# kwai/blaze

Hardware: NVIDIA H100
Metric: rows/sec on TPC-DS q1 hash-agg+filter at 1/2/4/8 H100; HBM GB/s vs 3.35 TB/s (higher is better)
Workload: dtype int64

## Files before the change

blaze_b200/csrc/capi.cu:

```cuda
#include <algorithm>
#include <cstdio>
#include <cstdlib>
#include <cstring>
#include <functional>
#include <mutex>

#include "lz4_frame.h"
#include "parquet_meta.h"
#include "runtime.h"

namespace b200q {

static thread_local std::string g_last_error;

static std::string format_of(const DType& t) {
  switch (t.id) {
    case T_BOOL: return "b"; case T_INT8: return "c"; case T_INT16: return "s"; case T_INT32: return "i"; case T_INT64: return "l";
    case T_FLOAT32: return "f"; case T_FLOAT64: return "g"; case T_DATE32: return "tdD"; case T_TIMESTAMP_US: return "tsu:";
    case T_DECIMAL128: return "d:" + std::to_string(t.precision) + "," + std::to_string(t.scale);
    case T_BINARY: return "z"; case T_UTF8: return "u"; default: return "n";
  }
}
DType type_of_format(const char* f) {
  DType d; std::string s(f ? f : "");
// ... 501 lines not shown
      const int32_t first = ho[0];
      hc.values = d2h((const uint8_t*)dc.values->ptr + first, (size_t)(ho[n] - first));
      if (first) for (int64_t i = 0; i <= n; i++) ho[i] -= first;
    } else if (dc.type.id == T_BOOL) hc.values = d2h(dc.values->ptr, (size_t)(n + 7) / 8);
    else if (dc.type.id != T_NULL) hc.values = d2h(dc.values->ptr, (size_t)n * dc.type.byte_width());
    hb.cols.push_back(hc);
  }
  B200Q_CUDA(cudaStreamSynchronize(cx.stream));
  return hb;
}

struct ArrayPriv {
  std::shared_ptr<HostBlock> block;
  std::vector<DevMemP> dev;
  std::vector<const void*> buffers;
  std::vector<ArrowArray> children; std::vector<ArrowArray*> child_ptrs;
};
static void release_array(ArrowArray* a) {
  if (!a || !a->release) return;
  auto* p = (ArrayPriv*)a->private_data;
  for (auto& c : p->children) if (c.release) c.release(&c);
  delete p; a->release = nullptr;
}
static int64_t count_nulls(const uint8_t* bits, int64_t off, int64_t n) {
  int64_t set = 0;
  for (int64_t i = 0; i < n; i++) set += (bits[(off + i) >> 3] >> ((off + i) & 7)) & 1;
  return n - set;
}
static void export_host_slice(const HostBatch& hb, int64_t off, int64_t len, ArrowArray* out) {
  auto* top = new ArrayPriv(); top->block = hb.block;
  memset(out, 0, sizeof(*out));
  out->length = len; out->null_count = 0; out->offset = 0; out->n_buffers = 1;
  top->buffers.push_back(nullptr); out->buffers = top->buffers.data();
  top->children.resize(hb.cols.size()); top->child_ptrs.resize(hb.cols.size());
  for (size_t i = 0; i < hb.cols.size(); i++) {
    const HostColumn& hc = hb.cols[i];
    auto* cp = new ArrayPriv(); cp->block = hb.block;
    ArrowArray& c = top->children[i]; memset(&c, 0, sizeof(c));
    c.length = len; c.offset = off;
    c.null_count = hc.validity ? count_nulls((const uint8_t*)hc.validity, off, len) : 0;
    if (hc.type.id == T_NULL) { c.null_count = len; c.n_buffers = 0; }
    else if (hc.type.is_varlen()) { cp->buffers = {hc.validity, hc.offsets, hc.values}; c.n_buffers = 3; }
    else { cp->buffers = {hc.validity, hc.values}; c.n_buffers = 2; }
    c.buffers = cp->buffers.data(); c.release = release_array; c.private_data = cp;
    top->child_ptrs[i] = &c;
  }
  out->n_children = (int64_t)hb.cols.size(); out->children = top->child_ptrs.data();
  out->release = release_array; out->private_data = top;
}
void export_device(DevBatch& db, int device, ArrowDeviceArray* out) {
  auto* top = new ArrayPriv();
  memset(out, 0, sizeof(*out));
  ArrowArray& a = out->array;
  a.length = db.num_rows; a.n_buffers = 1; top->buffers.push_back(nullptr); a.buffers = top->buffers.data();
  top->children.resize(db.cols.size()); top->child_ptrs.resize(db.cols.size());
  for (size_t i = 0; i < db.cols.size(); i++) {
    DevColumn& dc = db.cols[i];
    auto* cp = new ArrayPriv();
    ArrowArray& c = top->children[i]; memset(&c, 0, sizeof(c));
    c.length = db.num_rows; c.offset = dc.offset; c.null_count = dc.validity ? -1 : 0;
    const void* v = dc.validity ? dc.validity->ptr : nullptr;
    if (dc.validity) cp->dev.push_back(dc.validity);
    if (dc.values) cp->dev.push_back(dc.values);
    if (dc.offsets) cp->dev.push_back(dc.offsets);
    if (dc.type.id == T_NULL) { c.n_buffers = 0; c.null_count = db.num_rows; }
    else if (dc.type.is_varlen()) { cp->buffers = {v, dc.offsets->ptr, dc.values->ptr}; c.n_buffers = 3; }
    else { cp->buffers = {v, dc.values ? dc.values->ptr : nullptr}; c.n_buffers = 2; }
    c.buffers = cp->buffers.data(); c.release = release_array; c.private_data = cp;
    top->child_ptrs[i] = &c;
  }
  a.n_children = (int64_t)db.cols.size(); a.children = top->child_ptrs.data();
  a.release = release_array; a.private_data = top;
  out->device_id = device; out->device_type = ARROW_DEVICE_CUDA; out->sync_event = nullptr;
}

static void conf_defaults(b200q_conf* c) {
  memset(c, 0, sizeof(*c));
  c->struct_size = sizeof(b200q_conf);
  c->batch_size = 10000;
  c->suggested_batch_mem_size = 8388608;
  c->partial_agg_skipping_enable = 1;
  c->partial_agg_skipping_ratio = 0.999;
  c->partial_agg_skipping_min_rows = 20000;
  c->staging_rows = 1 << 20;
  c->agg_initial_groups = 1 << 19;
  c->max_launch_rows = 1 << 27;
  c->partial_state_columnar = 0;
  c->force_generic_kernels = 0;
  c->agg_dense_keys = 1;
  c->agg_hot_key_cache = 1;
}

}

#define B200Q_STR2(x) #x
#define B200Q_STR(x) B200Q_STR2(x)

extern "C" {

int32_t b200q_version(void) { return 100; }
const char* b200q_build_info(void) { return "blaze_b200 hot path: Filter/Project/HashAgg, sm_90a, CUDA " B200Q_STR(CUDART_VERSION); }
const char* b200q_last_error(void) { return g_last_error.c_str(); }
int32_t b200q_device_count(void) { int n = 0; if (cudaGetDeviceCount(&n) != cudaSuccess) { cudaGetLastError(); return 0; } return n; }

b200q_status b200q_conf_init(b200q_conf* conf) {
  if (!conf) return fail(B200Q_ERR_INVALID_ARG, "conf is null");
  conf_defaults(conf); return B200Q_OK;
}

b200q_status b200q_plan_explain(const uint8_t* plan, size_t plan_len, int32_t plan_kind, char* buf, size_t cap, size_t* needed) {
  return guarded(nullptr, [&] {
    PlanP p = decode_plan(plan, plan_len, plan_kind);
    std::string s = explain_plan(p);
    if (needed) *needed = s.size() + 1;
    if (buf && cap) { const size_t n = std::min(cap - 1, s.size()); memcpy(buf, s.data(), n); buf[n] = 0; }
  });
}

b200q_status b200q_op_create(const uint8_t* plan, size_t plan_len, int32_t plan_kind, const struct ArrowSchema* input_schema,
                             const b200q_conf* conf, int32_t device, b200q_op** out) {
  if (!out) return fail(B200Q_ERR_INVALID_ARG, "out is null");
  *out = nullptr;
  b200q_op* op = nullptr;
  b200q_status st = guarded(nullptr, [&] {
    PlanP p = decode_plan(plan, plan_len, plan_kind);
    resolve_scalar_subqueries(*p);
    int ndev = 0;
    if (cudaGetDeviceCount(&ndev) != cudaSuccess || ndev == 0) { cudaGetLastError(); throw ExecError(B200Q_ERR_NO_DEVICE, "no CUDA device is visible: the sm_90a kernels cannot run and there is no CPU fallback"); }
    if (device < 0 || device >= ndev) throw ExecError(B200Q_ERR_INVALID_ARG, "invalid device ordinal");
    op = new b200q_op();
    op->plan = p; op->cx.device = device;
    conf_defaults(&op->cx.conf);
    if (conf) { const size_t n = std::min<size_t>(conf->struct_size ? conf->struct_size : sizeof(b200q_conf), sizeof(b200q_conf)); memcpy(&op->cx.conf, conf, n); op->cx.conf.struct_size = sizeof(b200q_conf); }
    if (op->cx.conf.batch_size <= 0) op->cx.conf.batch_size = 10000;
    if (op->cx.conf.max_launch_rows <= 0) op->cx.conf.max_launch_rows = 1 << 27;
    if (op->cx.conf.agg_initial_groups <= 0) op->cx.conf.agg_initial_groups = 1 << 19;
    B200Q_CUDA(cudaSetDevice(device));
    {
      cudaMemPool_t pool; unsigned long long keep = ~0ULL;
      if (cudaDeviceGetDefaultMemPool(&pool, device) == cudaSuccess) cudaMemPoolSetAttribute(pool, cudaMemPoolAttrReleaseThreshold, &keep);
    }
    op->stream_ref = stream_ref_create(device);
    op->cx.stream = op->stream_ref->s;
    B200Q_CUDA(cudaEventCreate(&op->cx.ev0)); B200Q_CUDA(cudaEventCreate(&op->cx.ev1));
    build_pipeline(op);
    if (op->leaf->leaf_kind == "IpcReader") op->ipc = make_ipc_source(op->cx, op->in_schema, op->stages[0]->used_input_cols);
    if (input_schema) {
      if (input_schema->n_children != (int64_t)op->in_schema.fields.size()) throw PlanError(B200Q_ERR_INVALID_ARG, "input_schema does not match the plan leaf: column count");
      for (int64_t i = 0; i < input_schema->n_children; i++)
        if (type_of_format(input_schema->children[i]->format) != op->in_schema.fields[i].type)
          throw PlanError(B200Q_ERR_INVALID_ARG, "input_schema does not match the plan leaf: type of column " + std::to_string(i));
    }
  });
  if (st != B200Q_OK) { if (op) { op->stages.clear(); delete op; } return st; }
  *out = op;
  return B200Q_OK;
}

b200q_status b200q_op_input_schema(b200q_op* op, struct ArrowSchema* out) {
  if (!op || !out) return fail(B200Q_ERR_INVALID_ARG, "null argument");
  return guarded(nullptr, [&] { export_schema(op->in_schema, out); });
}
b200q_status b200q_op_output_schema(b200q_op* op, struct ArrowSchema* out) {
  if (!op || !out) return fail(B200Q_ERR_INVALID_ARG, "null argument");
  return guarded(nullptr, [&] { export_schema(op->out_schema, out); });
}

b200q_status b200q_op_push(b200q_op* op, struct ArrowArray* batch) {
  if (!op) return fail(B200Q_ERR_INVALID_ARG, "op is null");
  b200q_status st = guarded(op, [&] {
    check_push_state(op);
    begin_push(op, batch);
    op->cx.m.input_rows += batch->length; op->cx.m.input_batches++;
    if (batch->length == 0) return;
    const std::vector<int>& used = op->stages[0]->used_input_cols;
    const int64_t srows = op->cx.conf.staging_rows;
    if (srows > 0 && batch->length < srows / 2) { staging_append(op, batch); return; }
    if (op->staging_ready) staging_flush(op);
    DevBatch db = import_direct(op, batch, used);
    PendingRelease pr; pr.arr = *batch; batch->release = nullptr;
    B200Q_CUDA(cudaEventCreateWithFlags(&pr.ev, cudaEventDisableTiming));
    B200Q_CUDA(cudaEventRecord(pr.ev, op->cx.stream));
    op->pending.push_back(pr);
    run_stages(op, db, 0);
  });
  if (batch && batch->release) batch->release(batch);
  return st;
}

b200q_status b200q_op_push_ipc(b200q_op* op, const uint8_t* data, size_t len) {
  if (!op) return fail(B200Q_ERR_INVALID_ARG, "op is null");
  return guarded(op, [&] {
    if (op->finished) throw ExecError(B200Q_ERR_STATE, "push after finish");
    if (!op->ipc) throw ExecError(B200Q_ERR_STATE, "push_ipc: the op's leaf is not an IpcReaderExecNode");
    if (!data && len) throw ExecError(B200Q_ERR_INVALID_ARG, "push_ipc: null data");
    require_right_side(op);
    B200Q_CUDA(cudaSetDevice(op->cx.device));
    poll_pending(op, false);
    op->ipc->push(op->cx, data, len, [&](DevBatch& b) { run_stages(op, b, 0); });
  });
}

b200q_status b200q_op_push_device(b200q_op* op, struct ArrowDeviceArray* dbatch) {
  if (!op) return fail(B200Q_ERR_INVALID_ARG, "op is null");
  b200q_status st = guarded(op, [&] {
    check_push_state(op);
    if (!dbatch) throw ExecError(B200Q_ERR_INVALID_ARG, "null batch");
    if (dbatch->device_type != ARROW_DEVICE_CUDA || dbatch->device_id != op->cx.device) throw ExecError(B200Q_ERR_INVALID_ARG, "push_device: batch is not on this op's CUDA device");
    ArrowArray* batch = &dbatch->array;
    begin_push(op, batch);
    if (op->staging_ready) staging_flush(op);
    if (dbatch->sync_event) B200Q_CUDA(cudaStreamWaitEvent(op->cx.stream, *(cudaEvent_t*)dbatch->sync_event, 0));
    op->cx.m.input_rows += batch->length; op->cx.m.input_batches++;
    if (batch->length == 0) return;
    DevBatch db; db.num_rows = batch->length; db.cols.resize(op->in_schema.fields.size());
    for (size_t i = 0; i < db.cols.size(); i++) {
      const ArrowArray* c = batch->children[i]; DevColumn& dc = db.cols[i];
      dc.type = op->in_schema.fields[i].type; dc.offset = c->offset + batch->offset;
      const size_t huge = (size_t)1 << 60;
      if (c->n_buffers > 0 && c->buffers[0] && c->null_count != 0) dc.validity = DevMem::borrow(c->buffers[0], huge, nullptr);
      if (dc.type.is_varlen()) { dc.offsets = DevMem::borrow(c->buffers[1], huge, nullptr); dc.values = DevMem::borrow(c->buffers[2], huge, nullptr); }
      else if (c->n_buffers > 1 && c->buffers[1]) dc.values = DevMem::borrow(c->buffers[1], huge, nullptr);
    }
    PendingRelease pr; pr.arr = *batch;
    B200Q_CUDA(cudaEventCreateWithFlags(&pr.ev, cudaEventDisableTiming));
    batch->release = nullptr;
    op->pending.push_back(pr);
    const cudaEvent_t ev = pr.ev;
    try { run_stages(op, db, 0); } catch (...) { cudaEventRecord(ev, op->cx.stream); throw; }
    B200Q_CUDA(cudaEventRecord(ev, op->cx.stream));
  });
  if (dbatch && dbatch->array.release) dbatch->array.release(&dbatch->array);
  return st;
}

b200q_status b200q_op_finish(b200q_op* op) {
  if (!op) return fail(B200Q_ERR_INVALID_ARG, "op is null");
  return guarded(op, [&] {
    if (op->finished) return;
    require_right_side(op);
    B200Q_CUDA(cudaSetDevice(op->cx.device));
    if (op->leaf->leaf_kind == "ParquetScan") {
      if (op->cx.m.input_batches) throw ExecError(B200Q_ERR_STATE, "an op whose leaf is a ParquetScanExecNode takes no pushed batches");
      run_parquet_scan(op->cx, *op->leaf, [&](DevBatch& b) { run_stages(op, b, 0); });
    }
    if (op->ipc) op->ipc->flush(op->cx, [&](DevBatch& b) { run_stages(op, b, 0); });
    if (op->staging_ready) staging_flush(op);
    for (size_t i = 0; i < op->stages.size(); i++) {
      std::vector<DevBatch> outs;
      op->cx.cur_stage = (int)i;
      op->stages[i]->finish(op->cx, outs);
      route_outputs(op, i, outs);
    }
    B200Q_CUDA(cudaStreamSynchronize(op->cx.stream));
    poll_pending(op, true);
    op->finished = true;
  });
}

b200q_status b200q_op_pull(b200q_op* op, struct ArrowArray* out, int32_t* has_batch) {
  if (!op || !out || !has_batch) return fail(B200Q_ERR_INVALID_ARG, "null argument");
  *has_batch = 0;
  return guarded(op, [&] {
    if (op->taken) throw ExecError(B200Q_ERR_STATE, "pull: the op's output is the right side of a sort-merge join (b200q_op_attach_right)");
    B200Q_CUDA(cudaSetDevice(op->cx.device));
    if (!op->has_cur_host) {
      if (op->out_queue.empty()) return;
      op->cur_host = to_host(op, op->out_queue.front());
      op->out_queue.pop_front();
      op->has_cur_host = true;
    }
    HostBatch& hb = op->cur_host;
    const int64_t len = std::min<int64_t>(op->cx.conf.batch_size, hb.num_rows - hb.cursor);
    export_host_slice(hb, hb.cursor, len, out);
    hb.cursor += len;
    if (hb.cursor >= hb.num_rows) { op->has_cur_host = false; op->cur_host = HostBatch(); }
    op->cx.m.output_batches++;
    *has_batch = 1;
  });
}

b200q_status b200q_op_pull_device(b200q_op* op, struct ArrowDeviceArray* out, int32_t* has_batch) {
  if (!op || !out || !has_batch) return fail(B200Q_ERR_INVALID_ARG, "null argument");
  *has_batch = 0;
  return guarded(op, [&] {
    if (op->taken) throw ExecError(B200Q_ERR_STATE, "pull_device: the op's output is the right side of a sort-merge join (b200q_op_attach_right)");
    if (op->has_cur_host) throw ExecError(B200Q_ERR_STATE, "pull_device while a host batch is partially pulled");
    if (op->out_queue.empty()) return;
    B200Q_CUDA(cudaSetDevice(op->cx.device));
    B200Q_CUDA(cudaStreamSynchronize(op->cx.stream));
    export_device(op->out_queue.front(), op->cx.device, out);
    op->out_queue.pop_front();
    op->cx.m.output_batches++;
    *has_batch = 1;
  });
}

b200q_status b200q_op_sync(b200q_op* op) {
  if (!op) return fail(B200Q_ERR_INVALID_ARG, "op is null");
  return guarded(op, [&] { B200Q_CUDA(cudaSetDevice(op->cx.device)); B200Q_CUDA(cudaStreamSynchronize(op->cx.stream)); poll_pending(op, true); });
}

b200q_status b200q_op_metrics(b200q_op* op, b200q_metrics* out) {
  if (!op || !out) return fail(B200Q_ERR_INVALID_ARG, "null argument");
  const Metrics& m = op->cx.m;
  b200q_metrics r; memset(&r, 0, sizeof(r)); r.struct_size = sizeof(r);
  r.input_rows = m.input_rows; r.input_batches = m.input_batches; r.output_rows = m.output_rows; r.output_batches = m.output_batches;
  r.elapsed_compute_ns = (int64_t)(m.gpu_ms * 1e6); r.gpu_kernel_launches = m.launches; r.h2d_bytes = m.h2d_bytes; r.d2h_bytes = m.d2h_bytes;
  r.hot_kernel_ns = (int64_t)(m.hot_ms * 1e6); r.hot_kernel_rows = m.hot_rows; r.hot_kernel_launches = m.hot_launches;
  r.num_groups = m.num_groups; r.table_capacity_slots = m.table_capacity; r.table_grow_count = m.grow_count; r.fast_path_launches = m.fast_launches;
  const size_t n = std::min<size_t>(out->struct_size ? out->struct_size : sizeof(r), sizeof(r));
  memcpy(out, &r, n);
  return B200Q_OK;
}

void b200q_op_destroy(b200q_op* op) {
  if (!op) return;
  cudaSetDevice(op->cx.device);
  if (op->cx.stream) cudaStreamSynchronize(op->cx.stream);
  poll_pending(op, true);
  op->out_queue.clear(); op->has_cur_host = false; op->cur_host = HostBatch();
  op->ipc.reset();
  op->stages.clear();
  staging_free(op);
  if (op->cx.ev0) cudaEventDestroy(op->cx.ev0);
  if (op->cx.ev1) cudaEventDestroy(op->cx.ev1);
  if (op->cx.stream) cudaStreamSynchronize(op->cx.stream);
  delete op;
}

b200q_status b200q_parquet_explain(const uint8_t* footer, size_t n, char* buf, size_t cap, size_t* needed) {
  return guarded(nullptr, [&] {
    const PqFileMeta m = parquet_parse_footer(footer, n);
    std::string o = "rows=" + std::to_string(m.num_rows) + " flat=" + (m.flat ? "true" : "false") + "\n";
    for (auto& c : m.columns) o += "column " + c.name + " physical=" + std::to_string(c.type) + (c.optional ? " optional" : " required") + " arrow=" + (c.arrow.id == T_NULL ? std::string("unsupported") : c.arrow.str()) + "\n";
    for (size_t g = 0; g < m.row_groups.size(); g++) {
      o += "row_group " + std::to_string(g) + " rows=" + std::to_string(m.row_groups[g].num_rows) + "\n";
      for (size_t c = 0; c < m.row_groups[g].columns.size(); c++) {
        const PqColumnChunk& cc = m.row_groups[g].columns[c];
        o += "  chunk " + std::to_string(c) + " codec=" + std::to_string(cc.codec) + " values=" + std::to_string(cc.num_values) + " start=" + std::to_string(cc.start()) + " bytes=" + std::to_string(cc.total_compressed_size) +
             " nulls=" + std::to_string(cc.stats.null_count) + " min_max=" + (cc.stats.has_min && cc.stats.has_max ? "yes" : "no") + "\n";
      }
    }
    if (needed) *needed = o.size() + 1;
    if (buf && cap) { const size_t k = std::min(cap - 1, o.size()); memcpy(buf, o.data(), k); buf[k] = 0; }
  });
}
b200q_status b200q_snappy_uncompress(const uint8_t* src, size_t n, uint8_t* dst, size_t cap, size_t* out_len) {
  if ((!src && n) || !out_len) return fail(B200Q_ERR_INVALID_ARG, "null argument");
  return guarded(nullptr, [&] {
    ByteBuf v; snappy_uncompress(src, n, v);
    *out_len = v.size();
    if (!dst || cap < v.size()) throw ExecError(B200Q_ERR_INVALID_ARG, "snappy output needs " + std::to_string(v.size()) + " bytes");
    if (v.size()) memcpy(dst, v.data(), v.size());
  });
}
b200q_status b200q_set_file_reader(b200q_file_reader_fn fn, void* ctx) { set_file_reader(fn, ctx); return B200Q_OK; }
b200q_status b200q_set_scalar_subquery_resolver(b200q_scalar_subquery_fn fn, void* ctx) { set_scalar_subquery_resolver((void*)fn, ctx); return B200Q_OK; }

b200q_status b200q_op_attach_build(b200q_op* probe_op, b200q_op* build_op) {
  if (!probe_op || !build_op) return fail(B200Q_ERR_INVALID_ARG, "null argument");
  return guarded(probe_op, [&] {
    const JoinBuildResult* b = build_op->stages.empty() ? nullptr : dynamic_cast<const JoinBuildResult*>(build_op->stages.back().get());
    if (!b) throw ExecError(B200Q_ERR_STATE, "attach_build: the build op's plan is not rooted at a BroadcastJoinBuildHashMapExecNode");
    if (!build_op->finished || !b->built()) throw ExecError(B200Q_ERR_STATE, "attach_build: finish the build op first");
    JoinProbeAttach* a = nullptr;
    for (auto& st : probe_op->stages) if (auto* j = dynamic_cast<JoinProbeAttach*>(st.get())) a = j;
    if (!a) throw ExecError(B200Q_ERR_STATE, "attach_build: the probe op's plan has no join");
    a->attach(b->built());
  });
}

b200q_status b200q_op_attach_right(b200q_op* join_op, b200q_op* right_op) {
  if (!join_op || !right_op || join_op == right_op) return fail(B200Q_ERR_INVALID_ARG, "attach_right: null or identical op handles");
  if (right_op->sticky_code) return fail(right_op->sticky_code, right_op->sticky_error);
  return guarded(join_op, [&] {
    SmjRightAttach* j = smj_of(join_op);
    if (!j) throw ExecError(B200Q_ERR_STATE, "attach_right: the op's plan has no SortMergeJoinExecNode");
    if (j->right_attached()) throw ExecError(B200Q_ERR_STATE, "attach_right: a right side is already attached");
    if (join_op->finished || join_op->cx.m.input_batches) throw ExecError(B200Q_ERR_STATE, "attach_right: the join op already has input");
    if (!right_op->finished) throw ExecError(B200Q_ERR_STATE, "attach_right: finish the right op first");
    if (right_op->taken || right_op->has_cur_host || right_op->cx.m.output_batches) throw ExecError(B200Q_ERR_STATE, "attach_right: the right op's output has already been pulled or attached");
    if (right_op->cx.device != join_op->cx.device) throw ExecError(B200Q_ERR_INVALID_ARG, "attach_right: the right op runs on another device");
    B200Q_CUDA(cudaSetDevice(join_op->cx.device));
    std::vector<DevBatch> batches(right_op->out_queue.begin(), right_op->out_queue.end());
    j->attach_right(join_op->cx, batches, right_op->out_schema);
    right_op->out_queue.clear();
    right_op->taken = true;
  });
}

b200q_status b200q_op_shuffle_chunk_count(b200q_op* op, int64_t* out_count) {
  if (!op || !out_count) return fail(B200Q_ERR_INVALID_ARG, "null argument");
  return guarded(op, [&] {
    const ShuffleResult* r = op->stages.empty() ? nullptr : dynamic_cast<const ShuffleResult*>(op->stages.back().get());
    if (!r) throw ExecError(B200Q_ERR_STATE, "the plan is not rooted at a ShuffleWriterExecNode");
    *out_count = r->chunk_count();
  });
}
b200q_status b200q_op_shuffle_chunk(b200q_op* op, int64_t index, b200q_shuffle_chunk* out) {
  if (!op || !out) return fail(B200Q_ERR_INVALID_ARG, "null argument");
  return guarded(op, [&] {
    const ShuffleResult* r = op->stages.empty() ? nullptr : dynamic_cast<const ShuffleResult*>(op->stages.back().get());
    if (!r) throw ExecError(B200Q_ERR_STATE, "the plan is not rooted at a ShuffleWriterExecNode");
    if (index < 0 || index >= r->chunk_count()) throw ExecError(B200Q_ERR_INVALID_ARG, "shuffle chunk index out of range");
    r->chunk(index, out);
  });
}
b200q_status b200q_lz4_frame_compress(const uint8_t* src, size_t n, uint8_t* dst, size_t cap, size_t* out_len) {
  if ((!src && n) || !out_len) return fail(B200Q_ERR_INVALID_ARG, "null argument");
  return guarded(nullptr, [&] {
    std::vector<uint8_t> v; lz4_frame_append(src, n, v);
    *out_len = v.size();
    if (!dst || cap < v.size()) throw ExecError(B200Q_ERR_INVALID_ARG, "lz4 frame needs " + std::to_string(v.size()) + " bytes");
    memcpy(dst, v.data(), v.size());
  });
}

b200q_status b200q_lz4_frame_decompress(const uint8_t* src, size_t n, uint8_t* dst, size_t cap, size_t* out_len) {
  if ((!src && n) || !out_len) return fail(B200Q_ERR_INVALID_ARG, "null argument");
  return guarded(nullptr, [&] {
    size_t bound = 0;
    try {
      bound = lz4_frame_bound(src, n);
      if (dst && cap >= bound) { *out_len = lz4_frame_decompress(src, n, dst, cap); return; }
      std::vector<uint8_t> v(bound);
      *out_len = lz4_frame_decompress(src, n, v.data(), v.size());
      if (dst && cap >= *out_len) { memcpy(dst, v.data(), *out_len); return; }
    } catch (const Lz4FrameError& e) {
      throw ExecError(B200Q_ERR_INVALID_ARG, std::string(e.what()) + " at byte " + std::to_string(e.offset));
    }
    throw ExecError(B200Q_ERR_INVALID_ARG, "lz4 frame content needs " + std::to_string(*out_len) + " bytes");
  });
}

b200q_status b200q_murmur3_partition(const struct ArrowSchema* key_schema, const struct ArrowDeviceArray* keys, int32_t num_partitions,
                                     uint32_t* out_pids_device, void* cuda_stream) {
  return guarded(nullptr, [&] {
    if (!key_schema || !keys || !out_pids_device) throw ExecError(B200Q_ERR_INVALID_ARG, "null argument");
    if (num_partitions <= 0) throw ExecError(B200Q_ERR_INVALID_ARG, "num_partitions must be positive");
    const ArrowArray& a = keys->array;
    if (a.n_children != key_schema->n_children || a.n_children > VM_MAX_COLS) throw ExecError(B200Q_ERR_INVALID_ARG, "key schema / array mismatch");
    ColTable ct{}; uint8_t phys[VM_MAX_COLS];
    for (int64_t i = 0; i < a.n_children; i++) {
      const DType t = type_of_format(key_schema->children[i]->format);
      if (t.is_varlen()) throw ExecError(B200Q_ERR_UNSUPPORTED, "murmur3 partition ids over a " + t.str() + " key are not on the GPU path");
      const ArrowArray* c = a.children[i];
      DevColumn dc; dc.type = t; dc.offset = c->offset + a.offset;
      phys[i] = phys_of(t);
      const int w = t.byte_width();
      ct.col[i].values = c->n_buffers > 1 ? (const uint8_t*)c->buffers[1] + (size_t)dc.offset * w : nullptr;
      ct.col[i].validity = (c->n_buffers > 0 && c->null_count != 0) ? (const uint8_t*)c->buffers[0] : nullptr;
      ct.col[i].bit_offset = (uint32_t)dc.offset;
    }
    launch_murmur3_partition(ct, phys, (int)a.n_children, a.length, num_partitions, out_pids_device, (cudaStream_t)cuda_stream);
    B200Q_CUDA(cudaGetLastError());
  });
}

}
```

blaze_b200/csrc/kernels.cu:

```cuda
#include <cstdio>
#include <cstdlib>
#include <cuda_runtime.h>
#include <stdint.h>

#include "agg_device.cuh"
#include "kernels.cuh"
#include "vm.cuh"
#include "emit_device.cuh"

namespace b200q {

__device__ __forceinline__ void load_program(const VmProgram* __restrict__ g, VmInstr* s_code, uint64_t* s_pool) {
  const uint32_t nc = g->n_code, np = g->n_pool;
  for (uint32_t i = threadIdx.x; i < nc; i += blockDim.x) s_code[i] = g->code[i];
  for (uint32_t i = threadIdx.x; i < np; i += blockDim.x) s_pool[i] = g->pool[i];
  __syncthreads();
}

constexpr int FP_BLOCK = 256;
constexpr int FP_R = 2;
constexpr int FP_TILE = FP_BLOCK * FP_R;
constexpr int FP_NW = FP_BLOCK / 32;
constexpr unsigned long long ST_AGG = 1ULL << 62, ST_PREFIX = 2ULL << 62, ST_VALUE = (1ULL << 62) - 1;

// ... 465 lines not shown
  unsigned flags;
  bool inserted = false;
  const uint64_t slot = agg_find_or_insert(lay, tab, kw, knull, h, &flags, &inserted);
  if (slot == AGG_NO_SLOT) return false;
  if (inserted) atomicAdd(tab.counters, 1ULL);
  unsigned long long* const ke = tab.keys + slot * (uint64_t)lay.kstride;
  unsigned long long* const ae = tab.accs + slot * (uint64_t)lay.astride;
  const uint32_t skip = sd->acc_skip;
  int lost = -1;
  for (int j = 0; j < lay.nacc; j++) {
    if ((skip >> j) & 1) continue;
    const AccOp a = lay.acc[j];
    if (acc_is_first(a.kind)) {
      const int o = sd->acc_arg[j][0];
      const bool ov = o != AGG_NO_ARG && ((vb >> o) & 1);
      if (a.oword != lost && first_eligible(a, lay, buf, vb, o, sd->acc_arg[j][1]) &&
          !first_apply(ke, ae, a, buf + lay.out_word[o == AGG_NO_ARG ? 0 : o], ov, ord)) lost = a.oword;
      continue;
    }
    bool valid = true;
    for (int i = 0; i < 4; i++) { const int o = sd->acc_arg[j][i]; if (o != AGG_NO_ARG) valid = valid && ((vb >> o) & 1); }
    if (!valid) continue;
    const int o = sd->acc_arg[j][0];
    acc_apply(a.kind, ke, ae + a.word, buf + lay.out_word[o == AGG_NO_ARG ? 0 : o]);
    slot_mark(ke, flags, a.vbit);
  }
  return true;
}

__global__ void __launch_bounds__(AG_BLOCK) agg_update_kernel(const VmProgram* __restrict__ prog, const ColTable cols, const AggLayout lay, const AggTable tab,
                                                              long long row_begin, long long n, const uint32_t* __restrict__ row_list,
                                                              unsigned long long ord_base) {
  __shared__ VmInstr s_code[VM_MAX_CODE];
  __shared__ uint64_t s_pool[VM_MAX_POOL];
  load_program(prog, s_code, s_pool);
  int* err = (int*)(tab.counters + 2);
  const long long ntiles = (n + AG_TILE - 1) / AG_TILE;
  for (long long tile = blockIdx.x; tile < ntiles; tile += gridDim.x) {
    long long row[AG_R]; bool inb[AG_R], alive[AG_R];
    uint32_t rel[AG_R];
#pragma unroll
    for (int r = 0; r < AG_R; r++) {
      const long long i = tile * AG_TILE + r * AG_BLOCK + threadIdx.x;
      inb[r] = i < n; alive[r] = inb[r];
      rel[r] = inb[r] ? (row_list ? row_list[i] : (uint32_t)i) : 0;
      row[r] = row_begin + rel[r];
    }
    uint64_t buf[AG_R][AGG_MAX_ROW_WORDS];
    uint32_t vb[AG_R];
#pragma unroll
    for (int r = 0; r < AG_R; r++) vb[r] = 0;
    AggSink sink{buf, vb, lay.out_word};
    vm_run<AG_R>(s_code, s_pool, 0, cols, row, inb, alive, err, sink);
#pragma unroll
    for (int r = 0; r < AG_R; r++) {
      if (alive[r] && !agg_upsert(lay, tab, buf[r], vb[r], ord_base + (unsigned long long)row[r])) {
        const unsigned long long at = atomicAdd(tab.counters + 1, 1ULL);
        tab.deferred[at] = rel[r];
      }
    }
  }
}

__global__ void __launch_bounds__(AG_BLOCK) agg_update_sets_kernel(const VmProgram* __restrict__ prog, const ColTable cols, const AggLayout lay, const AggTable tab,
                                                                   long long row_begin, long long n, const uint32_t* __restrict__ row_list,
                                                                   const AggSetDesc* __restrict__ sets, int nsets, unsigned long long ord_base) {
  __shared__ VmInstr s_code[VM_MAX_CODE];
  __shared__ uint64_t s_pool[VM_MAX_POOL];
  load_program(prog, s_code, s_pool);
  int* err = (int*)(tab.counters + 2);
  const long long ntiles = (n + AG_TILE - 1) / AG_TILE;
  for (long long tile = blockIdx.x; tile < ntiles; tile += gridDim.x) {
    long long row[AG_R]; bool inb[AG_R], alive[AG_R];
    uint32_t rel[AG_R]; int only[AG_R];
#pragma unroll
    for (int r = 0; r < AG_R; r++) {
      const long long i = tile * AG_TILE + r * AG_BLOCK + threadIdx.x;
      inb[r] = i < n; alive[r] = inb[r];
      const uint32_t e = inb[r] ? (row_list ? row_list[i] : (uint32_t)i) : 0;
      rel[r] = row_list ? e / (uint32_t)nsets : e;
      only[r] = row_list ? (int)(e % (uint32_t)nsets) : -1;
      row[r] = row_begin + rel[r];
    }
    uint64_t buf[AG_R][AGG_MAX_ROW_WORDS];
    uint32_t vb[AG_R];
#pragma unroll
    for (int r = 0; r < AG_R; r++) vb[r] = 0;
    AggSink sink{buf, vb, lay.out_word};
    vm_run<AG_R>(s_code, s_pool, 0, cols, row, inb, alive, err, sink);
#pragma unroll
    for (int r = 0; r < AG_R; r++) {
      if (!alive[r]) continue;
      const int s0 = only[r] < 0 ? 0 : only[r], s1 = only[r] < 0 ? nsets : only[r] + 1;
      for (int s = s0; s < s1; s++) {
        if (!agg_upsert_set(lay, tab, buf[r], vb[r], sets + s, (ord_base + (unsigned long long)row[r]) * (unsigned)nsets + (unsigned)s)) {
          const unsigned long long at = atomicAdd(tab.counters + 1, 1ULL);
          tab.deferred[at] = rel[r] * (uint32_t)nsets + (uint32_t)s;
        }
      }
    }
  }
}

static int grid_for(int64_t ntiles, int per_sm) {
  int dev = 0, sms = 132; cudaGetDevice(&dev); cudaDeviceGetAttribute(&sms, cudaDevAttrMultiProcessorCount, dev);
  const int64_t cap = (int64_t)sms * per_sm;
  return (int)(ntiles < cap ? (ntiles < 1 ? 1 : ntiles) : cap);
}

int launch_agg_update(const VmProgram* d_prog, const ColTable& cols, const AggLayout& lay, const AggTable& tab, int64_t row_begin, int64_t n,
                      const uint32_t* d_row_list, uint64_t ord_base, cudaStream_t s) {
  if (n <= 0) return 0;
  const int64_t ntiles = (n + AG_TILE - 1) / AG_TILE;
  agg_update_kernel<<<grid_for(ntiles, 8), AG_BLOCK, 0, s>>>(d_prog, cols, lay, tab, row_begin, n, d_row_list, ord_base);
  return 1;
}

int launch_agg_update_sets(const VmProgram* d_prog, const ColTable& cols, const AggLayout& lay, const AggTable& tab, int64_t row_begin, int64_t n,
                           const uint32_t* d_row_list, const AggSetDesc* d_sets, int nsets, uint64_t ord_base, cudaStream_t s) {
  if (n <= 0) return 0;
  const int64_t ntiles = (n + AG_TILE - 1) / AG_TILE;
  agg_update_sets_kernel<<<grid_for(ntiles, 8), AG_BLOCK, 0, s>>>(d_prog, cols, lay, tab, row_begin, n, d_row_list, d_sets, nsets, ord_base);
  return 1;
}

__global__ void __launch_bounds__(256) agg_rehash_kernel(const AggLayout lay, const AggTable old_tab, const AggTable new_tab) {
  const uint64_t cap = old_tab.capacity;
  for (uint64_t i = blockIdx.x * (uint64_t)blockDim.x + threadIdx.x; i < cap; i += (uint64_t)gridDim.x * blockDim.x) {
    const unsigned long long* src = old_tab.keys + i * (uint64_t)lay.kstride;
    const unsigned long long hdr = src[0];
    if ((unsigned)hdr < 2) continue;
    const unsigned knull = (unsigned)(hdr >> 48);
    const uint64_t h = agg_hash_words((const uint64_t*)src + 1, lay.nkw, knull);
    uint64_t s = agg_first_slot(h, new_tab.capacity);
    while (true) {
      unsigned long long* dst = new_tab.keys + s * (uint64_t)lay.kstride;
      if (atomicCAS((unsigned*)dst, TAG_EMPTY, TAG_LOCKED) == TAG_EMPTY) {
        for (int w = 1; w < lay.kstride; w++) dst[w] = src[w];
        for (int w = 0; w < lay.astride; w++) new_tab.accs[s * (uint64_t)lay.astride + w] = old_tab.accs[i * (uint64_t)lay.astride + w];
        ((unsigned*)dst)[1] = (unsigned)(hdr >> 32) & ~FLAG_SLOT_LOCK;
        __threadfence();
        st_release_u32((unsigned*)dst, (unsigned)hdr);
        atomicAdd(new_tab.counters, 1ULL);
        break;
      }
      s = agg_next_slot(s, new_tab.capacity);
    }
  }
}

int launch_agg_rehash(const AggLayout& lay, const AggTable& old_tab, const AggTable& new_tab, cudaStream_t s) {
  const int64_t cap = (int64_t)old_tab.capacity;
  agg_rehash_kernel<<<grid_for((cap + 255) / 256, 8), 256, 0, s>>>(lay, old_tab, new_tab);
  return 1;
}

__global__ void __launch_bounds__(256) agg_emit_kernel(const AggLayout lay, const AggTable tab, const EmitTable emit, unsigned long long* out_count) {
  const uint64_t cap = tab.capacity;
  const unsigned lane = threadIdx.x & 31;
  const uint64_t stride = (uint64_t)gridDim.x * blockDim.x;
  const uint64_t rounds = (cap + stride - 1) / stride;
  for (uint64_t it = 0; it < rounds; it++) {
    const uint64_t i = it * stride + blockIdx.x * (uint64_t)blockDim.x + threadIdx.x;
    const unsigned long long* ke = tab.keys + i * (uint64_t)lay.kstride;
    const unsigned long long* slot = tab.accs + i * (uint64_t)lay.astride;
    unsigned long long hdr = 0;
    if (i < cap) hdr = ke[0];
    const bool occ = (unsigned)hdr >= 2;
    const unsigned m = __ballot_sync(0xffffffffu, occ);
    if (!m) continue;
    unsigned long long base = 0;
    if (lane == 0) base = atomicAdd(out_count, (unsigned long long)__popc(m));
    base = __shfl_sync(0xffffffffu, base, 0);
    if (!occ) continue;
    const unsigned long long at = base + __popc(m & lanemask_lt());
    const unsigned flags = (unsigned)(hdr >> 32);
    emit_row_columns(emit, at, ke, slot, flags);
  }
}

int launch_agg_emit(const AggLayout& lay, const AggTable& tab, const EmitTable& emit, unsigned long long* d_out_count, cudaStream_t s) {
  const int64_t cap = (int64_t)tab.capacity;
  agg_emit_kernel<<<grid_for((cap + 255) / 256, 8), 256, 0, s>>>(lay, tab, emit, d_out_count);
  return 1;
}

__global__ void __launch_bounds__(256) pack_valid_kernel(const uint8_t* __restrict__ bytes, uint32_t* __restrict__ bits, long long n) {
  const long long nwords = (n + 31) / 32;
  const unsigned lane = threadIdx.x & 31;
  const long long warp_id = (blockIdx.x * (long long)blockDim.x + threadIdx.x) >> 5, nwarps = ((long long)gridDim.x * blockDim.x) >> 5;
  for (long long w = warp_id; w < nwords; w += nwarps) {
    const long long i = w * 32 + lane;
    const unsigned m = __ballot_sync(0xffffffffu, i < n && bytes[i] != 0);
    if (lane == 0) bits[w] = m;
  }
}

int launch_pack_valid(const uint8_t* bytes, uint32_t* bits, int64_t n, cudaStream_t s) {
  if (n <= 0) return 0;
  pack_valid_kernel<<<grid_for((n + 8191) / 8192, 8), 256, 0, s>>>(bytes, bits, n);
  return 1;
}

__device__ __forceinline__ int varint_len(unsigned long long v) { int n = 1; while (v >= 128) { v >>= 7; n++; } return n; }

__device__ __forceinline__ unsigned long long state_value_bits(const FrozenField& f, long long i, unsigned long long& hi) {
  hi = 0;
  switch (f.phys) {
    case PH_I8: return (unsigned long long)(long long)((const int8_t*)f.values)[i];
    case PH_I16: return (unsigned long long)(long long)((const int16_t*)f.values)[i];
    case PH_I32: return (unsigned long long)(long long)((const int32_t*)f.values)[i];
    case PH_F32: return (unsigned long long)((const uint32_t*)f.values)[i];
    case PH_DEC128: hi = ((const unsigned long long*)f.values)[2 * i + 1]; return ((const unsigned long long*)f.values)[2 * i];
    default: return ((const unsigned long long*)f.values)[i];
  }
}

__global__ void __launch_bounds__(256) frozen_lengths_kernel(const FrozenTable ft, long long n, int32_t* __restrict__ lengths) {
  for (long long i = blockIdx.x * (long long)blockDim.x + threadIdx.x; i < n; i += (long long)gridDim.x * blockDim.x) {
    int len = 0;
    for (int k = 0; k < ft.nfields; k++) {
      const FrozenField& f = ft.f[k];
      if (f.kind == FZ_COUNT) len += varint_len(((const unsigned long long*)f.values)[i]);
      else if (f.kind == FZ_BOOL) len += 1;
      else len += 1 + ((f.valid ? f.valid[i] != 0 : true) ? f.width : 0);
    }
    lengths[i] = len;
  }
}

__global__ void __launch_bounds__(256) frozen_write_kernel(const FrozenTable ft, long long n, const int32_t* __restrict__ offsets, uint8_t* __restrict__ data) {
  for (long long i = blockIdx.x * (long long)blockDim.x + threadIdx.x; i < n; i += (long long)gridDim.x * blockDim.x) {
    uint8_t* p = data + offsets[i];
    for (int k = 0; k < ft.nfields; k++) {
      const FrozenField& f = ft.f[k];
      if (f.kind == FZ_COUNT) {
        unsigned long long v = ((const unsigned long long*)f.values)[i];
        while (v >= 128) { *p++ = (uint8_t)(128 + (v & 127)); v >>= 7; }
        *p++ = (uint8_t)v;
      } else if (f.kind == FZ_BOOL) {
        const uint8_t v = ((const uint8_t*)f.values)[i] != 0;
        *p++ = f.valid ? (f.valid[i] ? 1 + v : 0) : (v ? 2 : 0);
      } else {
        const bool valid = f.valid ? f.valid[i] != 0 : true;
        *p++ = valid ? 1 : 0;
        if (valid) {
          unsigned long long hi, lo = state_value_bits(f, i, hi);
          for (int b = 0; b < f.width && b < 8; b++) *p++ = (uint8_t)(lo >> (8 * b));
          for (int b = 8; b < f.width; b++) *p++ = (uint8_t)(hi >> (8 * (b - 8)));
        }
      }
    }
  }
}

__global__ void __launch_bounds__(256) frozen_read_kernel(const FrozenTable ft, long long n, const int32_t* __restrict__ offsets, long long obase,
                                                          const uint8_t* __restrict__ data, int* err) {
  for (long long i = blockIdx.x * (long long)blockDim.x + threadIdx.x; i < n; i += (long long)gridDim.x * blockDim.x) {
    const uint8_t* p = data + offsets[obase + i];
    const uint8_t* end = data + offsets[obase + i + 1];
    for (int k = 0; k < ft.nfields; k++) {
      const FrozenField& f = ft.f[k];
      if (f.kind == FZ_COUNT) {
        unsigned long long v = 0; int shift = 0;
        while (true) {
          if (p >= end) { atomicOr(err, 4); break; }
          const uint8_t b = *p++;
          if (b < 128) { v += (unsigned long long)b << shift; break; }
          v += (unsigned long long)(b - 128) << shift; shift += 7;
        }
        ((unsigned long long*)f.values)[i] = v;
      } else if (f.kind == FZ_BOOL) {
        if (p >= end) { atomicOr(err, 4); break; }
        const uint8_t b = *p++;
        if (f.valid) { ((uint8_t*)f.valid)[i] = b != 0; ((uint8_t*)f.values)[i] = b > 1; }
        else ((uint8_t*)f.values)[i] = b != 0;
      } else {
        if (p >= end) { atomicOr(err, 4); break; }
        const bool valid = *p++ == 1;
        unsigned long long lo = 0, hi = 0;
        if (valid) {
          if (p + f.width > end) { atomicOr(err, 4); break; }
          for (int b = 0; b < f.width && b < 8; b++) lo |= (unsigned long long)(*p++) << (8 * b);
          for (int b = 8; b < f.width; b++) hi |= (unsigned long long)(*p++) << (8 * (b - 8));
        }
        ((uint8_t*)f.valid)[i] = valid ? 1 : 0;
        switch (f.phys) {
          case PH_I8: ((int8_t*)f.values)[i] = (int8_t)lo; break;
          case PH_I16: ((int16_t*)f.values)[i] = (int16_t)lo; break;
          case PH_I32: case PH_F32: ((uint32_t*)f.values)[i] = (uint32_t)lo; break;
          case PH_DEC128: ((unsigned long long*)f.values)[2 * i] = lo; ((unsigned long long*)f.values)[2 * i + 1] = hi; break;
          default: ((unsigned long long*)f.values)[i] = lo; break;
        }
      }
    }
  }
}

int launch_frozen_lengths(const FrozenTable& ft, int64_t n, int32_t* lengths, cudaStream_t s) {
  if (n <= 0) return 0;
  frozen_lengths_kernel<<<grid_for((n + 255) / 256, 8), 256, 0, s>>>(ft, n, lengths); return 1;
}
int launch_frozen_write(const FrozenTable& ft, int64_t n, const int32_t* offsets, uint8_t* data, cudaStream_t s) {
  if (n <= 0) return 0;
  frozen_write_kernel<<<grid_for((n + 255) / 256, 8), 256, 0, s>>>(ft, n, offsets, data); return 1;
}
// ... 278 lines not shown
```

blaze_b200/csrc/kernels.cuh:

```cuda
#pragma once
#include <cuda_runtime.h>
#include <stdint.h>

#include "vm.h"

namespace b200q {

constexpr int AGG_MAX_KEYS = 8;
constexpr int AGG_MAX_ACC = 16;
constexpr int AGG_MAX_ROW_WORDS = 24;
constexpr int AGG_MAX_SLOT_WORDS = 32;

enum AccKind : uint8_t {
  ACC_ADD_I64 = 0,
  ACC_ADD_F64,
  ACC_ADD_DEC,
  ACC_COUNT,
  ACC_MIN_I64, ACC_MAX_I64,
  ACC_MIN_F64, ACC_MAX_F64,
  ACC_MIN_DEC, ACC_MAX_DEC,
  ACC_FIRST,
  ACC_FIRST_VALID,
};
__host__ __device__ inline bool acc_is_first(uint8_t kind) { return kind == ACC_FIRST || kind == ACC_FIRST_VALID; }

struct AccOp {
  uint8_t kind;
  uint8_t word;
  uint8_t vbit;
  uint8_t nargs;
  uint8_t arg_out[4];
  uint8_t oword;
  uint8_t nwords;
};

struct AggLayout {
  int32_t nkeys, nkw, nacc, kstride, astride, nouts;
  uint8_t key_out[AGG_MAX_KEYS];
  uint8_t key_word[AGG_MAX_KEYS];
  uint8_t key_nwords[AGG_MAX_KEYS];
  uint8_t out_word[VM_MAX_OUT];
  AccOp acc[AGG_MAX_ACC];
  uint64_t init[AGG_MAX_SLOT_WORDS];
  uint32_t init_flags;
};

constexpr int AGG_MAX_SETS = 64;
constexpr uint8_t AGG_KEY_CONST = 0xFF;
constexpr uint8_t AGG_NO_ARG = 0xFF;
struct AggSetDesc {
  uint8_t key_out[AGG_MAX_KEYS];
  uint8_t acc_arg[AGG_MAX_ACC][4];
  uint32_t key_null;
  uint32_t acc_skip;
  uint64_t key_const[AGG_MAX_KEYS * 2];
};

struct AggTable {
  unsigned long long* keys;
  unsigned long long* accs;
  uint64_t capacity;
  uint64_t max_groups;
  unsigned long long* counters;
  uint32_t* deferred;
};

enum EmitKind : uint8_t {
  EMIT_KEY = 0,
  EMIT_ACC_VALUE,
  EMIT_AVG_F64,
  EMIT_AVG_DEC,
  EMIT_FIRST_VALUE,
  EMIT_FIRST_FLAG,
};
struct EmitCol {
  uint8_t kind, phys, word, word2;
  uint8_t vbit;
  uint8_t key;
  uint8_t sum_is_f64;
  uint8_t is_order_key;
  void* values;
  uint8_t* valid_bytes;
};
constexpr int EMIT_MAX_COLS = 40;
struct EmitTable { int32_t ncols; EmitCol col[EMIT_MAX_COLS]; };

enum FrozenKind : uint8_t { FZ_PRIM = 0, FZ_COUNT = 1, FZ_BOOL = 2 };
struct FrozenField {
  uint8_t kind;
  uint8_t width;
  uint8_t phys;
  uint8_t _pad;
  const void* values;
  const uint8_t* valid;
};
constexpr int FROZEN_MAX_FIELDS = 32;
struct FrozenTable { int32_t nfields; FrozenField f[FROZEN_MAX_FIELDS]; };

int launch_filter_project(const VmProgram* d_prog, const ColTable& cols, const OutTable& outs, int nouts, int64_t n,
                          bool has_filters, unsigned long long* d_tile_status, unsigned long long* d_scratch ,
                          cudaStream_t s);
int64_t filter_project_num_tiles(int64_t n);

struct LeanFpSpec {
  int32_t nfilt, nout;
  struct { int8_t col; uint8_t op; uint8_t _pad[6]; long long lit; } filt[4];
  struct { uint8_t kind; int8_t a; int8_t b; uint8_t _pad[5]; long long lit; } out[8];
};
int launch_filter_project_lean(const ColTable& cols, int ncols , const LeanFpSpec& sp, long long* const* out_values, int64_t n,
                               void* d_work , unsigned long long* d_scratch, cudaStream_t s);
int64_t filter_project_lean_scratch_bytes(int64_t n);

int launch_agg_update(const VmProgram* d_prog, const ColTable& cols, const AggLayout& lay, const AggTable& tab, int64_t row_begin, int64_t n,
                      const uint32_t* d_row_list , uint64_t ord_base, cudaStream_t s);
int launch_agg_update_sets(const VmProgram* d_prog, const ColTable& cols, const AggLayout& lay, const AggTable& tab, int64_t row_begin, int64_t n,
                           const uint32_t* d_row_list, const AggSetDesc* d_sets, int nsets, uint64_t ord_base, cudaStream_t s);
int launch_agg_rehash(const AggLayout& lay, const AggTable& old_tab, const AggTable& new_tab, cudaStream_t s);
int launch_agg_emit(const AggLayout& lay, const AggTable& tab, const EmitTable& emit, unsigned long long* d_out_count, cudaStream_t s);
int launch_pack_valid(const uint8_t* bytes, uint32_t* bits, int64_t n, cudaStream_t s);
int launch_frozen_lengths(const FrozenTable& ft, int64_t n, int32_t* lengths, cudaStream_t s);
int launch_exclusive_scan_i32(const int32_t* in, int32_t* out , int64_t n, int32_t* d_block_sums, cudaStream_t s);
int launch_frozen_write(const FrozenTable& ft, int64_t n, const int32_t* offsets, uint8_t* data, cudaStream_t s);
int launch_frozen_read(const FrozenTable& ft, int64_t n, const int32_t* offsets, int64_t offsets_base, const uint8_t* data, int* d_err, cudaStream_t s);
int launch_murmur3_partition(const ColTable& cols, const uint8_t* phys, int ncols, int64_t n, int32_t num_partitions, uint32_t* out, cudaStream_t s);
int64_t scan_num_blocks(int64_t n);

int launch_varlen_lengths(const DevCol& src, const uint32_t* sel, int64_t m, int32_t* lengths, uint32_t* out_valid, unsigned long long* d_total, cudaStream_t s);
int launch_varlen_copy(const DevCol& src, const uint32_t* sel, int64_t m, const int32_t* out_offsets, uint8_t* out_data, cudaStream_t s);

constexpr int IPC_TILE = 1024;
constexpr int IPC_COPY_PIECE = 32768;
struct IpcFixedJob { const uint8_t* src; uint8_t* dst; int64_t rows; int32_t width; int32_t _pad; };
struct IpcTile { int32_t job; int32_t row0; };
struct IpcBitCol { uint32_t* dst; const uint8_t* const* src; };
struct IpcCopy { const uint8_t* src; uint8_t* dst; int64_t len; };
int launch_ipc_decode_fixed(const IpcFixedJob* jobs, const IpcTile* tiles, int64_t ntiles, cudaStream_t s);
int launch_ipc_decode_bits(const IpcBitCol* cols, int ncols, const int64_t* rec_row , int64_t nrec, int64_t rows, cudaStream_t s);
int launch_ipc_decode_bytes(const IpcCopy* copies, int64_t n, cudaStream_t s);

}
```

blaze_b200/csrc/kernels_fast.cu:

```cuda
#include <algorithm>
#include <cstdlib>
#include <cuda_runtime.h>
#include <stdint.h>

#include "agg_device.cuh"
#include "kernels_fast.cuh"

namespace b200q {

constexpr int FA_BLOCK = 256;

__device__ __forceinline__ uint64_t make_evict_first_policy() {
  uint64_t pol; asm volatile("createpolicy.fractional.L2::evict_first.b64 %0, 1.0;" : "=l"(pol)); return pol;
}
__device__ __forceinline__ long long ld_stream_s64(const long long* p) {
  long long v; const uint64_t pol = make_evict_first_policy();
  asm volatile("ld.global.nc.L1::no_allocate.L2::cache_hint.s64 %0, [%1], %2;" : "=l"(v) : "l"(p), "l"(pol)); return v;
}
__device__ __forceinline__ bool col_valid(const DevCol& c, long long i) {
  if (!c.validity) return true;
  const unsigned long long bi = (unsigned long long)i + c.bit_offset;
  return (__ldg(c.validity + (bi >> 3)) >> (bi & 7)) & 1;
}
__device__ __forceinline__ long long col_load_int(const DevCol& c, int phys, long long i) {
// ... 536 lines not shown
  __syncthreads();
  const unsigned lane = threadIdx.x & 31;
  const long long gwarp = (long long)blockIdx.x * (FA_BLOCK / 32) + (threadIdx.x >> 5), nwarps = (long long)gridDim.x * (FA_BLOCK / 32);
  const long long nunits = (n + 31) / 32;
  const bool add0 = fs.acc[0].kind == FAST_ACC_ADD, add1 = NACC == 2 && fs.acc[1].kind == FAST_ACC_ADD;

  for (long long unit0 = gwarp * U; unit0 < nunits; unit0 += nwarps * U) {
    long long k[U], k1[U]; unsigned long long v0[U], v1[U]; bool alive[U]; unsigned meta[U];
#pragma unroll
    for (int u = 0; u < U; u++) {
      const long long rel = (unit0 + u) * 32 + lane, row = row_begin + rel;
      alive[u] = rel < n; meta[u] = 0xC; k[u] = 0; k1[u] = 0; v0[u] = 1; v1[u] = 1;
      if (!alive[u]) continue;
      if (!TYPED) {
        k[u] = ld_stream_vec((const long long*)cols.col[fs.key_col[0]].values + row, (i64xG<1>*)nullptr).v[0];
        if (NK == 2) k1[u] = ld_stream_vec((const long long*)cols.col[fs.key_col[1]].values + row, (i64xG<1>*)nullptr).v[0];
        if (add0) v0[u] = (unsigned long long)ld_stream_vec((const long long*)cols.col[fs.acc[0].col].values + row, (i64xG<1>*)nullptr).v[0];
        if (add1) v1[u] = (unsigned long long)ld_stream_vec((const long long*)cols.col[fs.acc[1].col].values + row, (i64xG<1>*)nullptr).v[0];
      } else {
        { const DevCol& c = cols.col[fs.key_col[0]]; if (col_valid(c, row)) k[u] = col_load_int(c, fs.key_phys[0], row); else meta[u] |= 1u; }
        if (NK == 2) { const DevCol& c = cols.col[fs.key_col[1]]; if (col_valid(c, row)) k1[u] = col_load_int(c, fs.key_phys[1], row); else meta[u] |= 2u; }
        if (fs.acc[0].col >= 0) {
          const DevCol& c = cols.col[fs.acc[0].col];
          if (!col_valid(c, row)) { meta[u] &= ~4u; v0[u] = 0; } else if (add0) v0[u] = (unsigned long long)col_load_int(c, fs.acc[0].phys, row);
        }
        if (NACC == 2 && fs.acc[1].col >= 0) {
          const DevCol& c = cols.col[fs.acc[1].col];
          if (!col_valid(c, row)) { meta[u] &= ~8u; v1[u] = 0; } else if (add1) v1[u] = (unsigned long long)col_load_int(c, fs.acc[1].phys, row);
        }
      }
    }
    for (int f = 0; f < fs.nfilt; f++) {
      const DevCol& c = cols.col[fs.filt[f].col];
#pragma unroll
      for (int u = 0; u < U; u++) {
        const long long row = row_begin + (unit0 + u) * 32 + lane;
        if (!alive[u]) continue;
        if (!TYPED) alive[u] = cmp_apply(fs.filt[f].op, ld_stream_vec((const long long*)c.values + row, (i64xG<1>*)nullptr).v[0], fs.filt[f].lit);
        else alive[u] = col_valid(c, row) && cmp_apply(fs.filt[f].op, col_load_int(c, fs.filt[f].phys, row), fs.filt[f].lit);
      }
    }
#pragma unroll
    for (int u = 0; u < U; u++) {
      unsigned long long idx;
      const bool in = dense_index<NK>(fs, k[u], k1[u], idx) && alive[u] && !(meta[u] & 3u);
      if (in) {
        unsigned* const e = s_tab + 2 * (unsigned)idx * G;
#pragma unroll
        for (int m = 0; m < 4; m++) {
          if (m >= G) break;
          const int src = fs.dense_word_src[m];
          if (src == -1) smem_add64(e + 2 * m, 1ULL);
          else if (src == 0) { if (meta[u] & 4u) smem_add64(e + 2 * m, v0[u]); }
          else if (src == 1 && NACC == 2) { if (meta[u] & 8u) smem_add64(e + 2 * m, v1[u]); }
          else if (src >= 2) { if (meta[u] & (4u << (src - 2))) smem_add64(e + 2 * m, 1ULL); }
        }
      }
      const bool fb = alive[u] && !in;
      if (__any_sync(0xffffffffu, fb)) {
        bool inserted = false;
        if (fb) {
          uint64_t kw[2] = {(uint64_t)k[u], NK == 2 ? (uint64_t)k1[u] : 0ULL};
          const unsigned knull = meta[u] & 3u;
          unsigned fl = 0;
          const uint64_t si = agg_find_or_insert(lay, tab, kw, knull, agg_hash2(kw[0], kw[1], knull), &fl, &inserted);
          if (si == AGG_NO_SLOT) { const unsigned long long at = atomicAdd(tab.counters + 1, 1ULL); tab.deferred[at] = (uint32_t)((unit0 + u) * 32 + lane); }
          else {
            unsigned long long* const p = tab.accs + si * (uint64_t)lay.astride;
            unsigned long long* const ke = tab.keys + si * (uint64_t)lay.kstride;
            if (meta[u] & 4u) { red_add_u64(p + fs.acc[0].word, v0[u]); slot_mark(ke, fl, fs.acc[0].vbit); }
            if (NACC == 2 && (meta[u] & 8u)) { red_add_u64(p + fs.acc[1].word, v1[u]); slot_mark(ke, fl, fs.acc[1].vbit); }
          }
        }
        const unsigned b = __ballot_sync(0xffffffffu, inserted);
        if (lane == 0 && b) atomicAdd(tab.counters, (unsigned long long)__popc(b));
      }
    }
  }
  __syncthreads();
  for (unsigned w = threadIdx.x; w < nwords; w += FA_BLOCK) {
    const unsigned long long val = (unsigned long long)s_tab[2 * w] | ((unsigned long long)s_tab[2 * w + 1] << 32);
    if (val) red_add_u64(fs.dense_tab + w, val);
  }
}

static int fast_grid(int64_t ntiles) {
  int dev = 0, sms = 132; cudaGetDevice(&dev); cudaDeviceGetAttribute(&sms, cudaDevAttrMultiProcessorCount, dev);
  const int64_t cap = (int64_t)sms * 8;
  return (int)(ntiles < cap ? (ntiles < 1 ? 1 : ntiles) : cap);
}

int launch_agg_fast_update(const ColTable& cols, const FastSpec& fs, const AggLayout& lay, const AggTable& tab, int64_t row_begin, int64_t n, cudaStream_t s) {
  if (n <= 0) return 0;
  const int dg = fs.dense ? fs.dense_stride : 0;
  if (dg && fs.dense_cap * (unsigned long long)dg <= (unsigned long long)DS_MAX_WORDS) {
    const int g = (int)std::max<int64_t>(1, std::min<int64_t>((n + FA_BLOCK * 4 - 1) / (FA_BLOCK * 4), (int64_t)fast_grid(1 << 30) / 8 * 3));
#define B200Q_DS(NACC, TYPED, NK) agg_dense_smem_kernel<NACC, TYPED, NK><<<g, FA_BLOCK, 0, s>>>(cols, fs, lay, tab, row_begin, n)
    if (fs.nkeys == 1) {
      if (fs.lean) { if (fs.nacc == 2) B200Q_DS(2, false, 1); else B200Q_DS(1, false, 1); } else { if (fs.nacc == 2) B200Q_DS(2, true, 1); else B200Q_DS(1, true, 1); }
    } else {
      if (fs.lean) { if (fs.nacc == 2) B200Q_DS(2, false, 2); else B200Q_DS(1, false, 2); } else { if (fs.nacc == 2) B200Q_DS(2, true, 2); else B200Q_DS(1, true, 2); }
    }
#undef B200Q_DS
    return 1;
  }
  if (dg && fs.lean && fs.hot_cache) {
    const int g = fast_grid((n + 32 * 8 * 4 - 1) / (32 * 8 * 4));
#define B200Q_HC(NACC, NK, G) agg_dense_hot_kernel<NACC, NK, G><<<g, FA_BLOCK, 0, s>>>(cols, fs, lay, tab, row_begin, n)
    if (fs.nkeys == 1) {
      if (fs.nacc == 2) { if (dg == 2) B200Q_HC(2, 1, 2); else B200Q_HC(2, 1, 4); } else { if (dg == 2) B200Q_HC(1, 1, 2); else B200Q_HC(1, 1, 4); }
    } else {
      if (fs.nacc == 2) { if (dg == 2) B200Q_HC(2, 2, 2); else B200Q_HC(2, 2, 4); } else { if (dg == 2) B200Q_HC(1, 2, 2); else B200Q_HC(1, 2, 4); }
    }
#undef B200Q_HC
    return 1;
  }
  if (dg && fs.lean && fs.nkeys == 1 && fs.nfilt == 0) {
    const int u = dg == 2 ? 4 : 2;
    const int g = fast_grid((n + 32 * 8 * u - 1) / (32 * 8 * u));
#define B200Q_LD(NACC, G) agg_lean_dense_kernel<NACC, G, 1><<<g, FA_BLOCK, 0, s>>>(cols, fs, lay, tab, row_begin, n)
    if (fs.nacc == 2) { if (dg == 2) B200Q_LD(2, 2); else B200Q_LD(2, 4); } else { if (dg == 2) B200Q_LD(1, 2); else B200Q_LD(1, 4); }
#undef B200Q_LD
    return 1;
  }
  if (dg && fs.nfcol >= 0) {
    if (fs.filt_never) return 0;
    return launch_agg_tile_dense(cols, fs, lay, tab, row_begin, n, s);
  }
  if (dg) {
    const int g = fast_grid((n + 32 * 8 * 4 - 1) / (32 * 8 * 4));
#define B200Q_DR(NACC, NK, G) do { if (fs.lean) agg_dense_row_kernel<NACC, NK, G, false><<<g, FA_BLOCK, 0, s>>>(cols, fs, lay, tab, row_begin, n); \
                                   else agg_dense_row_kernel<NACC, NK, G, true><<<g, FA_BLOCK, 0, s>>>(cols, fs, lay, tab, row_begin, n); } while (0)
    if (fs.nkeys == 1) {
      if (fs.nacc == 2) { if (dg == 2) B200Q_DR(2, 1, 2); else B200Q_DR(2, 1, 4); } else { if (dg == 2) B200Q_DR(1, 1, 2); else B200Q_DR(1, 1, 4); }
    } else {
      if (fs.nacc == 2) { if (dg == 2) B200Q_DR(2, 2, 2); else B200Q_DR(2, 2, 4); } else { if (dg == 2) B200Q_DR(1, 2, 2); else B200Q_DR(1, 2, 4); }
    }
#undef B200Q_DR
    return 1;
  }
  if (!dg) {
    const int64_t tiles = (n + 32 * (LH_BLOCK / 32) * LH_U - 1) / (32 * (LH_BLOCK / 32) * LH_U);
    const int g = (int)std::max<int64_t>(1, std::min<int64_t>(tiles, (int64_t)fast_grid(1 << 30) / 8 * (fs.lean ? 6 : 4)));
#define B200Q_LH(NK, NACC, TYPED) agg_lean_hash_kernel<NK, NACC, TYPED><<<g, LH_BLOCK, 0, s>>>(cols, fs, lay, tab, row_begin, n)
    if (fs.lean) { if (fs.nkeys == 1) { if (fs.nacc == 2) B200Q_LH(1, 2, false); else B200Q_LH(1, 1, false); } else { if (fs.nacc == 2) B200Q_LH(2, 2, false); else B200Q_LH(2, 1, false); } }
    else { if (fs.nkeys == 1) { if (fs.nacc == 2) B200Q_LH(1, 2, true); else B200Q_LH(1, 1, true); } else { if (fs.nacc == 2) B200Q_LH(2, 2, true); else B200Q_LH(2, 1, true); } }
#undef B200Q_LH
    return 1;
  }
  return 0;
}

__global__ void __launch_bounds__(256) key_range_kernel(const DevCol col, int phys, long long n, long long* out ) {
  long long mn = INT64_MAX, mx = INT64_MIN; unsigned long long cnt = 0;
  for (long long i = blockIdx.x * (long long)blockDim.x + threadIdx.x; i < n; i += (long long)gridDim.x * blockDim.x) {
    if (!col_valid(col, i)) continue;
    const long long v = col_load_int(col, phys, i);
    mn = v < mn ? v : mn; mx = v > mx ? v : mx; cnt++;
  }
#pragma unroll
  for (int d = 16; d > 0; d >>= 1) {
    const long long a = __shfl_xor_sync(0xffffffffu, mn, d), b = __shfl_xor_sync(0xffffffffu, mx, d);
    mn = a < mn ? a : mn; mx = b > mx ? b : mx; cnt += __shfl_xor_sync(0xffffffffu, cnt, d);
  }
  if ((threadIdx.x & 31) == 0) { atomicMin(out, mn); atomicMax(out + 1, mx); atomicAdd((unsigned long long*)out + 2, cnt); }
}
int launch_key_skew_probe(const DevCol* key_cols, const uint8_t* phys, int nkeys, int64_t n, unsigned* d_hist, cudaStream_t s) {
  key_skew_hist_kernel<<<fast_grid((n + 2047) / 2048), 256, 0, s>>>(key_cols[0], key_cols[nkeys == 2 ? 1 : 0], phys[0], phys[nkeys == 2 ? 1 : 0], nkeys, n, d_hist);
  key_skew_max_kernel<<<32, 256, 0, s>>>(d_hist);
  return 2;
}
int launch_key_range(const DevCol& col, int phys, int64_t n, long long* d_out, cudaStream_t s) {
  key_range_kernel<<<fast_grid((n + 2047) / 2048), 256, 0, s>>>(col, phys, n, d_out);
  return 1;
}

__device__ __forceinline__ void dense_store(const EmitCol& c, unsigned long long at, uint64_t lo, bool valid) {
  if (c.valid_bytes) c.valid_bytes[at] = valid ? 1 : 0;
  switch (c.phys) {
    case PH_BOOL: ((uint8_t*)c.values)[at] = lo != 0; break;
    case PH_I8: ((int8_t*)c.values)[at] = (int8_t)lo; break;
    case PH_I16: ((int16_t*)c.values)[at] = (int16_t)lo; break;
    case PH_I32: ((int32_t*)c.values)[at] = (int32_t)lo; break;
    default: ((uint64_t*)c.values)[at] = lo; break;
  }
}
__global__ void __launch_bounds__(256) agg_emit_dense_kernel(const FastSpec fs, const EmitTable emit, const DenseEmitMap map, unsigned long long* out_count) {
  const unsigned lane = threadIdx.x & 31;
  const uint64_t stride = (uint64_t)gridDim.x * blockDim.x;
  const uint64_t rounds = (fs.dense_cap + stride - 1) / stride;
  for (uint64_t it = 0; it < rounds; it++) {
    const uint64_t i = it * stride + blockIdx.x * (uint64_t)blockDim.x + threadIdx.x;
    const uint64_t pe = fs.nkeys == 2 && fs.dense_key0_minor ? dense_entry2(fs, i / fs.dense_r1, i % fs.dense_r1) : i;
    const unsigned long long* e = fs.dense_tab + pe * fs.dense_stride;
    const bool occ = i < fs.dense_cap && e[fs.dense_presence_word] != 0;
    const unsigned m = __ballot_sync(0xffffffffu, occ);
    if (!m) continue;
    unsigned long long base = 0;
    if (lane == 0) base = atomicAdd(out_count, (unsigned long long)__popc(m));
    base = __shfl_sync(0xffffffffu, base, 0);
    if (!occ) continue;
    const unsigned long long at = base + __popc(m & lanemask_lt());
    for (int c = 0; c < emit.ncols; c++) {
      const EmitCol ec = emit.col[c];
      if (ec.kind == EMIT_KEY) {
        const long long kv = fs.nkeys == 1 ? fs.dense_base + (long long)i
                           : ec.key == 0 ? fs.dense_base + (long long)(i / fs.dense_r1) : fs.dense_base1 + (long long)(i % fs.dense_r1);
        dense_store(ec, at, (uint64_t)kv, true);
      }
      else {
        const int w = map.word[c], vw = map.valid_word[c];
        const bool valid = vw == 0xFF ? true : e[vw] != 0;
        dense_store(ec, at, valid ? e[w] : 0, valid);
      }
    }
  }
}
int launch_agg_emit_dense(const FastSpec& fs, const EmitTable& emit, const DenseEmitMap& map, unsigned long long* d_out_count, cudaStream_t s) {
  agg_emit_dense_kernel<<<fast_grid(((int64_t)fs.dense_cap + 255) / 256), 256, 0, s>>>(fs, emit, map, d_out_count);
  return 1;
}

__global__ void __launch_bounds__(256) dense_count_kernel(const FastSpec fs, unsigned long long* out) {
  unsigned long long c = 0;
  for (uint64_t i = blockIdx.x * (uint64_t)blockDim.x + threadIdx.x; i < fs.dense_cap; i += (uint64_t)gridDim.x * blockDim.x)
    c += fs.dense_tab[i * fs.dense_stride + fs.dense_presence_word] != 0;
#pragma unroll
  for (int d = 16; d > 0; d >>= 1) c += __shfl_xor_sync(0xffffffffu, c, d);
  if ((threadIdx.x & 31) == 0 && c) atomicAdd(out, c);
}
int launch_dense_count(const FastSpec& fs, unsigned long long* d_out, cudaStream_t s) {
  dense_count_kernel<<<fast_grid(((int64_t)fs.dense_cap + 255) / 256), 256, 0, s>>>(fs, d_out);
  return 1;
}

}
```

blaze_b200/csrc/kernels_fast.cuh:

```cuda
#pragma once
#include <cstddef>

#include "kernels.cuh"

namespace b200q {

enum FastAccKind : uint8_t { FAST_ACC_ADD = 0, FAST_ACC_COUNT = 1 };

struct FilterInterval { int8_t col; uint8_t phys; uint8_t _pad[6]; long long lo; unsigned long long span; };

struct FastSpec {
  int32_t nkeys, nacc, nfilt, dense;
  int32_t lean, hot_cache;
  int8_t key_col[2]; uint8_t key_phys[2];
  struct { uint8_t kind; int8_t col; uint8_t phys; uint8_t vbit; uint8_t word; uint8_t _pad[3]; } acc[2];
  struct { int8_t col; uint8_t phys; uint8_t op; uint8_t _pad[5]; long long lit; } filt[4];
  int32_t nfcol;
  int32_t filt_never;
  FilterInterval frange[2];
  long long dense_base;
  unsigned long long dense_cap;
  long long dense_base1;
  unsigned long long dense_r1, dense_cap0;
  unsigned long long* dense_tab;
  int8_t dense_stride;
  int8_t dense_word_src[4];
  uint8_t dense_presence_word;
  uint8_t dense_key0_minor;
  uint8_t _pad1;
  unsigned long long* sink;
};
constexpr int FAST_SINK_WARPS = 4096;

struct DenseEmitMap { uint8_t word[EMIT_MAX_COLS]; uint8_t valid_word[EMIT_MAX_COLS]; };

__device__ __forceinline__ unsigned long long dense_entry2(const FastSpec& fs, unsigned long long d0, unsigned long long d1) {
  return fs.dense_key0_minor ? d1 * fs.dense_cap0 + d0 : d0 * fs.dense_r1 + d1;
}
template <int NK>
__device__ __forceinline__ bool dense_index_of(const FastSpec& fs, long long k0, long long k1, unsigned long long& idx) {
  const unsigned long long d0 = (unsigned long long)(k0 - fs.dense_base);
  if (NK == 1) { idx = d0; return d0 < fs.dense_cap; }
  const unsigned long long d1 = (unsigned long long)(k1 - fs.dense_base1);
  idx = dense_entry2(fs, d0, d1);
  return d0 < fs.dense_cap0 && d1 < fs.dense_r1;
}

enum TileFlavour : uint8_t { TF_ADD_U64 = 0, TF_ADD_F64 = 1, TF_MIN_S64 = 2 };
__host__ __device__ constexpr unsigned long long tile_identity(int flavour) {
  return flavour == TF_MIN_S64 ? 0x7FFFFFFFFFFFFFFFULL : flavour == TF_ADD_F64 ? 0x8000000000000000ULL : 0ULL;
}
enum TileArgCvt : uint8_t { TC_NONE = 0, TC_I2F = 1 , TC_ORDER = 2  };
enum TileRecon : uint8_t { TR_COPY = 0 , TR_NOT = 1 ,
                           TR_F2I = 2 , TR_DEC3 = 3  };
struct TileWord {
  uint8_t srcsel;
  uint8_t sh;
  uint8_t gate;
  uint8_t _pad[5];
  unsigned long long msk, inv, cst;
};
struct TileAggSpec {
  int32_t nkeys, nargs, nfcol, filt_never, nacc, G, flavour, arg_is_dec;
  int8_t key_col[2]; uint8_t key_phys[2];
  int8_t arg_col[2]; uint8_t arg_phys[2]; uint8_t arg_cvt[2]; uint8_t arg_values[2];
  FilterInterval frange[2];
  long long dense_base, dense_base1;
  unsigned long long dense_cap, dense_r1, dense_cap0;
  unsigned long long* dense_tab;
  unsigned long long* sink;
  unsigned long long dec_mul;
  TileWord word[8];
  uint8_t presence_word, dec_word , _pad2[6];
  struct { int8_t arg; uint8_t recon; uint8_t w0; uint8_t valid_word; uint8_t lay_acc; uint8_t _pad[3]; } acc[4];
};
static_assert(sizeof(FastSpec) == 232 && offsetof(FastSpec, frange) == 120, "FastSpec layout");
static_assert(sizeof(TileAggSpec) == 456 && offsetof(TileAggSpec, frange) == 48, "TileAggSpec layout");

int launch_agg_tile_wide(const ColTable& cols, const TileAggSpec& ts, const AggLayout& lay, const AggTable& tab, int64_t row_begin, int64_t n, cudaStream_t s);
int launch_tile_wide_init(const TileAggSpec& ts, cudaStream_t s);
int launch_tile_wide_count(const TileAggSpec& ts, unsigned long long* d_out, cudaStream_t s);
int launch_tile_wide_normalise(const TileAggSpec& ts, cudaStream_t s);
int launch_tile_wide_emit(const TileAggSpec& ts, const AggLayout& lay, const EmitTable& emit, unsigned long long* d_out_count, cudaStream_t s);

int launch_agg_tile_dense(const ColTable& cols, const FastSpec& fs, const AggLayout& lay, const AggTable& tab, int64_t row_begin, int64_t n, cudaStream_t s);
int launch_agg_fast_update(const ColTable& cols, const FastSpec& fs, const AggLayout& lay, const AggTable& tab, int64_t row_begin, int64_t n, cudaStream_t s);
int launch_key_skew_probe(const DevCol* key_cols, const uint8_t* phys, int nkeys, int64_t n, unsigned* d_hist , cudaStream_t s);
int launch_key_range(const DevCol& col, int phys, int64_t n, long long* d_out, cudaStream_t s);
int launch_agg_emit_dense(const FastSpec& fs, const EmitTable& emit, const DenseEmitMap& map, unsigned long long* d_out_count, cudaStream_t s);
int launch_dense_count(const FastSpec& fs, unsigned long long* d_out, cudaStream_t s);

}
```

blaze_b200/csrc/kernels_tile.cu:

```cuda
#include <cuda_runtime.h>
#include <stdint.h>

#include <algorithm>

#include "agg_device.cuh"
#include "emit_device.cuh"
#include "kernels_fast.cuh"

namespace b200q {

constexpr int TL_BLOCK = 256, TL_WARPS = TL_BLOCK / 32, TL_ROWS = 128;

__device__ __forceinline__ uint64_t tl_policy_evict_first() {
  uint64_t pol; asm volatile("createpolicy.fractional.L2::evict_first.b64 %0, 1.0;" : "=l"(pol)); return pol;
}
__device__ __forceinline__ void tl_ld_b64(const long long* p, unsigned on, uint64_t pol, long long& v) {
  asm volatile("{\n\t.reg .pred q;\n\tsetp.ne.u32 q, %2, 0;\n\t@q ld.global.nc.L1::no_allocate.L2::cache_hint.b64 %0, [%1], %3;\n\t}"
               : "+l"(v) : "l"(p), "r"(on), "l"(pol));
}
__device__ __forceinline__ void tl_ld_v2b64(const long long* p, unsigned on, uint64_t pol, long long& a, long long& b) {
  asm volatile("{\n\t.reg .pred q;\n\tsetp.ne.u32 q, %3, 0;\n\t@q ld.global.nc.L1::no_allocate.L2::cache_hint.v2.b64 {%0,%1}, [%2], %4;\n\t}"
               : "+l"(a), "+l"(b) : "l"(p), "r"(on), "l"(pol));
}
__device__ __forceinline__ void tl_ld_b32(const int* p, unsigned on, uint64_t pol, int& v) {
// ... 227 lines not shown
  const bool a16 = ((uintptr_t)c.values & 15) == 0;
#pragma unroll
  for (int j = 0; j < 4; j++) {
    lo[j] = 0; hi[j] = 0;
    if (a16) tl_ld_v2b64(p + 64 * j, (ld >> j) & 1u, pol, lo[j], hi[j]);
    else { tl_ld_b64(p + 64 * j, (ld >> j) & 1u, pol, lo[j]); tl_ld_b64(p + 64 * j + 1, (ld >> j) & 1u, pol, hi[j]); }
  }
}

__device__ __forceinline__ unsigned long long tw_convert(long long v, int cvt) {
  if (cvt == TC_I2F) return f64_bits(__ll2double_rn(v));
  if (cvt == TC_ORDER) return (unsigned long long)total_order_key((uint64_t)v);
  return (unsigned long long)v;
}

__device__ __forceinline__ void tw_slot_update(const AggLayout& lay, const TileAggSpec& ts, unsigned long long* ke, unsigned long long* ae, unsigned flags,
                                               unsigned long long x0, unsigned long long x1, bool valid0, bool valid1) {
  for (int a = 0; a < ts.nacc; a++) {
    const AccOp op = lay.acc[ts.acc[a].lay_acc];
    const int arg = ts.acc[a].arg;
    const bool valid = arg < 0 ? true : (arg == 0 ? valid0 : valid1);
    if (!valid) continue;
    const unsigned long long x = arg == 1 ? x1 : x0;
    unsigned long long* w = ae + op.word;
    switch (op.kind) {
      case ACC_ADD_I64: red_add_u64(w, x); break;
      case ACC_ADD_F64: red_add_f64(w, as_f64(x)); break;
      case ACC_ADD_DEC: { const unsigned long long old = atomicAdd(w, x0); red_add_u64(w + 1, x1 + ((old + x0) < old ? 1ULL : 0ULL)); break; }
      case ACC_COUNT: red_add_u64(w, 1ULL); break;
      case ACC_MIN_I64: case ACC_MIN_F64: red_min_s64(w, (long long)x); break;
      default: red_max_s64(w, (long long)x); break;
    }
    slot_mark(ke, flags, op.vbit);
  }
}

template <int NK, int NF, int G, int FLAV>
__global__ void __launch_bounds__(TL_BLOCK, TW_MIN_CTAS(NK, NF)) agg_tile_wide_kernel(const ColTable cols, const TileAggSpec ts, const AggLayout lay, const AggTable tab, long long row_begin, long long n) {
  constexpr unsigned IDX_MASK = 0x0FFFFFFFu, ALWAYS = 1u << 30, FULL = 0xffffffffu;
  __shared__ TileQueue queues[TL_WARPS];
  TileQueue& q = queues[threadIdx.x >> 5];
  const unsigned lane = threadIdx.x & 31, qw = lane & (G - 1);
  const long long gwarp = (long long)blockIdx.x * TL_WARPS + (threadIdx.x >> 5), nwarps = (long long)gridDim.x * TL_WARPS;
  const long long ntiles = (n + TL_ROWS - 1) / TL_ROWS;
  const TileWord tw = ts.word[qw];
  const bool use1 = tw.srcsel == 1, use_c = tw.srcsel == 2;
  const unsigned long long noop = tw_noop<FLAV>();
  unsigned long long* const sink = ts.sink + ((gwarp & (FAST_SINK_WARPS - 1)) << 2) + (lane & 3);
  const uint64_t pol = tl_policy_evict_first();
  const bool dec = ts.arg_is_dec != 0;

  long long f[NF > 0 ? NF : 1][4]; unsigned fv[NF > 0 ? NF : 1];
  tl_load_filters<NF>(cols, ts.frange, row_begin, gwarp * TL_ROWS + lane, n, pol, f, fv);
  for (long long tile = gwarp; tile < ntiles; tile += nwarps) {
    const long long rel0 = tile * TL_ROWS + lane, row0 = row_begin + rel0;
    const unsigned alive = tl_pass<NF>(ts.frange, f, fv, tl_rows_in(rel0, n));
    long long k0[4], k1[4], a0[4], a1[4]; unsigned kv0, kv1 = 0xF, av0 = 0xF, av1 = 0xF;
    tl_column<NF>(cols, ts.frange, f, fv, ts.key_col[0], ts.key_phys[0], row0, alive, true, pol, k0, kv0);
    if (NK == 2) tl_column<NF>(cols, ts.frange, f, fv, ts.key_col[1], ts.key_phys[1], row0, alive, true, pol, k1, kv1);
    else { k1[0] = k1[1] = k1[2] = k1[3] = 0; }
    a0[0] = a0[1] = a0[2] = a0[3] = 0; a1[0] = a1[1] = a1[2] = a1[3] = 0;
    if (dec) {
      tl_load_dec(cols.col[ts.arg_col[0]], row0, alive, pol, a0, a1, av0); av1 = av0;
      if (ts.dec_mul != 1) {
#pragma unroll
        for (int j = 0; j < 4; j++) { const i128_t v = mk128((uint64_t)a0[j], (uint64_t)a1[j]) * (i128_t)ts.dec_mul; a0[j] = (long long)lo64(v); a1[j] = (long long)hi64(v); }
      }
    }
    else {
      if (ts.nargs > 0) tl_column<NF>(cols, ts.frange, f, fv, ts.arg_col[0], ts.arg_phys[0], row0, alive, ts.arg_values[0] != 0, pol, a0, av0);
      if (ts.nargs > 1) tl_column<NF>(cols, ts.frange, f, fv, ts.arg_col[1], ts.arg_phys[1], row0, alive, ts.arg_values[1] != 0, pol, a1, av1);
    }
    tl_load_filters<NF>(cols, ts.frange, row_begin, rel0 + nwarps * TL_ROWS, n, pol, f, fv);
    const unsigned knull = (~kv0 | (NK == 2 ? ~kv1 : 0u)) & 0xFu;
    int total = 0; unsigned fb = 0;
#pragma unroll
    for (int j = 0; j < 4; j++) {
      const unsigned long long d0 = (unsigned long long)(k0[j] - ts.dense_base), d1 = (unsigned long long)(k1[j] - ts.dense_base1);
      const unsigned long long di = NK == 1 ? d0 : d0 * ts.dense_r1 + d1;
      const bool inr = NK == 1 ? d0 < ts.dense_cap : (d0 < ts.dense_cap0 && d1 < ts.dense_r1);
      const bool live = (alive >> j) & 1u;
      const bool in = inr && live && !((knull >> j) & 1u);
      fb |= (unsigned)(live && !in) << j;
      const unsigned m = __ballot_sync(FULL, in);
      if (in) {
        const int at = total + __popc(m & lanemask_lt());
        q.idx[at] = (unsigned)di | (((av0 >> j) & 1u) << 28) | (((av1 >> j) & 1u) << 29) | ALWAYS;
        q.v0[at] = dec ? (unsigned long long)a0[j] : tw_convert(a0[j], ts.arg_cvt[0]);
        q.v1[at] = dec ? (unsigned long long)a1[j] : tw_convert(a1[j], ts.arg_cvt[1]);
      }
      total += __popc(m);
    }
    __syncwarp();
    for (int e0 = 0; e0 < total; e0 += 32 / G) {
      const int e = e0 + (int)(lane / G);
      const bool live = e < total;
      const int er = live ? e : 0;
      const unsigned pk = q.idx[er];
      const unsigned long long x = use1 ? q.v1[er] : q.v0[er];
      unsigned long long val = use_c ? tw.cst : (((x >> tw.sh) & tw.msk) ^ tw.inv);
      const bool on = live && ((pk >> tw.gate) & 1u);
      val = on ? val : noop;
      tw_red<FLAV>(live ? ts.dense_tab + (uint64_t)(pk & IDX_MASK) * G + qw : sink, val);
    }
    __syncwarp();
    if (__any_sync(FULL, fb != 0)) {
#pragma unroll
      for (int j = 0; j < 4; j++) {
        bool inserted = false;
        if ((fb >> j) & 1u) {
          const unsigned kn = ((~kv0 >> j) & 1u) | (NK == 2 ? (((~kv1 >> j) & 1u) << 1) : 0u);
          uint64_t kw[2] = {(kn & 1u) ? 0ULL : (uint64_t)k0[j], (NK == 2 && !(kn & 2u)) ? (uint64_t)k1[j] : 0ULL};
          unsigned fl = 0;
          const uint64_t si = agg_find_or_insert(lay, tab, kw, kn, agg_hash2(kw[0], kw[1], kn), &fl, &inserted);
          if (si == AGG_NO_SLOT) { const unsigned long long at = atomicAdd(tab.counters + 1, 1ULL); tab.deferred[at] = (uint32_t)(rel0 + 32 * j); }
          else tw_slot_update(lay, ts, tab.keys + si * (uint64_t)lay.kstride, tab.accs + si * (uint64_t)lay.astride, fl,
                              dec ? (unsigned long long)a0[j] : tw_convert(a0[j], ts.arg_cvt[0]), dec ? (unsigned long long)a1[j] : tw_convert(a1[j], ts.arg_cvt[1]),
                              (av0 >> j) & 1u, (av1 >> j) & 1u);
        }
        const unsigned bl = __ballot_sync(FULL, inserted);
        if (lane == 0 && bl) atomicAdd(tab.counters, (unsigned long long)__popc(bl));
      }
    }
  }
}

int launch_agg_tile_wide(const ColTable& cols, const TileAggSpec& ts, const AggLayout& lay, const AggTable& tab, int64_t row_begin, int64_t n, cudaStream_t s) {
  if (n <= 0 || ts.filt_never) return 0;
  const int64_t units = ((n + TL_ROWS - 1) / TL_ROWS + TL_WARPS - 1) / TL_WARPS;
#define B200Q_TW(NK, NF, G_, FL) do { auto k_ = agg_tile_wide_kernel<NK, NF, G_, FL>; k_<<<tile_grid(k_, units), TL_BLOCK, 0, s>>>(cols, ts, lay, tab, row_begin, n); } while (0)
#define B200Q_TW_FL(NK, NF, G_) do { if (ts.flavour == TF_ADD_U64) B200Q_TW(NK, NF, G_, TF_ADD_U64); else if (ts.flavour == TF_ADD_F64) B200Q_TW(NK, NF, G_, TF_ADD_F64); else B200Q_TW(NK, NF, G_, TF_MIN_S64); } while (0)
#define B200Q_TW_G(NK, NF) do { if (ts.G == 2) B200Q_TW_FL(NK, NF, 2); else if (ts.G == 4) B200Q_TW_FL(NK, NF, 4); else B200Q_TW_FL(NK, NF, 8); } while (0)
#define B200Q_TW_NF(NK) do { if (ts.nfcol == 0) B200Q_TW_G(NK, 0); else if (ts.nfcol == 1) B200Q_TW_G(NK, 1); else B200Q_TW_G(NK, 2); } while (0)
  if (ts.nkeys == 1) B200Q_TW_NF(1); else B200Q_TW_NF(2);
#undef B200Q_TW_NF
#undef B200Q_TW_G
#undef B200Q_TW_FL
#undef B200Q_TW
  return 1;
}

__global__ void __launch_bounds__(256) tile_wide_fill_kernel(unsigned long long* tab, unsigned long long nwords, unsigned long long v) {
  for (unsigned long long i = blockIdx.x * (unsigned long long)blockDim.x + threadIdx.x; i < nwords; i += (unsigned long long)gridDim.x * blockDim.x) tab[i] = v;
}
int launch_tile_wide_init(const TileAggSpec& ts, cudaStream_t s) {
  const unsigned long long nwords = ts.dense_cap * (unsigned long long)ts.G;
  tile_wide_fill_kernel<<<tile_grid(tile_wide_fill_kernel, (int64_t)((nwords + 8191) / 8192)), 256, 0, s>>>(ts.dense_tab, nwords, tile_identity(ts.flavour));
  return 1;
}
__device__ __forceinline__ bool tw_marked(const TileAggSpec& ts, unsigned long long w) {
  return ts.flavour == TF_MIN_S64 ? w == 0 : ts.flavour == TF_ADD_F64 ? as_f64(w) != 0.0 : w != 0;
}
__device__ __forceinline__ bool tw_present(const TileAggSpec& ts, const unsigned long long* e) { return tw_marked(ts, e[ts.presence_word]); }
__global__ void __launch_bounds__(256) tile_wide_count_kernel(const TileAggSpec ts, unsigned long long* out) {
  unsigned long long c = 0;
  for (uint64_t i = blockIdx.x * (uint64_t)blockDim.x + threadIdx.x; i < ts.dense_cap; i += (uint64_t)gridDim.x * blockDim.x) c += tw_present(ts, ts.dense_tab + i * ts.G);
#pragma unroll
  for (int d = 16; d > 0; d >>= 1) c += __shfl_xor_sync(0xffffffffu, c, d);
  if ((threadIdx.x & 31) == 0 && c) atomicAdd(out, c);
}
int launch_tile_wide_count(const TileAggSpec& ts, unsigned long long* d_out, cudaStream_t s) {
  tile_wide_count_kernel<<<tile_grid(tile_wide_count_kernel, ((int64_t)ts.dense_cap + 16383) / 16384), 256, 0, s>>>(ts, d_out);
  return 1;
}
__global__ void __launch_bounds__(256) tile_wide_normalise_kernel(const TileAggSpec ts) {
  for (uint64_t i = blockIdx.x * (uint64_t)blockDim.x + threadIdx.x; i < ts.dense_cap; i += (uint64_t)gridDim.x * blockDim.x) {
    unsigned long long* e = ts.dense_tab + i * ts.G + ts.dec_word;
    unsigned long long w0 = e[0], w1 = e[1], w2 = e[2];
    w1 += w0 >> 32; w0 &= 0xFFFFFFFFULL; w2 += w1 >> 32; w1 &= 0xFFFFFFFFULL;
    e[0] = w0; e[1] = w1; e[2] = w2;
  }
}
int launch_tile_wide_normalise(const TileAggSpec& ts, cudaStream_t s) {
  if (ts.dec_word == 0xFF) return 0;
  tile_wide_normalise_kernel<<<tile_grid(tile_wide_normalise_kernel, ((int64_t)ts.dense_cap + 16383) / 16384), 256, 0, s>>>(ts);
  return 1;
}
__global__ void __launch_bounds__(256) tile_wide_emit_kernel(const TileAggSpec ts, const AggLayout lay, const EmitTable emit, unsigned long long* out_count) {
  const unsigned lane = threadIdx.x & 31;
  const uint64_t stride = (uint64_t)gridDim.x * blockDim.x;
  const uint64_t rounds = (ts.dense_cap + stride - 1) / stride;
  for (uint64_t it = 0; it < rounds; it++) {
    const uint64_t i = it * stride + blockIdx.x * (uint64_t)blockDim.x + threadIdx.x;
    const unsigned long long* e = ts.dense_tab + i * ts.G;
    const bool occ = i < ts.dense_cap && tw_present(ts, e);
    const unsigned m = __ballot_sync(0xffffffffu, occ);
    if (!m) continue;
    unsigned long long base = 0;
    if (lane == 0) base = atomicAdd(out_count, (unsigned long long)__popc(m));
    base = __shfl_sync(0xffffffffu, base, 0);
    if (!occ) continue;
    const unsigned long long at = base + __popc(m & lanemask_lt());
    unsigned long long ke[4] = {0, 0, 0, 0}, slot[16];
    ke[lay.key_word[0]] = (unsigned long long)(ts.nkeys == 1 ? ts.dense_base + (long long)i : ts.dense_base + (long long)(i / ts.dense_r1));
    if (ts.nkeys == 2) ke[lay.key_word[1]] = (unsigned long long)(ts.dense_base1 + (long long)(i % ts.dense_r1));
#pragma unroll
    for (int w = 0; w < 16; w++) slot[w] = 0;
    unsigned flags = 0;
    for (int a = 0; a < ts.nacc; a++) {
      const AccOp op = lay.acc[ts.acc[a].lay_acc];
      const unsigned long long d = e[ts.acc[a].w0];
      switch (ts.acc[a].recon) {
        case TR_COPY: slot[op.word] = d; break;
        case TR_NOT: slot[op.word] = ~d; break;
        case TR_F2I: slot[op.word] = (unsigned long long)__double2ll_rn(as_f64(d)); break;
        default: {
          const unsigned long long w0 = d, w1 = e[ts.acc[a].w0 + 1], w2 = e[ts.acc[a].w0 + 2];
          const unsigned long long c1 = w1 + (w0 >> 32);
          slot[op.word] = (w0 & 0xFFFFFFFFULL) | (c1 << 32); slot[op.word + 1] = w2 + (c1 >> 32);
          break;
        }
      }
      const uint8_t vw = ts.acc[a].valid_word;
      const bool valid = vw == 0xFF ? true : tw_marked(ts, e[vw]);
      if (op.vbit != 0xFF && valid) flags |= 1u << op.vbit;
    }
    emit_row_columns(emit, at, ke, slot, flags);
  }
}
int launch_tile_wide_emit(const TileAggSpec& ts, const AggLayout& lay, const EmitTable& emit, unsigned long long* d_out_count, cudaStream_t s) {
  tile_wide_emit_kernel<<<tile_grid(tile_wide_emit_kernel, ((int64_t)ts.dense_cap + 16383) / 16384), 256, 0, s>>>(ts, lay, emit, d_out_count);
  return 1;
}

}
```

blaze_b200/csrc/runtime.h:

```cpp
#pragma once
#include <cuda_runtime.h>

#include <algorithm>
#include <deque>
#include <functional>
#include <memory>
#include <string>
#include <vector>

#include "../../include/blaze_b200.h"
#include "compile.h"
#include "ir.h"
#include "kernels.cuh"

namespace b200q {

struct CudaError : std::runtime_error {
  CudaError(const std::string& m) : std::runtime_error(m) {}
};
struct ExecError : std::runtime_error {
  int code;
  ExecError(int c, const std::string& m) : std::runtime_error(m), code(c) {}
};

#define B200Q_CUDA(expr)                                                                                      \
  do {                                                                                                        \
    cudaError_t _e = (expr);                                                                                  \
    if (_e != cudaSuccess) throw ::b200q::CudaError(std::string(#expr) + ": " + cudaGetErrorString(_e));      \
  } while (0)

struct StreamRef {
  cudaStream_t s = nullptr; int device = 0;
  ~StreamRef();
};
std::shared_ptr<StreamRef> stream_ref_create(int device);
std::shared_ptr<StreamRef> stream_ref_lookup(cudaStream_t s);

struct DevMem {
  void* ptr = nullptr;
  size_t bytes = 0;
  cudaStream_t stream = nullptr;
  bool owned = false;
  std::shared_ptr<void> owner;
  std::shared_ptr<StreamRef> stream_keep;
  ~DevMem();
  static std::shared_ptr<DevMem> alloc(size_t bytes, cudaStream_t s, bool zero = false);
  static std::shared_ptr<DevMem> borrow(const void* p, size_t bytes, std::shared_ptr<void> owner);
};
using DevMemP = std::shared_ptr<DevMem>;

struct DevColumn {
  DType type;
  DevMemP values;
  DevMemP validity;
  DevMemP offsets;
  int64_t offset = 0;
};

struct DevBatch {
  std::vector<DevColumn> cols;
  int64_t num_rows = 0;
};

struct Metrics {
  int64_t input_rows = 0, input_batches = 0, output_rows = 0, output_batches = 0;
  int64_t launches = 0, fast_launches = 0, h2d_bytes = 0, d2h_bytes = 0;
  int64_t num_groups = 0, table_capacity = 0, grow_count = 0;
  double gpu_ms = 0;
  double hot_ms = 0; int64_t hot_rows = 0, hot_launches = 0;
};

struct OpContext {
  int device = 0;
  cudaStream_t stream = nullptr;
  b200q_conf conf;
  Metrics m;
  cudaEvent_t ev0 = nullptr, ev1 = nullptr;
  int cur_stage = 0;
};

class Stage {
 public:
  virtual ~Stage() {}
  SchemaDef in_schema, out_schema;
  std::vector<int> used_input_cols;
  virtual void push(OpContext& cx, DevBatch& in, std::vector<DevBatch>& outs) = 0;
  virtual void finish(OpContext& cx, std::vector<DevBatch>& outs) = 0;
};

std::unique_ptr<Stage> make_filter_project_stage(OpContext& cx, const SchemaDef& in_schema, const std::vector<ExprP>& filters,
                                                 const std::vector<ExprP>& outs, const SchemaDef& out_schema);
std::unique_ptr<Stage> make_expand_stage(OpContext& cx, const SchemaDef& in_schema, const std::vector<ExprP>& filters,
                                         const std::vector<std::vector<ExprP>>& projections, const SchemaDef& out_schema);
struct AggSetExprs { std::vector<ExprP> group_exprs; std::vector<std::vector<ExprP>> agg_args; };
std::unique_ptr<Stage> make_agg_stage(OpContext& cx, const SchemaDef& in_schema, const std::vector<ExprP>& filters, const PlanNode& agg,
                                      const std::vector<ExprP>& group_exprs, const std::vector<std::vector<ExprP>>& agg_args,
                                      const std::vector<AggSetExprs>& sets = {});

std::unique_ptr<Stage> make_bloom_agg_stage(OpContext& cx, const SchemaDef& in_schema, const PlanNode& agg, const std::vector<int>& value_cols);

std::unique_ptr<Stage> make_shuffle_write_stage(OpContext& cx, const SchemaDef& in_schema, const PlanNode& node);
struct ShuffleResult {
  virtual ~ShuffleResult() {}
  virtual int64_t chunk_count() const = 0;
  virtual void chunk(int64_t i, b200q_shuffle_chunk* out) const = 0;
};

void run_parquet_scan(OpContext& cx, const PlanNode& leaf, const std::function<void(DevBatch&)>& emit);
void set_file_reader(b200q_file_reader_fn fn, void* ctx);
void* pinned_alloc(size_t n);
void pinned_free(void* p);

class IpcSource {
 public:
  virtual ~IpcSource() {}
  virtual void push(OpContext& cx, const uint8_t* data, size_t len, const std::function<void(DevBatch&)>& emit) = 0;
  virtual void flush(OpContext& cx, const std::function<void(DevBatch&)>& emit) = 0;
};
std::unique_ptr<IpcSource> make_ipc_source(OpContext& cx, const SchemaDef& schema, const std::vector<int>& used_cols);

std::unique_ptr<Stage> make_sort_stage(OpContext& cx, const SchemaDef& in_schema, const PlanNode& node);

struct WindowCols { std::vector<int> partition_cols, order_cols; std::vector<std::vector<int>> agg_args; size_t n_fwd = 0; };
std::unique_ptr<Stage> make_window_stage(OpContext& cx, const SchemaDef& in_schema, const PlanNode& node, const WindowCols& cols);

struct JoinBuilt;
std::unique_ptr<Stage> make_join_build_stage(OpContext& cx, const SchemaDef& in_schema, const PlanNode& node);
std::unique_ptr<Stage> make_join_probe_stage(OpContext& cx, const SchemaDef& in_schema, const PlanNode& node);
struct GatherSrc { DType type; const void* values; const uint8_t* vbits; uint32_t bit_offset; const uint8_t* vbytes; bool may_be_null; };
std::vector<DevColumn> gather_columns(OpContext& cx, const std::vector<GatherSrc>& srcs, const uint32_t* idx, int64_t n);
struct JoinBuildResult { virtual ~JoinBuildResult() {} virtual std::shared_ptr<JoinBuilt> built() const = 0; };
struct JoinProbeAttach { virtual ~JoinProbeAttach() {} virtual void attach(std::shared_ptr<JoinBuilt> b) = 0; };

std::unique_ptr<Stage> make_smj_stage(OpContext& cx, const SchemaDef& in_schema, const PlanNode& node);
struct SmjRightAttach {
  virtual ~SmjRightAttach() {}
  virtual bool right_attached() const = 0;
  virtual void attach_right(OpContext& cx, const std::vector<DevBatch>& batches, const SchemaDef& schema) = 0;
};

DevCol dev_col_of(const DevColumn& c);

inline size_t bitmap_bytes(int64_t n) { return (size_t)((n + 31) / 32) * 4; }
DevMemP pack_bits(OpContext& cx, const void* bytes, int64_t n);
struct ByteCols { int64_t rows = 0; std::vector<DevMemP> values, valid; };
ByteCols to_byte_cols(OpContext& cx, const SchemaDef& schema, const std::vector<const DevBatch*>& parts);
ByteCols concat(OpContext& cx, const SchemaDef& schema, std::vector<ByteCols>&& parts);
std::vector<DevColumn> null_columns(OpContext& cx, const SchemaDef& schema, int64_t n);
void add_kernel_time(OpContext& cx, int64_t rows, bool hot);
inline bool kept_alive(const DevMemP& m) { return !m || m->owned || m->owner; }
inline bool forwardable(const DevColumn& c) { return c.offset == 0 && kept_alive(c.values) && kept_alive(c.validity) && kept_alive(c.offsets); }
template <class F> void for_each_window(const DevBatch& in, int64_t rows, F&& f) {
  for (int64_t r0 = 0; r0 < in.num_rows; r0 += rows) {
    DevBatch part; part.num_rows = std::min(rows, in.num_rows - r0);
    for (auto& c : in.cols) { DevColumn p = c; p.offset = c.offset + r0; part.cols.push_back(p); }
    f(part);
  }
}
inline GatherSrc gather_src_of(const DevColumn& c, bool nil_possible) {
  return GatherSrc{c.type, (const uint8_t*)c.values->ptr + (size_t)c.offset * c.type.byte_width(), c.validity ? (const uint8_t*)c.validity->ptr : nullptr,
                   (uint32_t)c.offset, nullptr, nil_possible || (bool)c.validity};
}

DType type_of_format(const char* arrow_format);
void export_device(DevBatch& db, int device, ArrowDeviceArray* out);
b200q_status fail(int code, const std::string& msg);
b200q_status guarded_call(const std::function<void()>& f);

struct StateCols { std::vector<FieldDef> fields; std::vector<uint8_t> frozen; };
StateCols state_columns_of(const AggDef& a);

}
```

blaze_b200/csrc/stages.cu:

```cuda
#include <algorithm>
#include <chrono>
#include <cstdlib>
#include <cstring>
#include <mutex>
#include <unordered_map>

#include "runtime.h"
#include "kernels_fast.cuh"
#include "kernels_join.cuh"

namespace b200q {

static std::mutex g_stream_mu;
static std::unordered_map<cudaStream_t, std::weak_ptr<StreamRef>> g_streams;

StreamRef::~StreamRef() {
  { std::lock_guard<std::mutex> l(g_stream_mu); g_streams.erase(s); }
  if (s) { cudaSetDevice(device); cudaStreamSynchronize(s); cudaStreamDestroy(s); }
}
std::shared_ptr<StreamRef> stream_ref_create(int device) {
  auto r = std::make_shared<StreamRef>(); r->device = device;
  B200Q_CUDA(cudaStreamCreateWithFlags(&r->s, cudaStreamNonBlocking));
  std::lock_guard<std::mutex> l(g_stream_mu); g_streams[r->s] = r;
  return r;
}
std::shared_ptr<StreamRef> stream_ref_lookup(cudaStream_t s) {
  std::lock_guard<std::mutex> l(g_stream_mu);
  auto it = g_streams.find(s);
  return it == g_streams.end() ? nullptr : it->second.lock();
}

DevMem::~DevMem() {
  if (owned && ptr) {
    if (stream_keep) { cudaSetDevice(stream_keep->device); cudaFreeAsync(ptr, stream_keep->s); }
    else cudaFree(ptr);
  }
}
DevMemP DevMem::alloc(size_t bytes, cudaStream_t s, bool zero) {
  auto m = std::make_shared<DevMem>();
  m->bytes = bytes; m->stream = s; m->owned = true; m->stream_keep = stream_ref_lookup(s);
  if (bytes == 0) bytes = 16;
  {
    const cudaError_t e = cudaMallocAsync(&m->ptr, bytes, s);
    if (e == cudaErrorMemoryAllocation) {
      cudaGetLastError(); m->ptr = nullptr; m->owned = false;
      throw ExecError(B200Q_ERR_UNSUPPORTED, "out of HBM: a device allocation of " + std::to_string(bytes) + " bytes failed; this task must fall back to the host path");
    }
    B200Q_CUDA(e);
  }
  if (zero) B200Q_CUDA(cudaMemsetAsync(m->ptr, 0, bytes, s));
  return m;
}
DevMemP DevMem::borrow(const void* p, size_t bytes, std::shared_ptr<void> owner) {
  auto m = std::make_shared<DevMem>();
  m->ptr = const_cast<void*>(p); m->bytes = bytes; m->owned = false; m->owner = std::move(owner);
  return m;
}

DevCol dev_col_of(const DevColumn& c) {
  DevCol d{};
  const int w = c.type.byte_width();
  d.values = c.values ? (const uint8_t*)c.values->ptr + (size_t)c.offset * (size_t)w : nullptr;
  if (c.type.is_varlen()) d.offsets = c.offsets ? (const int32_t*)c.offsets->ptr + c.offset : nullptr;
  d.validity = c.validity ? (const uint8_t*)c.validity->ptr : nullptr;
  d.bit_offset = (uint32_t)c.offset;
  if (c.offset > 0xFFFFFFFFLL) throw ExecError(B200Q_ERR_UNSUPPORTED, "column offset beyond 2^32 rows");
  return d;
}

DevMemP pack_bits(OpContext& cx, const void* bytes, int64_t n) {
  DevMemP bits = DevMem::alloc(bitmap_bytes(n), cx.stream);
  cx.m.launches += launch_pack_valid((const uint8_t*)bytes, (uint32_t*)bits->ptr, n, cx.stream);
  return bits;
}

ByteCols to_byte_cols(OpContext& cx, const SchemaDef& schema, const std::vector<const DevBatch*>& parts) {
  ByteCols out;
  for (auto* p : parts) out.rows += p->num_rows;
  for (size_t c = 0; c < schema.fields.size(); c++) {
    const size_t w = (size_t)schema.fields[c].type.byte_width();
    DevMemP v = DevMem::alloc((size_t)out.rows * w + 16, cx.stream), vb;
    bool any = false; for (auto* p : parts) any = any || p->cols[c].validity;
    if (any) vb = DevMem::alloc((size_t)out.rows + 16, cx.stream);
    int64_t at = 0;
    for (auto* p : parts) {
      const DevColumn& dc = p->cols[c];
      B200Q_CUDA(cudaMemcpyAsync((uint8_t*)v->ptr + (size_t)at * w, (const uint8_t*)dc.values->ptr + (size_t)dc.offset * w, (size_t)p->num_rows * w, cudaMemcpyDeviceToDevice, cx.stream));
      if (dc.validity) cx.m.launches += launch_unpack_bits((const uint8_t*)dc.validity->ptr, (uint32_t)dc.offset, p->num_rows, (uint8_t*)vb->ptr + at, cx.stream);
      else if (vb) B200Q_CUDA(cudaMemsetAsync((uint8_t*)vb->ptr + at, 1, (size_t)p->num_rows, cx.stream));
      at += p->num_rows;
    }
    out.values.push_back(v); out.valid.push_back(vb);
  }
  return out;
}

ByteCols concat(OpContext& cx, const SchemaDef& schema, std::vector<ByteCols>&& parts) {
  const std::vector<ByteCols> ps = std::move(parts);
  ByteCols out;
  for (auto& p : ps) out.rows += p.rows;
  for (size_t c = 0; c < schema.fields.size(); c++) {
    const size_t w = (size_t)schema.fields[c].type.byte_width();
    DevMemP v = DevMem::alloc((size_t)out.rows * w + 16, cx.stream), vb;
    bool any = false; for (auto& p : ps) any = any || p.valid[c];
    if (any) vb = DevMem::alloc((size_t)out.rows + 16, cx.stream);
    int64_t at = 0;
    for (auto& p : ps) {
      B200Q_CUDA(cudaMemcpyAsync((uint8_t*)v->ptr + (size_t)at * w, p.values[c]->ptr, (size_t)p.rows * w, cudaMemcpyDeviceToDevice, cx.stream));
      if (p.valid[c]) B200Q_CUDA(cudaMemcpyAsync((uint8_t*)vb->ptr + at, p.valid[c]->ptr, (size_t)p.rows, cudaMemcpyDeviceToDevice, cx.stream));
      else if (vb) B200Q_CUDA(cudaMemsetAsync((uint8_t*)vb->ptr + at, 1, (size_t)p.rows, cx.stream));
      at += p.rows;
    }
    out.values.push_back(v); out.valid.push_back(vb);
  }
  return out;
}

std::vector<DevColumn> null_columns(OpContext& cx, const SchemaDef& schema, int64_t n) {
  std::vector<DevColumn> out;
  for (auto& f : schema.fields) {
    DevColumn o; o.type = f.type;
    o.values = DevMem::alloc((size_t)n * f.type.byte_width() + 16, cx.stream, true); o.validity = DevMem::alloc(bitmap_bytes(n), cx.stream, true);
    out.push_back(o);
  }
  return out;
}

void add_kernel_time(OpContext& cx, int64_t rows, bool hot) {
  float ms = 0; B200Q_CUDA(cudaEventElapsedTime(&ms, cx.ev0, cx.ev1));
  cx.m.gpu_ms += ms;
  if (hot) { cx.m.hot_ms += ms; cx.m.hot_rows += rows; cx.m.hot_launches++; }
}

static DevMemP upload_program(const CompiledProgram& cp, cudaStream_t s, std::vector<DevMemP>& blooms) {
  DevMemP d = DevMem::alloc(sizeof(VmProgram), s);
  VmProgram p = relocated_program(cp, d->ptr);
  for (const auto& b : cp.blooms) {
    const size_t bytes = b.filter->words.size() * 8;
    DevMemP w = DevMem::alloc(bytes, s);
    B200Q_CUDA(cudaMemcpyAsync(w->ptr, b.filter->words.data(), bytes, cudaMemcpyHostToDevice, s));
    p.pool[b.pool_index] = (uint64_t)(uintptr_t)w->ptr;
    blooms.push_back(w);
  }
  B200Q_CUDA(cudaMemcpyAsync(d->ptr, &p, sizeof(VmProgram), cudaMemcpyHostToDevice, s));
  B200Q_CUDA(cudaStreamSynchronize(s));
  return d;
}

static void check_device_error_flags(int flags) {
  if (flags & 1) throw ExecError(B200Q_ERR_EXECUTION, "Arrow error: Divide by zero error");
  if (flags & 2) throw ExecError(B200Q_ERR_EXECUTION, "Arrow error: Arithmetic overflow");
  if (flags & 4) throw ExecError(B200Q_ERR_EXECUTION, "corrupted accumulator row in the Binary agg buffer column");
}

class FilterProjectStage : public Stage {
  CompiledProgram cp_;
  DevMemP d_prog_;
  std::vector<DevMemP> d_blooms_;
  bool has_filters_;
  bool identity_ = false;
  bool lean_possible_ = false;
  LeanFpSpec lean_{};
  std::vector<int> out_src_, vm_out_;
  bool varlen_ = false;
  int sel_out_ = -1;

  int slot_of(int col_index) const { for (size_t i = 0; i < cp_.used_cols.size(); i++) if (cp_.used_cols[i] == col_index) return (int)i; return -1; }
  static bool is_i64(const DType& t) { return t.id == T_INT64 || t.id == T_TIMESTAMP_US; }

  void detect_lean(const std::vector<ExprP>& filters, const std::vector<ExprP>& outs) {
    lean_possible_ = false;
    if (filters.size() > 4 || outs.size() > 8 || outs.empty() || cp_.used_cols.empty() || cp_.used_cols.size() > 4) return;
    LeanFpSpec sp{}; sp.nfilt = (int)filters.size(); sp.nout = (int)outs.size();
    for (size_t f = 0; f < filters.size(); f++) {
      const ExprP& p = filters[f];
      if (p->kind != E_BINARY || p->op < OP_EQ || p->op > OP_GE) return;
      ExprP l = p->children[0], r = p->children[1]; int op = p->op - OP_EQ;
      if (l->kind == E_LITERAL && r->kind == E_COLUMN) { std::swap(l, r); static const int flip[] = {CMP_EQ, CMP_NE, CMP_GT, CMP_GE, CMP_LT, CMP_LE}; op = flip[op]; }
      if (l->kind != E_COLUMN || r->kind != E_LITERAL || r->lit_null || !is_i64(l->type) || !is_i64(r->type)) return;
      const int s = slot_of(l->col_index); if (s < 0 || s > 127) return;
      sp.filt[f].col = (int8_t)s; sp.filt[f].op = (uint8_t)op; sp.filt[f].lit = (long long)r->lit_lo;
    }
    for (size_t o = 0; o < outs.size(); o++) {
      const ExprP& e = outs[o];
      if (!is_i64(e->type)) return;
      if (e->kind == E_COLUMN) { const int s = slot_of(e->col_index); if (s < 0 || s > 127) return; sp.out[o].kind = 0; sp.out[o].a = (int8_t)s; sp.out[o].b = -1; continue; }
      if (e->kind != E_BINARY || (e->op != OP_PLUS && e->op != OP_MINUS && e->op != OP_MUL)) return;
      const ExprP &l = e->children[0], &r = e->children[1];
      if (l->kind != E_COLUMN || !is_i64(l->type)) return;
      const int sa = slot_of(l->col_index); if (sa < 0 || sa > 127) return;
      sp.out[o].kind = (uint8_t)(e->op == OP_PLUS ? 1 : e->op == OP_MINUS ? 2 : 3); sp.out[o].a = (int8_t)sa;
      if (r->kind == E_COLUMN && is_i64(r->type)) { const int sb = slot_of(r->col_index); if (sb < 0 || sb > 127) return; sp.out[o].b = (int8_t)sb; }
      else if (r->kind == E_LITERAL && !r->lit_null && is_i64(r->type)) { sp.out[o].b = -1; sp.out[o].lit = (long long)r->lit_lo; }
      else return;
    }
    lean_ = sp; lean_possible_ = true;
  }

 public:
  FilterProjectStage(OpContext& cx, const SchemaDef& in, const std::vector<ExprP>& filters, const std::vector<ExprP>& outs, const SchemaDef& out) {
    in_schema = in; out_schema = out;
    has_filters_ = !filters.empty();
    identity_ = !has_filters_ && outs.size() == in.fields.size();
    for (size_t i = 0; identity_ && i < outs.size(); i++) identity_ = outs[i]->kind == E_COLUMN && outs[i]->col_index == (int)i && outs[i]->type == in.fields[i].type;
    std::vector<ExprP> vm_outs;
    for (const ExprP& o : outs) {
      ExprP e = o;
      while ((e->kind == E_TRY_CAST || e->kind == E_CAST) && e->children[0]->type == e->type) e = e->children[0];
      if (!e->type.is_varlen()) { out_src_.push_back(-1); vm_out_.push_back((int)vm_outs.size()); vm_outs.push_back(o); continue; }
      if (e->kind != E_COLUMN)
        throw PlanError(B200Q_ERR_UNSUPPORTED, "ProjectExec: " + explain_expr(o) + " produces a " + e->type.str() + " value; only " + e->type.str() + " column references are on the hot path");
      out_src_.push_back(e->col_index); vm_out_.push_back(-1);
    }
    varlen_ = vm_outs.size() != outs.size();
    if (varlen_ && has_filters_) sel_out_ = (int)vm_outs.size();
    cp_ = compile_program(filters, vm_outs, has_filters_, sel_out_);
    used_input_cols = cp_.used_cols;
    for (int c : out_src_) if (c >= 0 && std::find(used_input_cols.begin(), used_input_cols.end(), c) == used_input_cols.end()) used_input_cols.push_back(c);
    if (!cx.conf.force_generic_kernels && !varlen_ && !cp_.has_strings && !cp_.vm_only) detect_lean(filters, outs);
    d_prog_ = upload_program(cp_, cx.stream, d_blooms_);
  }

  void push(OpContext& cx, DevBatch& in, std::vector<DevBatch>& outs) override {
    const int64_t n = in.num_rows;
    if (n == 0) return;
    if (n > 0x7FFFFFFFLL) throw ExecError(B200Q_ERR_UNSUPPORTED, "batches above 2^31-1 rows must be split by the caller");
    if (identity_ && std::all_of(in.cols.begin(), in.cols.end(), forwardable)) { outs.push_back(in); return; }
    ColTable ct{};
    for (size_t i = 0; i < cp_.used_cols.size(); i++) ct.col[i] = dev_col_of(in.cols[cp_.used_cols[i]]);
    OutTable ot{};
    DevBatch ob;
    for (size_t i = 0; i < cp_.outs.size(); i++) {
      const OutDesc& od = cp_.outs[i];
      DevColumn c; c.type = od.type;
      const bool is_bool = od.type.id == T_BOOL;
      c.values = is_bool ? DevMem::alloc(bitmap_bytes(n), cx.stream, true) : DevMem::alloc((size_t)n * od.type.byte_width(), cx.stream);
      if (od.nullable) c.validity = DevMem::alloc(bitmap_bytes(n), cx.stream, true);
      ot.values[i] = c.values->ptr; ot.validity[i] = c.validity ? (uint32_t*)c.validity->ptr : nullptr; ot.phys[i] = phys_of(od.type);
      ob.cols.push_back(c);
    }
    DevMemP sel;
    if (sel_out_ >= 0) { sel = DevMem::alloc((size_t)n * 4, cx.stream); ot.values[sel_out_] = sel->ptr; ot.validity[sel_out_] = nullptr; ot.phys[sel_out_] = PH_SEL; }
    bool lean = lean_possible_;
    for (size_t i = 0; lean && i < cp_.used_cols.size(); i++) lean = ct.col[i].validity == nullptr;
    DevMemP scratch = DevMem::alloc(32, cx.stream, true);
    DevMemP status;
    B200Q_CUDA(cudaEventRecord(cx.ev0, cx.stream));
    if (lean) {
      for (auto& c : ob.cols) if (c.validity) B200Q_CUDA(cudaMemsetAsync(c.validity->ptr, 0xFF, c.validity->bytes, cx.stream));
      if (has_filters_) status = DevMem::alloc((size_t)filter_project_lean_scratch_bytes(n), cx.stream, true);
      long long* outp[8]; for (size_t i = 0; i < cp_.outs.size(); i++) outp[i] = (long long*)ot.values[i];
      cx.m.launches += launch_filter_project_lean(ct, (int)cp_.used_cols.size(), lean_, outp, n, status ? status->ptr : nullptr, (unsigned long long*)scratch->ptr, cx.stream);
      cx.m.fast_launches++;
    } else {
      if (has_filters_) status = DevMem::alloc((size_t)filter_project_num_tiles(n) * 8, cx.stream, true);
      cx.m.launches += launch_filter_project((const VmProgram*)d_prog_->ptr, ct, ot, (int)cp_.outs.size(), n, has_filters_,
                                             status ? (unsigned long long*)status->ptr : nullptr, (unsigned long long*)scratch->ptr, cx.stream);
    }
    B200Q_CUDA(cudaEventRecord(cx.ev1, cx.stream));
    B200Q_CUDA(cudaGetLastError());
    unsigned long long h[4];
    B200Q_CUDA(cudaMemcpyAsync(h, scratch->ptr, 32, cudaMemcpyDeviceToHost, cx.stream));
    B200Q_CUDA(cudaStreamSynchronize(cx.stream));
    add_kernel_time(cx, n, cx.cur_stage == 0);
    check_device_error_flags((int)h[2]);
    ob.num_rows = (int64_t)h[1];
    if (ob.num_rows == 0) return;
    if (!varlen_) { outs.push_back(std::move(ob)); return; }
    DevBatch res; res.num_rows = ob.num_rows;
    for (size_t i = 0; i < out_src_.size(); i++) res.cols.push_back(out_src_[i] < 0 ? ob.cols[(size_t)vm_out_[i]] : DevColumn());
    gather_varlen(cx, in, sel ? (const uint32_t*)sel->ptr : nullptr, res);
    outs.push_back(std::move(res));
  }

  void gather_varlen(OpContext& cx, const DevBatch& in, const uint32_t* sel, DevBatch& res) {
    const int64_t m = res.num_rows;
    struct Job { size_t out; DevCol src; };
    std::vector<Job> jobs;
    for (size_t i = 0; i < out_src_.size(); i++) {
      if (out_src_[i] < 0) continue;
      const DevColumn& c = in.cols[(size_t)out_src_[i]];
      if (!sel && forwardable(c)) { res.cols[i] = c; continue; }
      jobs.push_back(Job{i, dev_col_of(c)});
    }
    if (jobs.empty()) return;
    const size_t nj = jobs.size();
    DevMemP totals = DevMem::alloc(nj * 8, cx.stream, true);
    std::vector<DevMemP> keep;
    for (size_t j = 0; j < nj; j++) {
      DevColumn& o = res.cols[jobs[j].out];
      const DevColumn& c = in.cols[(size_t)out_src_[jobs[j].out]];
      o.type = c.type;
      o.offsets = DevMem::alloc((size_t)(m + 1) * 4, cx.stream);
      if (c.validity && out_schema.fields[jobs[j].out].nullable) o.validity = DevMem::alloc(bitmap_bytes(m), cx.stream);
      DevMemP lengths = DevMem::alloc((size_t)m * 4 + 16, cx.stream), sums = DevMem::alloc((size_t)scan_num_blocks(m) * 4 + 16, cx.stream);
      cx.m.launches += launch_varlen_lengths(jobs[j].src, sel, m, (int32_t*)lengths->ptr, o.validity ? (uint32_t*)o.validity->ptr : nullptr,
                                             (unsigned long long*)totals->ptr + j, cx.stream);
      cx.m.launches += launch_exclusive_scan_i32((const int32_t*)lengths->ptr, (int32_t*)o.offsets->ptr, m, (int32_t*)sums->ptr, cx.stream);
      keep.push_back(lengths); keep.push_back(sums);
    }
    std::vector<unsigned long long> bytes(nj);
    B200Q_CUDA(cudaMemcpyAsync(bytes.data(), totals->ptr, nj * 8, cudaMemcpyDeviceToHost, cx.stream));
    B200Q_CUDA(cudaStreamSynchronize(cx.stream));
    for (size_t j = 0; j < nj; j++) {
      DevColumn& o = res.cols[jobs[j].out];
      if (bytes[j] > 0x7FFFFFFFULL) throw ExecError(B200Q_ERR_UNSUPPORTED, "a " + o.type.str() + " output column of one batch exceeds 2 GiB (32-bit Arrow offsets); push smaller batches");
      o.values = DevMem::alloc((size_t)bytes[j], cx.stream);
      cx.m.launches += launch_varlen_copy(jobs[j].src, sel, m, (const int32_t*)o.offsets->ptr, (uint8_t*)o.values->ptr, cx.stream);
    }
    B200Q_CUDA(cudaGetLastError());
  }
  void finish(OpContext&, std::vector<DevBatch>&) override {}
};

std::unique_ptr<Stage> make_filter_project_stage(OpContext& cx, const SchemaDef& in_schema, const std::vector<ExprP>& filters,
                                                 const std::vector<ExprP>& outs, const SchemaDef& out_schema) {
  return std::unique_ptr<Stage>(new FilterProjectStage(cx, in_schema, filters, outs, out_schema));
}

class ExpandStage : public Stage {
  std::vector<std::unique_ptr<FilterProjectStage>> sets_;
 public:
  ExpandStage(OpContext& cx, const SchemaDef& in, const std::vector<ExprP>& filters, const std::vector<std::vector<ExprP>>& projections, const SchemaDef& out) {
    in_schema = in; out_schema = out;
    for (auto& p : projections) {
      sets_.emplace_back(new FilterProjectStage(cx, in, filters, p, out));
      for (int c : sets_.back()->used_input_cols) if (std::find(used_input_cols.begin(), used_input_cols.end(), c) == used_input_cols.end()) used_input_cols.push_back(c);
    }
    std::sort(used_input_cols.begin(), used_input_cols.end());
  }
  void push(OpContext& cx, DevBatch& in, std::vector<DevBatch>& outs) override { for (auto& s : sets_) s->push(cx, in, outs); }
  void finish(OpContext&, std::vector<DevBatch>&) override {}
};

std::unique_ptr<Stage> make_expand_stage(OpContext& cx, const SchemaDef& in_schema, const std::vector<ExprP>& filters,
                                         const std::vector<std::vector<ExprP>>& projections, const SchemaDef& out_schema) {
  return std::unique_ptr<Stage>(new ExpandStage(cx, in_schema, filters, projections, out_schema));
}

static uint64_t host_mix64(uint64_t x) { x ^= x >> 33; x *= 0xff51afd7ed558ccdULL; x ^= x >> 33; x *= 0xc4ceb9fe1a85ec53ULL; x ^= x >> 33; return x; }

StateCols state_columns_of(const AggDef& a) {
  StateCols s; DType i64; i64.id = T_INT64;
  const uint8_t value_kind = a.data_type.id == T_BOOL ? FZ_BOOL : FZ_PRIM;
  switch (a.fn) {
    case AGG_COUNT: s.fields.push_back(FieldDef{a.field_name, i64, false}); s.frozen = {FZ_COUNT}; break;
    case AGG_AVG:
      s.fields.push_back(FieldDef{a.field_name + "#sum", a.data_type, true});
      s.fields.push_back(FieldDef{a.field_name + "#count", i64, false});
      s.frozen = {FZ_PRIM, FZ_COUNT};
      break;
    case AGG_FIRST: {
      DType i8; i8.id = T_INT8;
      s.fields.push_back(FieldDef{a.field_name, a.data_type, true});
      s.fields.push_back(FieldDef{a.field_name + "#flag", i8, false});
      s.frozen = {value_kind, FZ_BOOL};
      break;
    }
    default: s.fields.push_back(FieldDef{a.field_name, a.data_type, true}); s.frozen = {value_kind}; break;
  }
  return s;
}

static bool cast_may_fail(const DType& f, const DType& t) {
  if (f == t) return false;
  auto ii = [](const DType& d) { return d.is_integer() || d.id == T_DATE32 || d.id == T_TIMESTAMP_US || d.id == T_BOOL; };
  if (ii(f) && ii(t)) return t.int_bits() < f.int_bits();
  if (ii(f) && t.is_float()) return false;
  if (f.is_float() && (t.is_float() || t.is_integer() || t.id == T_BOOL)) return false;
  return true;
}
static bool can_be_null(const ExprP& e) {
  switch (e->kind) {
// ... 214 lines not shown
        std::vector<int> args;
        bool value_nullable = true;
        std::vector<int> set_o(nsets_, -1);
        if (partial && !multi) { args.push_back(add_out(agg_args[ai][0])); value_nullable = can_be_null(agg_args[ai][0]); }
        else if (partial) {
          value_nullable = false;
          for (int s = 0; s < nsets_; s++) {
            const ExprP& e = sets[s].agg_args[ai][0];
            if (is_null_literal(e)) { value_nullable = true; continue; }
            set_o[s] = add_out(e); value_nullable = value_nullable || can_be_null(e);
          }
          int o = 0; for (int s = nsets_ - 1; s >= 0; s--) if (set_o[s] >= 0) o = set_o[s];
          args.push_back(o);
        } else {
          args.push_back(add_out(state_col_expr(sc.fields[0])));
          if (!ign) {
            const ExprP flag = state_col_expr(sc.fields[1]);
            if (first_flag_out < 0) first_flag_out = add_out(flag);
            args.push_back(first_flag_out);
          }
        }
        const uint8_t vbit = (!ign && value_nullable) ? new_vbit() : (uint8_t)0xFF;
        const int nwords = dt.is_decimal() ? 2 : 1;
        const int vw = add_acc(ign ? ACC_FIRST_VALID : ACC_FIRST, nwords, vbit, args, 0, 0);
        AccOp& op = lay_.acc[lay_.nacc - 1];
        op.nwords = (uint8_t)nwords;
        int ow;
        if (!ign) { if (first_oword[partial] < 0) first_oword[partial] = new_oword(); ow = first_oword[partial]; }
        else ow = new_oword();
        op.oword = (uint8_t)ow;
        for (int s = 0; multi && s < nsets_; s++) {
          if (set_o[s] >= 0) sets_[s].acc_arg[lay_.nacc - 1][0] = (uint8_t)set_o[s];
          else if (ign) sets_[s].acc_skip |= 1u << (lay_.nacc - 1);
        }
        auto first_spec = [&](const FieldDef& f, EmitKind kind) {
          EmitSpec es{}; es.ec.kind = kind; es.ec.phys = phys_of(f.type); es.ec.word = (uint8_t)vw; es.ec.word2 = (uint8_t)ow; es.ec.vbit = vbit; es.field = f; return es;
        };
        if (final_) emit_.push_back(first_spec(agg.schema.fields[lay_.nkeys + ai], EMIT_FIRST_VALUE));
        else {
          emit_.push_back(first_spec(sc.fields[0], EMIT_FIRST_VALUE)); emit_.back().frozen_bool = sc.frozen[0] == FZ_BOOL;
          if (!ign) { emit_.push_back(first_spec(sc.fields[1], EMIT_FIRST_FLAG)); emit_.back().frozen_bool = true; }
        }
        continue;
      }
      if (a.fn != AGG_COUNT) {
        ExprP arg;
        if (partial) { arg = agg_args[ai][0]; }
        else { arg = state_col_expr(state_columns_of(a).fields[0]); }
        std::vector<int> set_o(nsets_, -1);
        bool set_nullable = false;
        for (int s = 0; multi && s < nsets_; s++) {
          const ExprP& e = sets[s].agg_args[ai][0];
          if (is_null_literal(e)) { set_nullable = true; continue; }
          set_o[s] = add_out(e); set_nullable = set_nullable || can_be_null(e);
        }
        int o = 0;
        if (!multi) o = add_out(arg);
        else for (int s = nsets_ - 1; s >= 0; s--) if (set_o[s] >= 0) o = set_o[s];
        const bool nullable_arg = (multi ? set_nullable : can_be_null(arg)) || lay_.nkeys == 0;
        const uint8_t vbit = nullable_arg ? new_vbit() : (uint8_t)0xFF;
        AccKind kind; int nwords = 1; uint64_t ilo = 0, ihi = 0;
        if (a.fn == AGG_SUM || a.fn == AGG_AVG) {
          if (dt.is_decimal()) { kind = ACC_ADD_DEC; nwords = 2; }
          else if (dt.id == T_FLOAT64) { kind = ACC_ADD_F64; ilo = 0x8000000000000000ULL; }
          else if (dt.is_integer()) kind = ACC_ADD_I64;
          else throw PlanError(B200Q_ERR_UNSUPPORTED, "sum/avg accumulating at " + dt.str() + " is not on the hot path");
        } else {
          const bool mn = a.fn == AGG_MIN;
          if (dt.is_decimal()) { kind = mn ? ACC_MIN_DEC : ACC_MAX_DEC; nwords = 2; ilo = mn ? ~0ULL : 0ULL; ihi = mn ? 0x7FFFFFFFFFFFFFFFULL : 0x8000000000000000ULL; }
          else if (dt.is_float()) { kind = mn ? ACC_MIN_F64 : ACC_MAX_F64; ilo = mn ? 0x7FFFFFFFFFFFFFFFULL : 0x8000000000000000ULL; }
          else if (dt.is_intlike()) { kind = mn ? ACC_MIN_I64 : ACC_MAX_I64; ilo = mn ? 0x7FFFFFFFFFFFFFFFULL : 0x8000000000000000ULL; }
          else throw PlanError(B200Q_ERR_UNSUPPORTED, "min/max over " + dt.str() + " is not on the hot path");
        }
        sum_word = add_acc(kind, nwords, vbit, {o}, ilo, ihi); sum_vbit = vbit;
        for (int s = 0; multi && s < nsets_; s++) {
          if (set_o[s] < 0) sets_[s].acc_skip |= 1u << (lay_.nacc - 1);
          else sets_[s].acc_arg[lay_.nacc - 1][0] = (uint8_t)set_o[s];
        }
      }
      if (a.fn == AGG_COUNT || a.fn == AGG_AVG) {
        if (multi) {
          std::vector<std::vector<int>> set_args(nsets_);
          std::vector<bool> skip(nsets_, false);
          for (int s = 0; s < nsets_; s++) {
            const auto& srcs = a.fn == AGG_AVG ? std::vector<ExprP>{sets[s].agg_args[ai][0]} : sets[s].agg_args[ai];
            for (auto& e : srcs) {
              if (is_null_literal(e)) skip[s] = true;
              else if (can_be_null(e)) set_args[s].push_back(add_out(e));
            }
            if (set_args[s].size() > 4) throw PlanError(B200Q_ERR_UNSUPPORTED, "count over more than 4 nullable arguments");
          }
          cnt_word = add_acc(ACC_COUNT, 1, 0xFF, set_args[0], 0, 0);
          for (int s = 0; s < nsets_; s++) {
            if (skip[s]) { sets_[s].acc_skip |= 1u << (lay_.nacc - 1); continue; }
            for (size_t i = 0; i < set_args[s].size(); i++) sets_[s].acc_arg[lay_.nacc - 1][i] = (uint8_t)set_args[s][i];
          }
        } else if (partial) {
          std::vector<int> args;
          const auto& srcs = a.fn == AGG_AVG ? std::vector<ExprP>{agg_args[ai][0]} : agg_args[ai];
          for (auto& e : srcs) if (can_be_null(e)) args.push_back(add_out(e));
          if (args.size() > 4) throw PlanError(B200Q_ERR_UNSUPPORTED, "count over more than 4 nullable arguments");
          cnt_word = add_acc(ACC_COUNT, 1, 0xFF, args, 0, 0);
        } else {
          const auto sc = state_columns_of(a);
          const int o = add_out(state_col_expr(sc.fields.back()));
          cnt_word = add_acc(ACC_ADD_I64, 1, 0xFF, {o}, 0, 0);
        }
      }
      auto value_spec = [&](const FieldDef& f, int w, uint8_t vbit, bool order_key) {
        EmitSpec es{}; es.ec.kind = EMIT_ACC_VALUE; es.ec.phys = phys_of(f.type); es.ec.word = (uint8_t)w; es.ec.vbit = vbit; es.ec.is_order_key = order_key; es.field = f; return es;
      };
      const bool order_key = (a.fn == AGG_MIN || a.fn == AGG_MAX) && dt.is_float();
      if (final_) {
        const FieldDef& of = agg.schema.fields[lay_.nkeys + ai];
        if (a.fn == AGG_COUNT) emit_.push_back(value_spec(of, cnt_word, 0xFF, false));
        else if (a.fn == AGG_AVG) {
          EmitSpec es{}; es.field = of; es.ec.word = (uint8_t)sum_word; es.ec.word2 = (uint8_t)cnt_word; es.ec.vbit = sum_vbit;
          if (dt.is_decimal()) { es.ec.kind = EMIT_AVG_DEC; es.ec.phys = PH_DEC128; }
          else { es.ec.kind = EMIT_AVG_F64; es.ec.phys = PH_F64; es.ec.sum_is_f64 = dt.id == T_FLOAT64; }
          emit_.push_back(es);
        } else emit_.push_back(value_spec(of, sum_word, sum_vbit, order_key));
      } else {
        const auto sc = state_columns_of(a);
        if (a.fn == AGG_COUNT) { emit_.push_back(value_spec(sc.fields[0], cnt_word, 0xFF, false)); emit_.back().frozen_count = true; }
        else {
          emit_.push_back(value_spec(sc.fields[0], sum_word, sum_vbit, order_key));
          if (a.fn == AGG_AVG) { emit_.push_back(value_spec(sc.fields[1], cnt_word, 0xFF, false)); emit_.back().frozen_count = true; }
        }
      }
    }
    if (lay_.nkeys == 0 && lay_.nacc == 0) throw PlanError(B200Q_ERR_UNSUPPORTED, "aggregate without groupings and aggregates");
    auto stride_of = [](int words) { return words <= 1 ? 1 : words <= 2 ? 2 : words <= 4 ? 4 : (words + 3) & ~3; };
    lay_.kstride = std::max(2, stride_of(key_entry_words));
    lay_.astride = stride_of(std::max(word, 1));
    if (lay_.kstride > AGG_MAX_SLOT_WORDS || lay_.astride > AGG_MAX_SLOT_WORDS) throw PlanError(B200Q_ERR_UNSUPPORTED, "aggregate state too wide for one table slot");

    if (!final_ && columnar_) {
      out_schema.fields.resize(lay_.nkeys);
      for (size_t i = lay_.nkeys; i < emit_.size(); i++) out_schema.fields.push_back(emit_[i].field);
    }

    cp_ = compile_program(filters_, vm_outs_, false);
    lay_.nouts = (int)cp_.outs.size();
    int ow = 0;
    for (size_t i = 0; i < cp_.outs.size(); i++) { lay_.out_word[i] = (uint8_t)ow; ow += cp_.outs[i].slots; }
    if (ow > AGG_MAX_ROW_WORDS) {
      if (multi) throw PlanError(B200Q_ERR_UNSUPPORTED, "ExpandExec below AggExec: the grouping sets need " + std::to_string(ow) + " key/argument words per row, more than " + std::to_string(AGG_MAX_ROW_WORDS) + " (AGG_MAX_ROW_WORDS)");
      throw PlanError(B200Q_ERR_UNSUPPORTED, "too many key/argument words per row");
    }
    for (int c : cp_.used_cols) if (c < n_in_) used_input_cols.push_back(c);
    if (merge_mode_ && !columnar_) used_input_cols.push_back(n_in_ - 1);
    std::sort(used_input_cols.begin(), used_input_cols.end());
    used_input_cols.erase(std::unique(used_input_cols.begin(), used_input_cols.end()), used_input_cols.end());
    d_prog_ = upload_program(cp_, cx.stream, d_blooms_);
    if (multi) {
      d_sets_ = DevMem::alloc(sizeof(AggSetDesc) * sets_.size(), cx.stream);
      B200Q_CUDA(cudaMemcpyAsync(d_sets_->ptr, sets_.data(), sizeof(AggSetDesc) * sets_.size(), cudaMemcpyHostToDevice, cx.stream));
    }

    if (!cp_.has_strings && !cp_.vm_only && !multi) {
      detect_fast(cx);
      if (!fast_ok_) detect_wide(cx);
    }

    if (!final_) {
      for (size_t i = lay_.nkeys; i < emit_.size(); i++) {
        FrozenField f{}; const FieldDef& fd = emit_[i].field;
        f.kind = emit_[i].frozen_count ? FZ_COUNT : emit_[i].frozen_bool ? FZ_BOOL : FZ_PRIM; f.width = frozen_width(fd.type); f.phys = phys_of(fd.type);
        frozen_fields_.push_back(f);
      }
    }

    capacity_ = std::max<uint64_t>(1ULL << 20, (uint64_t)((double)std::max<int64_t>(cx.conf.agg_initial_groups, 1) * AGG_SLOTS_PER_GROUP));
    if (capacity_ >= (1ULL << 32)) throw PlanError(B200Q_ERR_UNSUPPORTED, "agg_initial_groups too large");
    alloc_table(cx, capacity_, keys_, accs_, counters_);
    if (lay_.nkeys == 0) seed_global_group(cx);
    B200Q_CUDA(cudaStreamSynchronize(cx.stream));
    cx.m.table_capacity = (int64_t)capacity_;
  }


  int prog_col_slot(int col_index) const {
    for (size_t i = 0; i < cp_.used_cols.size(); i++) if (cp_.used_cols[i] == col_index) return (int)i;
    return -1;
  }
  static bool int_phys(const DType& t) { return t.is_intlike(); }
  bool has_first() const { for (int j = 0; j < lay_.nacc; j++) if (acc_is_first(lay_.acc[j].kind)) return true; return false; }

  bool parse_keys_and_conjuncts(FastSpec& fs) const {
    if (lay_.nkeys < 1 || lay_.nkeys > 2 || filters_.size() > 4) return false;
    fs.nkeys = lay_.nkeys; fs.nfilt = (int)filters_.size();
    for (int k = 0; k < lay_.nkeys; k++) {
      const ExprP& e = vm_outs_[lay_.key_out[k]];
      if (e->kind != E_COLUMN || !int_phys(e->type) || lay_.key_nwords[k] != 1) return false;
      const int s = prog_col_slot(e->col_index); if (s < 0 || s > 127) return false;
      fs.key_col[k] = (int8_t)s; fs.key_phys[k] = phys_of(e->type);
    }
    for (size_t f = 0; f < filters_.size(); f++) {
      const ExprP& p = filters_[f];
      if (p->kind != E_BINARY || p->op < OP_EQ || p->op > OP_GE) return false;
      ExprP l = strip_noop_casts(p->children[0]), r = strip_noop_casts(p->children[1]);
      int op = p->op - OP_EQ;
      if (l->kind == E_LITERAL && r->kind == E_COLUMN) { std::swap(l, r); static const int flip[] = {CMP_EQ, CMP_NE, CMP_GT, CMP_GE, CMP_LT, CMP_LE}; op = flip[op]; }
      if (l->kind != E_COLUMN || r->kind != E_LITERAL || r->lit_null || !int_phys(l->type) || !int_phys(r->type)) return false;
      const int s = prog_col_slot(l->col_index); if (s < 0 || s > 127) return false;
      fs.filt[f].col = (int8_t)s; fs.filt[f].phys = phys_of(l->type); fs.filt[f].op = (uint8_t)op; fs.filt[f].lit = (long long)r->lit_lo;
    }
    merge_conjuncts(fs);
    return true;
  }

  void detect_fast(OpContext& cx) {
    fast_ok_ = false;
    if (cx.conf.force_generic_kernels || has_first()) return;
    if (lay_.nacc < 1 || lay_.nacc > 2) return;
    FastSpec fs{};
    if (!parse_keys_and_conjuncts(fs)) return;
    fs.nacc = lay_.nacc;
    for (int j = 0; j < lay_.nacc; j++) {
      const AccOp& a = lay_.acc[j];
      fs.acc[j].vbit = a.vbit; fs.acc[j].word = a.word; fs.acc[j].col = -1; fs.acc[j].phys = PH_I64;
      if (a.kind == ACC_ADD_I64) {
        const ExprP& e = vm_outs_[a.arg_out[0]];
        if (e->kind != E_COLUMN || !int_phys(e->type)) return;
        const int s = prog_col_slot(e->col_index); if (s < 0 || s > 127) return;
        fs.acc[j].kind = FAST_ACC_ADD; fs.acc[j].col = (int8_t)s; fs.acc[j].phys = phys_of(e->type);
        acc_arg_nullable_[j] = e->nullable;
      } else if (a.kind == ACC_COUNT && a.nargs <= 1) {
        fs.acc[j].kind = FAST_ACC_COUNT;
        if (a.nargs == 1) {
          const ExprP& e = vm_outs_[a.arg_out[0]];
          if (e->kind != E_COLUMN || !(e->type.is_intlike() || e->type.is_float() || e->type.is_decimal())) return;
          const int s = prog_col_slot(e->col_index); if (s < 0 || s > 127) return;
          fs.acc[j].col = (int8_t)s; fs.acc[j].phys = phys_of(e->type);
        }
      } else return;
    }
    if (lay_.nacc == 2 && lay_.acc[0].word / 4 != lay_.acc[1].word / 4) return;
    sink_ = DevMem::alloc((size_t)FAST_SINK_WARPS * 32, cx.stream, true);
    fs.sink = (unsigned long long*)sink_->ptr;
    fs_ = fs; fast_ok_ = true;
    dense_possible_ = cx.conf.agg_dense_keys != 0;
    if (dense_possible_) {
      for (size_t c = 0; c < emit_.size(); c++) {
        const EmitCol& ec = emit_[c].ec;
        if (ec.kind == EMIT_KEY) continue;
        bool found = false; for (int i = 0; i < lay_.nacc; i++) found |= fs_.acc[i].word == ec.word;
        if (ec.kind != EMIT_ACC_VALUE || ec.is_order_key || !found) { dense_possible_ = false; break; }
      }
    }
    if (dense_possible_) dense_possible_ = dense_layout();
  }

  static void merge_conjuncts(FastSpec& fs) {
    fs.nfcol = 0; fs.filt_never = 0;
    long long lo[2] = {INT64_MIN, INT64_MIN}, hi[2] = {INT64_MAX, INT64_MAX}; bool never = false;
    for (int f = 0; f < fs.nfilt; f++) {
      int c = -1;
      for (int i = 0; i < fs.nfcol; i++) if (fs.frange[i].col == fs.filt[f].col) c = i;
      if (c < 0) { if (fs.nfcol == 2) { fs.nfcol = -1; return; } c = fs.nfcol++; fs.frange[c].col = fs.filt[f].col; fs.frange[c].phys = fs.filt[f].phys; }
      const long long lit = fs.filt[f].lit;
      switch (fs.filt[f].op) {
        case CMP_EQ: lo[c] = std::max(lo[c], lit); hi[c] = std::min(hi[c], lit); break;
        case CMP_LT: if (lit == INT64_MIN) never = true; else hi[c] = std::min(hi[c], lit - 1); break;
        case CMP_LE: hi[c] = std::min(hi[c], lit); break;
        case CMP_GT: if (lit == INT64_MAX) never = true; else lo[c] = std::max(lo[c], lit + 1); break;
        case CMP_GE: lo[c] = std::max(lo[c], lit); break;
        default: fs.nfcol = -1; return;
      }
    }
    for (int c = 0; c < fs.nfcol; c++) {
      if (lo[c] > hi[c]) never = true;
      fs.frange[c].lo = lo[c]; fs.frange[c].span = (unsigned long long)hi[c] - (unsigned long long)lo[c];
    }
    fs.filt_never = never ? 1 : 0;
  }

  void detect_wide(OpContext& cx) {
    wide_possible_ = false;
    if (cx.conf.force_generic_kernels || !cx.conf.agg_dense_keys || has_first()) return;
    if (lay_.nacc < 1 || lay_.nacc > 4) return;
    TileAggSpec ts{};
    {
      FastSpec fs{};
      if (!parse_keys_and_conjuncts(fs) || fs.nfcol < 0) return;
      ts.nkeys = fs.nkeys; ts.nfcol = fs.nfcol; ts.filt_never = fs.filt_never;
      for (int k = 0; k < 2; k++) { ts.key_col[k] = fs.key_col[k]; ts.key_phys[k] = fs.key_phys[k]; ts.frange[k] = fs.frange[k]; }
    }
    ts.nacc = lay_.nacc; ts.dec_word = 0xFF;
    bool any_f64 = false, any_min = false, any_int = false;
    for (int j = 0; j < lay_.nacc; j++) {
      switch (lay_.acc[j].kind) {
        case ACC_ADD_F64: any_f64 = true; break;
        case ACC_MIN_I64: case ACC_MAX_I64: case ACC_MIN_F64: case ACC_MAX_F64: any_min = true; break;
        case ACC_ADD_I64: case ACC_ADD_DEC: any_int = true; break;
        case ACC_COUNT: break;
        default: return;
      }
    }
    if ((int)any_f64 + (int)any_min + (int)any_int > 1) return;
    ts.flavour = any_f64 ? TF_ADD_F64 : any_min ? TF_MIN_S64 : TF_ADD_U64;
    const unsigned long long ONE = ts.flavour == TF_ADD_F64 ? 0x3FF0000000000000ULL : ts.flavour == TF_MIN_S64 ? 0ULL : 1ULL;
    const unsigned long long NOOP = tile_identity(ts.flavour);
    struct ArgInfo { int col_index; int cvt; bool nullable; bool values; };
    std::vector<ArgInfo> args; std::vector<ExprP> arg_cols;
    unsigned long long dec_mul = 1; bool dec_mul_seen = false;
    auto arg_of = [&](const ExprP& e0, int want_cvt, bool values, bool dec) -> int {
      ExprP e = strip_noop_casts(e0); int cvt = TC_NONE;
      const bool nullable = can_be_null(e0);
      if ((e->kind == E_CAST || e->kind == E_TRY_CAST)) {
        const ExprP& c = e->children[0];
        if (c->kind == E_COLUMN && c->type.is_intlike() && e->type.id == T_FLOAT64) { cvt = TC_I2F; e = c; }
        else if (c->kind == E_COLUMN && c->type.is_decimal() && e->type.is_decimal() && e->type.scale >= c->type.scale && e->type.scale - c->type.scale <= 18 &&
                 (int)e->type.precision - (int)c->type.precision >= (int)e->type.scale - (int)c->type.scale) {
          unsigned long long mul = 1; for (int i = c->type.scale; i < e->type.scale; i++) mul *= 10ULL;
          if (dec_mul_seen && dec_mul != mul) return -1;
          dec_mul = mul; dec_mul_seen = true; e = c;
        }
        else return -1;
      }
      if (e->kind != E_COLUMN) return -1;
      if (!values) { for (size_t i = 0; i < args.size(); i++) if (args[i].col_index == e->col_index) { args[i].nullable = args[i].nullable || nullable; return (int)i; } }
      if (values) {
        if (dec) { if (!e->type.is_decimal()) return -1; }
        else if (want_cvt == TC_ORDER) { if (e->type.id != T_FLOAT64 || cvt != TC_NONE) return -1; cvt = TC_ORDER; }
        else if (ts.flavour == TF_ADD_F64) { if (!(e->type.id == T_FLOAT64 && cvt == TC_NONE) && cvt != TC_I2F) return -1; }
        else if (!e->type.is_intlike() || cvt != TC_NONE) return -1;
      }
      for (size_t i = 0; i < args.size(); i++)
        if (args[i].col_index == e->col_index && (!values || !args[i].values || args[i].cvt == cvt)) { args[i].nullable = args[i].nullable || nullable; if (values && !args[i].values) { args[i].values = true; args[i].cvt = cvt; } return (int)i; }
      if (args.size() == 2) return -1;
      args.push_back(ArgInfo{e->col_index, cvt, nullable, values}); arg_cols.push_back(e);
      return (int)args.size() - 1;
    };
    int acc_arg[4] = {-1, -1, -1, -1};
    for (int j = 0; j < lay_.nacc; j++) {
      const AccOp& a = lay_.acc[j];
      if (a.kind == ACC_COUNT) { if (a.nargs > 1) return; if (a.nargs == 1) { acc_arg[j] = arg_of(vm_outs_[a.arg_out[0]], TC_NONE, false, false); if (acc_arg[j] < 0) return; } continue; }
      const bool dec = a.kind == ACC_ADD_DEC, order = a.kind == ACC_MIN_F64 || a.kind == ACC_MAX_F64;
      acc_arg[j] = arg_of(vm_outs_[a.arg_out[0]], order ? TC_ORDER : TC_NONE, true, dec);
      if (acc_arg[j] < 0) return;
      if (dec) { if ((ts.arg_is_dec && acc_arg[j] != 0) || acc_arg[j] != 0) return; ts.arg_is_dec = 1; }
    }
    if (ts.arg_is_dec && args.size() > 1) return;
    ts.nargs = (int)args.size(); ts.dec_mul = dec_mul;
    for (size_t i = 0; i < args.size(); i++) {
      const int s = prog_col_slot(args[i].col_index); if (s < 0 || s > 127) return;
      const DType& t = arg_cols[i]->type;
      if (args[i].values && !ts.arg_is_dec && !(t.is_intlike() || t.id == T_FLOAT64)) return;
      ts.arg_col[i] = (int8_t)s; ts.arg_phys[i] = t.id == T_FLOAT64 ? (uint8_t)PH_I64 : phys_of(t); ts.arg_cvt[i] = (uint8_t)args[i].cvt; ts.arg_values[i] = args[i].values ? 1 : 0;
    }
    int w = 0;
    auto constant_word = [&](unsigned long long cst, int gate) { TileWord tw{}; tw.srcsel = 2; tw.gate = (uint8_t)gate; tw.cst = cst; return tw; };
    ts.presence_word = 0; ts.word[w++] = constant_word(ONE, 30);
    int valid_word[2] = {-1, -1};
    for (size_t i = 0; i < args.size(); i++) if (args[i].nullable) { valid_word[i] = w; ts.word[w++] = constant_word(ONE, 28 + (int)i); }
    for (int j = 0; j < lay_.nacc; j++) {
      const AccOp& a = lay_.acc[j]; const int arg = acc_arg[j];
      auto& out = ts.acc[j]; out.arg = (int8_t)arg; out.lay_acc = (uint8_t)j; out.valid_word = 0xFF; out.recon = TR_COPY;
      if (a.kind == ACC_COUNT) {
        if (ts.flavour == TF_MIN_S64) return;
        out.w0 = (uint8_t)(arg >= 0 && valid_word[arg] >= 0 ? valid_word[arg] : 0);
        out.recon = ts.flavour == TF_ADD_F64 ? TR_F2I : TR_COPY;
        continue;
      }
      if (a.vbit != 0xFF) { if (valid_word[arg] < 0) return; out.valid_word = (uint8_t)valid_word[arg]; }
      if (w + (a.kind == ACC_ADD_DEC ? 3 : 1) > 8) return;
      out.w0 = (uint8_t)w;
      TileWord tw{}; tw.srcsel = (uint8_t)arg; tw.gate = (uint8_t)(28 + arg); tw.msk = ~0ULL;
      if (a.kind == ACC_ADD_DEC) {
        ts.dec_word = (uint8_t)w; out.recon = TR_DEC3;
        TileWord lo = tw; lo.srcsel = 0; lo.msk = 0xFFFFFFFFULL; ts.word[w++] = lo;
        TileWord mid = lo; mid.sh = 32; ts.word[w++] = mid;
        TileWord hi = tw; hi.srcsel = 1; ts.word[w++] = hi;
      } else {
        if (a.kind == ACC_MAX_I64 || a.kind == ACC_MAX_F64) { tw.inv = ~0ULL; out.recon = TR_NOT; }
        ts.word[w++] = tw;
      }
    }
    if (w > 8) return;
    ts.G = w <= 2 ? 2 : w <= 4 ? 4 : 8;
    for (; w < ts.G; w++) ts.word[w] = constant_word(NOOP, 30);
    sink_ = DevMem::alloc((size_t)FAST_SINK_WARPS * 32, cx.stream);
    { std::vector<unsigned long long> fill((size_t)FAST_SINK_WARPS * 4, NOOP); B200Q_CUDA(cudaMemcpyAsync(sink_->ptr, fill.data(), fill.size() * 8, cudaMemcpyHostToDevice, cx.stream)); B200Q_CUDA(cudaStreamSynchronize(cx.stream)); }
    ts.sink = (unsigned long long*)sink_->ptr;
    ws_ = ts; wide_possible_ = true;
  }

  struct DenseRange { long long base[2] = {0, 0}; uint64_t span[2] = {1, 1}; uint64_t entries = 1; bool hot = false; };
  bool dense_range(OpContext& cx, const ColTable& ct, int64_t n, int nkeys, const int8_t* key_col, const uint8_t* key_phys, int entry_words,
                   bool probe_skew, DenseRange& dr) {
    const int64_t sample = std::min<int64_t>(n, 1 << 22);
    DevMemP d = DevMem::alloc(64, cx.stream);
    { const long long init[8] = {INT64_MAX, INT64_MIN, 0, INT64_MAX, INT64_MIN, 0, 0, 0};
      B200Q_CUDA(cudaMemcpyAsync(d->ptr, init, 64, cudaMemcpyHostToDevice, cx.stream)); }
    for (int k = 0; k < nkeys; k++) cx.m.launches += launch_key_range(ct.col[key_col[k]], key_phys[k], sample, (long long*)d->ptr + 3 * k, cx.stream);
    DevMemP hist;
    if (probe_skew) {
      hist = DevMem::alloc((65536 + 1) * 4, cx.stream, true);
      DevCol kc[2] = {ct.col[key_col[0]], ct.col[key_col[nkeys == 2 ? 1 : 0]]};
      cx.m.launches += launch_key_skew_probe(kc, key_phys, nkeys, sample, (unsigned*)hist->ptr, cx.stream);
    }
    long long hr[6] = {0}; unsigned mx = 0;
    B200Q_CUDA(cudaMemcpyAsync(hr, d->ptr, 48, cudaMemcpyDeviceToHost, cx.stream));
    if (probe_skew) B200Q_CUDA(cudaMemcpyAsync(&mx, (unsigned*)hist->ptr + 65536, 4, cudaMemcpyDeviceToHost, cx.stream));
    B200Q_CUDA(cudaStreamSynchronize(cx.stream));
    long long nonnull = 0;
    for (int k = 0; k < nkeys; k++) {
      const long long* h = hr + 3 * k;
      if (h[2] <= 0 || h[1] < h[0]) return false;
      const unsigned __int128 range = (unsigned __int128)((__int128)h[1] - (__int128)h[0]) + 1;
      if (range > ((uint64_t)1 << 26)) return false;
      const uint64_t r = (uint64_t)range, margin = r / 8 + std::min<uint64_t>(64, r / 2 + 1);
      dr.base[k] = h[0] > INT64_MIN + (long long)margin ? h[0] - (long long)margin : INT64_MIN;
      dr.span[k] = r + 2 * margin;
      nonnull = std::max(nonnull, h[2]);
    }
    const unsigned __int128 entries = (unsigned __int128)dr.span[0] * dr.span[1];
    const uint64_t budget = 8 * (uint64_t)std::max<int64_t>(std::max<int64_t>(nonnull, cx.conf.agg_initial_groups), 1 << 16);
    if (entries > budget || entries > ((uint64_t)1 << 26)) return false;
    if (cx.conf.agg_max_table_bytes > 0 && entries * entry_words * 8 > (unsigned __int128)cx.conf.agg_max_table_bytes) return false;
    dr.entries = (uint64_t)entries;
    dr.hot = probe_skew && dr.entries * entry_words > 4096 && (uint64_t)mx * 256 > (uint64_t)sample;
    return true;
  }

  void decide_wide(OpContext& cx, const ColTable& ct, int64_t n) {
    dense_decided_ = true;
    if (!wide_possible_ || n == 0) { wide_possible_ = false; return; }
    DenseRange dr;
    if (!dense_range(cx, ct, n, ws_.nkeys, ws_.key_col, ws_.key_phys, ws_.G, false, dr)) { wide_possible_ = false; return; }
    ws_.dense_base = dr.base[0]; ws_.dense_cap0 = dr.span[0]; ws_.dense_base1 = dr.base[1]; ws_.dense_r1 = dr.span[1]; ws_.dense_cap = dr.entries;
    dense_tab_ = DevMem::alloc((size_t)ws_.dense_cap * ws_.G * 8, cx.stream);
    ws_.dense_tab = (unsigned long long*)dense_tab_->ptr;
    cx.m.launches += launch_tile_wide_init(ws_, cx.stream);
  }

  bool dense_layout() {
    int star = -1;
    for (int j = 0; j < lay_.nacc; j++) if (fs_.acc[j].kind == FAST_ACC_COUNT && fs_.acc[j].col < 0) star = j;
    int word_of_acc[2] = {0, 0}, valid_word_of_acc[2] = {0xFF, 0xFF}, w = 0;
    for (int i = 0; i < 4; i++) fs_.dense_word_src[i] = -2;
    int8_t src[8]; for (int i = 0; i < 8; i++) src[i] = -2;
    if (star < 0) src[w++] = -1;
    for (int j = 0; j < lay_.nacc; j++) { word_of_acc[j] = w; src[w++] = (int8_t)j; }
    for (int j = 0; j < lay_.nacc; j++) {
      if (fs_.acc[j].kind != FAST_ACC_ADD || fs_.acc[j].vbit == 0xFF) continue;
      for (int i = 0; i < lay_.nacc; i++) if (i != j && fs_.acc[i].kind == FAST_ACC_COUNT && fs_.acc[i].col == fs_.acc[j].col) valid_word_of_acc[j] = word_of_acc[i];
      if (valid_word_of_acc[j] == 0xFF && !acc_arg_nullable_[j]) valid_word_of_acc[j] = star >= 0 ? word_of_acc[star] : 0;
      if (valid_word_of_acc[j] == 0xFF) { valid_word_of_acc[j] = w; src[w++] = (int8_t)(2 + j); }
    }
    if (w > 4) return false;
    fs_.dense_stride = w <= 2 ? 2 : 4;
    for (int i = 0; i < 4; i++) fs_.dense_word_src[i] = src[i];
    fs_.dense_presence_word = (uint8_t)(star >= 0 ? word_of_acc[star] : 0);
    for (size_t c = 0; c < emit_.size(); c++) {
      dmap_.word[c] = 0; dmap_.valid_word[c] = 0xFF;
      const EmitCol& ec = emit_[c].ec;
      if (ec.kind == EMIT_KEY) continue;
      int j = 0; for (int i = 0; i < lay_.nacc; i++) if (fs_.acc[i].word == ec.word) j = i;
      dmap_.word[c] = (uint8_t)word_of_acc[j];
      if (ec.vbit != 0xFF) dmap_.valid_word[c] = (uint8_t)valid_word_of_acc[j];
    }
    return true;
  }

  void decide_dense(OpContext& cx, const ColTable& ct, int64_t n) {
    dense_decided_ = true;
    if (!fast_ok_ || !dense_possible_ || n == 0) return;
    DenseRange dr;
    if (!dense_range(cx, ct, n, fs_.nkeys, fs_.key_col, fs_.key_phys, fs_.dense_stride, cx.conf.agg_hot_key_cache != 0, dr)) return;
    fs_.dense_base = dr.base[0]; fs_.dense_cap0 = dr.span[0];
    fs_.dense_base1 = dr.base[1]; fs_.dense_r1 = dr.span[1];
    fs_.dense_cap = dr.entries;
    fs_.dense_key0_minor = fs_.nkeys == 2 && dr.span[1] < dr.span[0];
    dense_tab_ = DevMem::alloc((size_t)fs_.dense_cap * fs_.dense_stride * 8, cx.stream, true);
    fs_.dense_tab = (unsigned long long*)dense_tab_->ptr;
    fs_.dense = 1;
    fs_.hot_cache = dr.hot ? 1 : 0;
  }

  bool lean_ok(const ColTable& ct, int64_t begin) const {
    if (begin % 4) return false;
    auto ok = [&](int slot, uint8_t phys) {
      const DevCol& c = ct.col[slot];
      return phys == PH_I64 && c.validity == nullptr && ((uintptr_t)c.values & 31) == 0;
    };
    for (int k = 0; k < fs_.nkeys; k++) if (!ok(fs_.key_col[k], fs_.key_phys[k])) return false;
    for (int j = 0; j < fs_.nacc; j++) {
      if (fs_.acc[j].col < 0) continue;
      if (fs_.acc[j].kind == FAST_ACC_ADD) { if (!ok(fs_.acc[j].col, fs_.acc[j].phys)) return false; }
      else if (ct.col[fs_.acc[j].col].validity != nullptr) return false;
    }
    for (int f = 0; f < fs_.nfilt; f++) if (!ok(fs_.filt[f].col, fs_.filt[f].phys)) return false;
    return true;
  }

  int launch_update(OpContext& cx, const ColTable& ct, const AggTable& t, int64_t begin, int64_t m, const uint32_t* list) {
    if (nsets_ > 1) return launch_agg_update_sets((const VmProgram*)d_prog_->ptr, ct, lay_, t, begin, m, list, (const AggSetDesc*)d_sets_->ptr, nsets_, rows_pushed_, cx.stream);
    if (wide_possible_ && ws_.dense_tab && !list) {
      cx.m.fast_launches++;
      if (ws_.dec_word != 0xFF) {
        if (wide_rows_since_norm_ + m > (1LL << 31)) { cx.m.launches += launch_tile_wide_normalise(ws_, cx.stream); wide_rows_since_norm_ = 0; }
        wide_rows_since_norm_ += m;
      }
      return launch_agg_tile_wide(ct, ws_, lay_, t, begin, m, cx.stream);
    }
    if (fast_ok_ && !list) {
      cx.m.fast_launches++;
      FastSpec fs = fs_;
      fs.lean = lean_ok(ct, begin) ? 1 : 0;
      return launch_agg_fast_update(ct, fs, lay_, t, begin, m, cx.stream);
    }
    return launch_agg_update((const VmProgram*)d_prog_->ptr, ct, lay_, t, begin, m, list, rows_pushed_, cx.stream);
  }

  void check_table_budget(OpContext& cx, unsigned __int128 bytes, const char* what) const {
    const int64_t budget = cx.conf.agg_max_table_bytes;
    if (budget > 0 && bytes > (unsigned __int128)budget)
      throw ExecError(B200Q_ERR_UNSUPPORTED, std::string("aggregate ") + what + " of " + std::to_string((unsigned long long)bytes) + " bytes exceeds the HBM budget (agg_max_table_bytes = " +
                                                 std::to_string(budget) + "): the table cannot spill on the GPU, fall back to the host path (agg_table.rs:540-588)");
  }
  void alloc_table(OpContext& cx, uint64_t cap, DevMemP& keys, DevMemP& accs, DevMemP& counters) {
    check_table_budget(cx, (unsigned __int128)cap * (lay_.kstride + lay_.astride) * 8, "hash table");
    keys = DevMem::alloc((size_t)cap * lay_.kstride * 8, cx.stream, true);
    accs = DevMem::alloc((size_t)cap * lay_.astride * 8, cx.stream);
    counters = DevMem::alloc(64, cx.stream, true);
  }

  void seed_global_group(OpContext& cx) {
    const uint64_t h = host_mix64(0x9E3779B97F4A7C15ULL);
    const uint64_t s = ((h >> 32) * (uint64_t)(uint32_t)capacity_) >> 32;
    const uint32_t tag2 = (uint32_t)h | 0x80000000u;
    std::vector<uint64_t> kimg(lay_.kstride, 0), aimg(lay_.astride, 0);
    for (int i = 0; i < lay_.astride; i++) aimg[i] = lay_.init[i];
    kimg[0] = (uint64_t)tag2 | ((uint64_t)lay_.init_flags << 32);
    B200Q_CUDA(cudaMemcpyAsync((uint8_t*)keys_->ptr + s * lay_.kstride * 8, kimg.data(), kimg.size() * 8, cudaMemcpyHostToDevice, cx.stream));
    B200Q_CUDA(cudaMemcpyAsync((uint8_t*)accs_->ptr + s * lay_.astride * 8, aimg.data(), aimg.size() * 8, cudaMemcpyHostToDevice, cx.stream));
    const unsigned long long one = 1;
    B200Q_CUDA(cudaMemcpyAsync(counters_->ptr, &one, 8, cudaMemcpyHostToDevice, cx.stream));
    B200Q_CUDA(cudaStreamSynchronize(cx.stream));
  }

  static constexpr double AGG_SLOTS_PER_GROUP = 3.0, AGG_LOAD_LIMIT = 0.5;
  static uint64_t load_limit(uint64_t cap) {
    const uint64_t lim = (uint64_t)((double)cap * AGG_LOAD_LIMIT);
    return cap > (1ULL << 19) ? std::min<uint64_t>(lim, cap - (1ULL << 19)) : lim;
  }

  AggTable table_view(int deferred_idx) const {
    AggTable t{};
    t.keys = (unsigned long long*)keys_->ptr; t.accs = (unsigned long long*)accs_->ptr; t.capacity = capacity_; t.max_groups = load_limit(capacity_);
    t.counters = (unsigned long long*)counters_->ptr;
    t.deferred = deferred_[deferred_idx] ? (uint32_t*)deferred_[deferred_idx]->ptr : nullptr;
    return t;
  }

  void grow(OpContext& cx, uint64_t min_groups) {
    uint64_t cap = capacity_;
    do cap <<= 1; while (load_limit(cap) < min_groups);
    if (cap >= (1ULL << 32)) throw ExecError(B200Q_ERR_UNSUPPORTED, "aggregate hash table beyond 2^32 slots");
    DevMemP nkeys, naccs, ncounters;
    alloc_table(cx, cap, nkeys, naccs, ncounters);
    AggTable oldt = table_view(0);
    AggTable newt{}; newt.keys = (unsigned long long*)nkeys->ptr; newt.accs = (unsigned long long*)naccs->ptr; newt.capacity = cap; newt.max_groups = load_limit(cap); newt.counters = (unsigned long long*)ncounters->ptr;
    cx.m.launches += launch_agg_rehash(lay_, oldt, newt, cx.stream);
    B200Q_CUDA(cudaGetLastError());
    keys_ = nkeys; accs_ = naccs; counters_ = ncounters; capacity_ = cap;
    cx.m.grow_count++; cx.m.table_capacity = (int64_t)cap;
  }

  void read_counters(OpContext& cx, unsigned long long (&h)[3]) {
    B200Q_CUDA(cudaMemcpyAsync(h, counters_->ptr, 24, cudaMemcpyDeviceToHost, cx.stream));
    B200Q_CUDA(cudaStreamSynchronize(cx.stream));
    check_device_error_flags((int)h[2]);
    ngroups_ = (int64_t)h[0];
    cx.m.num_groups = ngroups_;
  }

  struct Snap { unsigned long long* h = nullptr; cudaEvent_t ready = nullptr, k0 = nullptr, k1 = nullptr; };
  Snap snap_[2];
 public:
  ~AggStage() override { for (auto& s : snap_) { if (s.h) pinned_slots().put(s.h); if (s.ready) cudaEventDestroy(s.ready); if (s.k0) cudaEventDestroy(s.k0); if (s.k1) cudaEventDestroy(s.k1); } }
  void ensure_snaps() {
    if (snap_[0].h) return;
    for (auto& s : snap_) {
      s.h = pinned_slots().get();
      B200Q_CUDA(cudaEventCreateWithFlags(&s.ready, cudaEventDisableTiming)); B200Q_CUDA(cudaEventCreate(&s.k0)); B200Q_CUDA(cudaEventCreate(&s.k1));
    }
  }
  void account(OpContext& cx, const Snap& s, int64_t rows) {
    float ms = 0; B200Q_CUDA(cudaEventElapsedTime(&ms, s.k0, s.k1));
    cx.m.gpu_ms += ms; if (cx.cur_stage == 0) { cx.m.hot_ms += ms; cx.m.hot_rows += rows; cx.m.hot_launches++; }
  }
  void replay(OpContext& cx, const ColTable& ct, int64_t begin, const uint32_t* list, uint64_t ndef, bool grow_first) {
    if (!deferred_[1] || deferred_[1]->bytes < (size_t)deferred_cap_ * 4) deferred_[1] = DevMem::alloc((size_t)deferred_cap_ * 4, cx.stream);
    int wr = list == (const uint32_t*)deferred_[0]->ptr ? 1 : 0;
    while (ndef > 0) {
      if (grow_first) grow(cx, (uint64_t)ngroups_ + ndef);
      grow_first = true;
      B200Q_CUDA(cudaMemsetAsync((uint8_t*)counters_->ptr + 8, 0, 8, cx.stream));
      cx.m.launches += launch_update(cx, ct, table_view(wr), begin, (int64_t)ndef, list);
      B200Q_CUDA(cudaGetLastError());
      unsigned long long h[3];
      read_counters(cx, h);
      ndef = h[1]; list = (const uint32_t*)deferred_[wr]->ptr; wr ^= 1;
    }
  }

  void update_rows(OpContext& cx, const ColTable& ct, int64_t n) {
    int64_t chunk = std::max<int64_t>(1 << 16, std::min<int64_t>(cx.conf.max_launch_rows, 0x7FFFFFFFLL));
    if (nsets_ > 1) chunk = std::max<int64_t>(1 << 16, chunk / nsets_);
    static const bool dbg = getenv("B200Q_AGG_TIMING") != nullptr;
    auto hnow = [] { return std::chrono::duration<double, std::milli>(std::chrono::steady_clock::now().time_since_epoch()).count(); };
    const double tA = hnow();
    ensure_snaps();
    const double tB = hnow();
    const int64_t m_max = std::min(chunk, n);
    if (deferred_cap_ < 2 * m_max * nsets_) {
      deferred_cap_ = 2 * m_max * nsets_;
      deferred_[0] = DevMem::alloc((size_t)deferred_cap_ * 4, cx.stream);
      deferred_[1] = nullptr;
    }
    const double tC = hnow(); double t_launch = 0, t_settle = 0;
    int64_t prev_begin = 0, prev_m = 0; bool have_prev = false;
    int idx = 0;
    auto settle = [&](int pi, int64_t pb, int64_t pm, bool cur_in_flight, int64_t cb, int64_t cm) -> bool {
      Snap& sp = snap_[pi];
      B200Q_CUDA(cudaEventSynchronize(sp.ready));
      account(cx, sp, pm);
      check_device_error_flags((int)sp.h[2]);
      ngroups_ = (int64_t)sp.h[0]; cx.m.num_groups = ngroups_;
      const uint64_t d_prev = sp.h[1];
      if (d_prev == 0) return false;
      uint64_t d_cur = 0; DevMemP list_cur;
      if (cur_in_flight) {
        Snap& sc = snap_[pi ^ 1];
        B200Q_CUDA(cudaEventSynchronize(sc.ready));
        account(cx, sc, cm);
        check_device_error_flags((int)sc.h[2]);
        ngroups_ = (int64_t)sc.h[0]; cx.m.num_groups = ngroups_;
        d_cur = sc.h[1] - d_prev;
        if (d_cur) { list_cur = DevMem::alloc((size_t)d_cur * 4, cx.stream); B200Q_CUDA(cudaMemcpyAsync(list_cur->ptr, (const uint32_t*)deferred_[0]->ptr + d_prev, (size_t)d_cur * 4, cudaMemcpyDeviceToDevice, cx.stream)); }
      }
      replay(cx, ct, pb, (const uint32_t*)deferred_[0]->ptr, d_prev, true);
      if (d_cur) replay(cx, ct, cb, (const uint32_t*)list_cur->ptr, d_cur, false);
      return true;
    };
    for (int64_t begin = 0; begin < n; begin += chunk, idx++) {
      const int64_t m = std::min(chunk, n - begin);
      Snap& s = snap_[idx & 1];
      const double tl = hnow();
      B200Q_CUDA(cudaEventRecord(s.k0, cx.stream));
      cx.m.launches += launch_update(cx, ct, table_view(0), begin, m, nullptr);
      B200Q_CUDA(cudaEventRecord(s.k1, cx.stream));
      B200Q_CUDA(cudaGetLastError());
      B200Q_CUDA(cudaMemcpyAsync(s.h, counters_->ptr, 24, cudaMemcpyDeviceToHost, cx.stream));
      B200Q_CUDA(cudaEventRecord(s.ready, cx.stream));
      const double ts = hnow(); t_launch += ts - tl;
      const bool slow = have_prev && settle((idx & 1) ^ 1, prev_begin, prev_m, true, begin, m);
      t_settle += hnow() - ts;
      if (slow) { have_prev = false; continue; }
      prev_begin = begin; prev_m = m; have_prev = true;
    }
    const double tD = hnow();
    if (have_prev) settle((idx & 1) ^ 1, prev_begin, prev_m, false, 0, 0);
    if (dbg) fprintf(stderr, "update_rows: snaps %.3f ms, deferred buffers %.3f ms, launches %.3f ms, settles %.3f ms, last settle %.3f ms (%d chunks)\n", tB - tA, tC - tB, t_launch, t_settle, hnow() - tD, idx);
  }

  void push(OpContext& cx, DevBatch& in, std::vector<DevBatch>&) override {
    const int64_t n = in.num_rows;
    if (n == 0) return;
    ColTable ct{};
    std::vector<DevColumn> state_cols;
    if (merge_mode_ && !columnar_) unfreeze(cx, in, state_cols);
    for (size_t i = 0; i < cp_.used_cols.size(); i++) {
      const int c = cp_.used_cols[i];
      ct.col[i] = dev_col_of(c < n_in_ ? in.cols[c] : state_cols[c - n_in_]);
    }
    if (!dense_decided_) { if (wide_possible_) decide_wide(cx, ct, n); else decide_dense(cx, ct, n); }
    update_rows(cx, ct, n);
    rows_pushed_ += (uint64_t)n;
  }

  void unfreeze(OpContext& cx, DevBatch& in, std::vector<DevColumn>& state_cols) {
    const int64_t n = in.num_rows;
    const DevColumn& bc = in.cols.back();
    if (!bc.offsets || !bc.values) throw ExecError(B200Q_ERR_INVALID_ARG, "agg buffer column without offsets/data");
    FrozenTable ft{}; ft.nfields = (int)merge_state_fields_.size();
    if (ft.nfields > FROZEN_MAX_FIELDS) throw ExecError(B200Q_ERR_UNSUPPORTED, "too many accumulator fields");
    std::vector<DevMemP> valid_bytes(ft.nfields);
    std::vector<DevMemP> bool_bytes(ft.nfields);
    for (int k = 0; k < ft.nfields; k++) {
      const FieldDef& f = merge_state_fields_[k];
      DevColumn c; c.type = f.type;
      FrozenField& ff = ft.f[k];
      ff.kind = merge_state_kinds_[k]; ff.width = frozen_width(f.type); ff.phys = phys_of(f.type);
      if (f.type.id == T_BOOL) { bool_bytes[k] = DevMem::alloc((size_t)n, cx.stream); ff.values = bool_bytes[k]->ptr; }
      else { c.values = DevMem::alloc((size_t)n * f.type.byte_width(), cx.stream); ff.values = c.values->ptr; }
      if (f.nullable) { valid_bytes[k] = DevMem::alloc((size_t)n, cx.stream); ff.valid = (const uint8_t*)valid_bytes[k]->ptr; }
      state_cols.push_back(c);
    }
    int* d_err = (int*)((unsigned long long*)counters_->ptr + 2);
    cx.m.launches += launch_frozen_read(ft, n, (const int32_t*)bc.offsets->ptr, bc.offset, (const uint8_t*)bc.values->ptr, d_err, cx.stream);
    for (int k = 0; k < ft.nfields; k++) {
      if (valid_bytes[k]) state_cols[k].validity = pack_bits(cx, valid_bytes[k]->ptr, n);
      if (bool_bytes[k]) state_cols[k].values = pack_bits(cx, bool_bytes[k]->ptr, n);
    }
    B200Q_CUDA(cudaGetLastError());
  }

  void finish(OpContext& cx, std::vector<DevBatch>& outs) override {
    const bool wide = wide_possible_ && ws_.dense_tab;
    ensure_snaps();
    unsigned long long* hs = snap_[0].h;
    DevMemP dc;
    if (fs_.dense || wide) {
      dc = DevMem::alloc(8, cx.stream, true);
      if (wide) cx.m.launches += launch_tile_wide_normalise(ws_, cx.stream);
      cx.m.launches += fs_.dense ? launch_dense_count(fs_, (unsigned long long*)dc->ptr, cx.stream) : launch_tile_wide_count(ws_, (unsigned long long*)dc->ptr, cx.stream);
      B200Q_CUDA(cudaMemcpyAsync(hs + 3, dc->ptr, 8, cudaMemcpyDeviceToHost, cx.stream));
    } else hs[3] = 0;
    B200Q_CUDA(cudaMemcpyAsync(hs, counters_->ptr, 24, cudaMemcpyDeviceToHost, cx.stream));
    B200Q_CUDA(cudaStreamSynchronize(cx.stream));
    check_device_error_flags((int)hs[2]);
    ngroups_ = (int64_t)hs[0];
    const int64_t g = ngroups_ + (int64_t)hs[3];
    cx.m.num_groups = g;
    if (g == 0) return;
    EmitTable et{}; et.ncols = (int)emit_.size();
    if (et.ncols > EMIT_MAX_COLS) throw ExecError(B200Q_ERR_UNSUPPORTED, "too many output columns");
    DevBatch ob; ob.num_rows = g;
    std::vector<DevMemP> valid_bytes(emit_.size()), bool_bytes(emit_.size());
    for (size_t i = 0; i < emit_.size(); i++) {
      EmitCol ec = emit_[i].ec; const FieldDef& f = emit_[i].field;
      DevColumn c; c.type = f.type;
      if (f.type.id == T_BOOL) { bool_bytes[i] = DevMem::alloc((size_t)g, cx.stream); ec.values = bool_bytes[i]->ptr; }
      else { c.values = DevMem::alloc((size_t)g * f.type.byte_width(), cx.stream); ec.values = c.values->ptr; }
      if (f.nullable) { valid_bytes[i] = DevMem::alloc((size_t)g, cx.stream); ec.valid_bytes = (uint8_t*)valid_bytes[i]->ptr; }
      et.col[i] = ec;
      ob.cols.push_back(c);
    }
    DevMemP out_count = DevMem::alloc(8, cx.stream, true);
    cx.m.launches += launch_agg_emit(lay_, table_view(0), et, (unsigned long long*)out_count->ptr, cx.stream);
    if (fs_.dense) cx.m.launches += launch_agg_emit_dense(fs_, et, dmap_, (unsigned long long*)out_count->ptr, cx.stream);
    if (wide) cx.m.launches += launch_tile_wide_emit(ws_, lay_, et, (unsigned long long*)out_count->ptr, cx.stream);
    for (size_t i = 0; i < emit_.size(); i++) {
      if (valid_bytes[i]) ob.cols[i].validity = pack_bits(cx, valid_bytes[i]->ptr, g);
      if (bool_bytes[i]) ob.cols[i].values = pack_bits(cx, bool_bytes[i]->ptr, g);
    }
    B200Q_CUDA(cudaGetLastError());
    if (!final_ && !columnar_) {
      FrozenTable ft{}; ft.nfields = (int)frozen_fields_.size();
      for (int k = 0; k < ft.nfields; k++) {
        ft.f[k] = frozen_fields_[k];
        ft.f[k].values = bool_bytes[lay_.nkeys + k] ? bool_bytes[lay_.nkeys + k]->ptr : ob.cols[lay_.nkeys + k].values->ptr;
        ft.f[k].valid = valid_bytes[lay_.nkeys + k] ? (const uint8_t*)valid_bytes[lay_.nkeys + k]->ptr : nullptr;
      }
      DevMemP lengths = DevMem::alloc((size_t)g * 4, cx.stream);
      DevMemP offsets = DevMem::alloc((size_t)(g + 1) * 4, cx.stream);
      DevMemP block_sums = DevMem::alloc((size_t)scan_num_blocks(g) * 4 + 16, cx.stream);
      cx.m.launches += launch_frozen_lengths(ft, g, (int32_t*)lengths->ptr, cx.stream);
      cx.m.launches += launch_exclusive_scan_i32((const int32_t*)lengths->ptr, (int32_t*)offsets->ptr, g, (int32_t*)block_sums->ptr, cx.stream);
      int32_t total = 0;
      B200Q_CUDA(cudaMemcpyAsync(&total, (int32_t*)offsets->ptr + g, 4, cudaMemcpyDeviceToHost, cx.stream));
      B200Q_CUDA(cudaStreamSynchronize(cx.stream));
      if (total < 0) throw ExecError(B200Q_ERR_UNSUPPORTED, "frozen accumulator column exceeds 2 GiB; emit in smaller batches");
      DevMemP data = DevMem::alloc((size_t)total, cx.stream);
      cx.m.launches += launch_frozen_write(ft, g, (const int32_t*)offsets->ptr, (uint8_t*)data->ptr, cx.stream);
      B200Q_CUDA(cudaGetLastError());
      DevColumn bc; bc.type.id = T_BINARY; bc.values = data; bc.offsets = offsets;
      ob.cols.resize(lay_.nkeys);
      ob.cols.push_back(bc);
    }
    B200Q_CUDA(cudaStreamSynchronize(cx.stream));
    outs.push_back(std::move(ob));
  }
};

std::unique_ptr<Stage> make_agg_stage(OpContext& cx, const SchemaDef& in_schema, const std::vector<ExprP>& filters, const PlanNode& agg,
                                      const std::vector<ExprP>& group_exprs, const std::vector<std::vector<ExprP>>& agg_args,
                                      const std::vector<AggSetExprs>& sets) {
  return std::unique_ptr<Stage>(new AggStage(cx, in_schema, filters, agg, group_exprs, agg_args, sets));
}

}
```

Before: 84.56 billion.

## Remove host syncs, pool streams, defer table allocation, and fuse dense emit counting

Several unrelated changes aimed at host-side latency and small kernels. Idle CUDA streams are pooled and reused, program and sink uploads no longer block on a stream sync, and the hash table is allocated lazily (kept at the minimum size when a dense path is chosen). The separate dense-count and tile-wide-count kernels are dropped: output size is bounded upfront and the true count is read back after emit. Dense emit and key_range now reduce per block before issuing global atomics. The counter copy is replaced by a tiny snapshot kernel, and the skew probe is skipped when a filter column is present. Risks include over-allocating emit buffers to the bounded size and upload host buffers that live for the whole op.

```diff
diff --git a/blaze_b200/csrc/capi.cu b/blaze_b200/csrc/capi.cu
--- a/blaze_b200/csrc/capi.cu
+++ b/blaze_b200/csrc/capi.cu
@@ -677,7 +677,13 @@
           throw PlanError(B200Q_ERR_INVALID_ARG, "input_schema does not match the plan leaf: type of column " + std::to_string(i));
     }
   });
-  if (st != B200Q_OK) { if (op) { op->stages.clear(); delete op; } return st; }
+  if (st != B200Q_OK) {
+    if (op) {
+      if (op->cx.stream) cudaStreamSynchronize(op->cx.stream);
+      op->stages.clear(); delete op;
+    }
+    return st;
+  }
   *out = op;
   return B200Q_OK;
 }
@@ -850,7 +856,6 @@
   staging_free(op);
   if (op->cx.ev0) cudaEventDestroy(op->cx.ev0);
   if (op->cx.ev1) cudaEventDestroy(op->cx.ev1);
-  if (op->cx.stream) cudaStreamSynchronize(op->cx.stream);
   delete op;
 }
 
diff --git a/blaze_b200/csrc/kernels.cu b/blaze_b200/csrc/kernels.cu
--- a/blaze_b200/csrc/kernels.cu
+++ b/blaze_b200/csrc/kernels.cu
@@ -641,6 +641,14 @@
 int launch_agg_rehash(const AggLayout& lay, const AggTable& old_tab, const AggTable& new_tab, cudaStream_t s) {
   const int64_t cap = (int64_t)old_tab.capacity;
   agg_rehash_kernel<<<grid_for((cap + 255) / 256, 8), 256, 0, s>>>(lay, old_tab, new_tab);
+  return 1;
+}
+
+__global__ void agg_counters_snapshot_kernel(const unsigned long long* __restrict__ counters, unsigned long long* host_slot) {
+  if (threadIdx.x < 3) host_slot[threadIdx.x] = counters[threadIdx.x];
+}
+int launch_agg_counters_snapshot(const unsigned long long* counters, unsigned long long* host_slot, cudaStream_t s) {
+  agg_counters_snapshot_kernel<<<1, 32, 0, s>>>(counters, host_slot);
   return 1;
 }
 
diff --git a/blaze_b200/csrc/kernels.cuh b/blaze_b200/csrc/kernels.cuh
--- a/blaze_b200/csrc/kernels.cuh
+++ b/blaze_b200/csrc/kernels.cuh
@@ -117,6 +117,7 @@
                            const uint32_t* d_row_list, const AggSetDesc* d_sets, int nsets, uint64_t ord_base, cudaStream_t s);
 int launch_agg_rehash(const AggLayout& lay, const AggTable& old_tab, const AggTable& new_tab, cudaStream_t s);
 int launch_agg_emit(const AggLayout& lay, const AggTable& tab, const EmitTable& emit, unsigned long long* d_out_count, cudaStream_t s);
+int launch_agg_counters_snapshot(const unsigned long long* counters, unsigned long long* host_slot , cudaStream_t s);
 int launch_pack_valid(const uint8_t* bytes, uint32_t* bits, int64_t n, cudaStream_t s);
 int launch_frozen_lengths(const FrozenTable& ft, int64_t n, int32_t* lengths, cudaStream_t s);
 int launch_exclusive_scan_i32(const int32_t* in, int32_t* out , int64_t n, int32_t* d_block_sums, cudaStream_t s);
diff --git a/blaze_b200/csrc/kernels_fast.cu b/blaze_b200/csrc/kernels_fast.cu
--- a/blaze_b200/csrc/kernels_fast.cu
+++ b/blaze_b200/csrc/kernels_fast.cu
@@ -712,6 +712,8 @@
 }
 
 __global__ void __launch_bounds__(256) key_range_kernel(const DevCol col, int phys, long long n, long long* out ) {
+  __shared__ long long s_mn[8], s_mx[8];
+  __shared__ unsigned long long s_cnt[8];
   long long mn = INT64_MAX, mx = INT64_MIN; unsigned long long cnt = 0;
   for (long long i = blockIdx.x * (long long)blockDim.x + threadIdx.x; i < n; i += (long long)gridDim.x * blockDim.x) {
     if (!col_valid(col, i)) continue;
@@ -723,7 +725,13 @@
     const long long a = __shfl_xor_sync(0xffffffffu, mn, d), b = __shfl_xor_sync(0xffffffffu, mx, d);
     mn = a < mn ? a : mn; mx = b > mx ? b : mx; cnt += __shfl_xor_sync(0xffffffffu, cnt, d);
   }
-  if ((threadIdx.x & 31) == 0) { atomicMin(out, mn); atomicMax(out + 1, mx); atomicAdd((unsigned long long*)out + 2, cnt); }
+  const int warp = threadIdx.x >> 5, nwarps = blockDim.x >> 5;
+  if ((threadIdx.x & 31) == 0) { s_mn[warp] = mn; s_mx[warp] = mx; s_cnt[warp] = cnt; }
+  __syncthreads();
+  if (threadIdx.x == 0) {
+    for (int w = 1; w < nwarps; w++) { mn = s_mn[w] < mn ? s_mn[w] : mn; mx = s_mx[w] > mx ? s_mx[w] : mx; cnt += s_cnt[w]; }
+    if (cnt) { atomicMin(out, mn); atomicMax(out + 1, mx); atomicAdd((unsigned long long*)out + 2, cnt); }
+  }
 }
 int launch_key_skew_probe(const DevCol* key_cols, const uint8_t* phys, int nkeys, int64_t n, unsigned* d_hist, cudaStream_t s) {
   key_skew_hist_kernel<<<fast_grid((n + 2047) / 2048), 256, 0, s>>>(key_cols[0], key_cols[nkeys == 2 ? 1 : 0], phys[0], phys[nkeys == 2 ? 1 : 0], nkeys, n, d_hist);
@@ -746,34 +754,45 @@
   }
 }
 __global__ void __launch_bounds__(256) agg_emit_dense_kernel(const FastSpec fs, const EmitTable emit, const DenseEmitMap map, unsigned long long* out_count) {
-  const unsigned lane = threadIdx.x & 31;
+  __shared__ unsigned s_warp[8];
+  __shared__ unsigned long long s_base;
+  const unsigned lane = threadIdx.x & 31, warp = threadIdx.x >> 5;
   const uint64_t stride = (uint64_t)gridDim.x * blockDim.x;
   const uint64_t rounds = (fs.dense_cap + stride - 1) / stride;
   for (uint64_t it = 0; it < rounds; it++) {
     const uint64_t i = it * stride + blockIdx.x * (uint64_t)blockDim.x + threadIdx.x;
-    const uint64_t pe = fs.nkeys == 2 && fs.dense_key0_minor ? dense_entry2(fs, i / fs.dense_r1, i % fs.dense_r1) : i;
-    const unsigned long long* e = fs.dense_tab + pe * fs.dense_stride;
+    const unsigned long long* e = fs.dense_tab + i * fs.dense_stride;
     const bool occ = i < fs.dense_cap && e[fs.dense_presence_word] != 0;
     const unsigned m = __ballot_sync(0xffffffffu, occ);
-    if (!m) continue;
-    unsigned long long base = 0;
-    if (lane == 0) base = atomicAdd(out_count, (unsigned long long)__popc(m));
-    base = __shfl_sync(0xffffffffu, base, 0);
-    if (!occ) continue;
-    const unsigned long long at = base + __popc(m & lanemask_lt());
-    for (int c = 0; c < emit.ncols; c++) {
-      const EmitCol ec = emit.col[c];
-      if (ec.kind == EMIT_KEY) {
-        const long long kv = fs.nkeys == 1 ? fs.dense_base + (long long)i
-                           : ec.key == 0 ? fs.dense_base + (long long)(i / fs.dense_r1) : fs.dense_base1 + (long long)(i % fs.dense_r1);
-        dense_store(ec, at, (uint64_t)kv, true);
-      }
-      else {
-        const int w = map.word[c], vw = map.valid_word[c];
-        const bool valid = vw == 0xFF ? true : e[vw] != 0;
-        dense_store(ec, at, valid ? e[w] : 0, valid);
-      }
-    }
+    if (lane == 0) s_warp[warp] = __popc(m);
+    __syncthreads();
+    if (threadIdx.x == 0) {
+      unsigned tot = 0;
+      for (int w = 0; w < 8; w++) { const unsigned c = s_warp[w]; s_warp[w] = tot; tot += c; }
+      s_base = tot ? atomicAdd(out_count, (unsigned long long)tot) : 0;
+    }
+    __syncthreads();
+    if (occ) {
+      const unsigned long long at = s_base + s_warp[warp] + __popc(m & lanemask_lt());
+      uint64_t d0 = i, d1 = 0;
+      if (fs.nkeys == 2) {
+        if (fs.dense_key0_minor) { d0 = i % fs.dense_cap0; d1 = i / fs.dense_cap0; }
+        else { d0 = i / fs.dense_r1; d1 = i % fs.dense_r1; }
+      }
+      for (int c = 0; c < emit.ncols; c++) {
+        const EmitCol ec = emit.col[c];
+        if (ec.kind == EMIT_KEY) {
+          const long long kv = fs.nkeys == 2 && ec.key == 1 ? fs.dense_base1 + (long long)d1 : fs.dense_base + (long long)d0;
+          dense_store(ec, at, (uint64_t)kv, true);
+        }
+        else {
+          const int w = map.word[c], vw = map.valid_word[c];
+          const bool valid = vw == 0xFF ? true : e[vw] != 0;
+          dense_store(ec, at, valid ? e[w] : 0, valid);
+        }
+      }
+    }
+    __syncthreads();
   }
 }
 int launch_agg_emit_dense(const FastSpec& fs, const EmitTable& emit, const DenseEmitMap& map, unsigned long long* d_out_count, cudaStream_t s) {
@@ -781,17 +800,4 @@
   return 1;
 }
 
-__global__ void __launch_bounds__(256) dense_count_kernel(const FastSpec fs, unsigned long long* out) {
-  unsigned long long c = 0;
-  for (uint64_t i = blockIdx.x * (uint64_t)blockDim.x + threadIdx.x; i < fs.dense_cap; i += (uint64_t)gridDim.x * blockDim.x)
-    c += fs.dense_tab[i * fs.dense_stride + fs.dense_presence_word] != 0;
-#pragma unroll
-  for (int d = 16; d > 0; d >>= 1) c += __shfl_xor_sync(0xffffffffu, c, d);
-  if ((threadIdx.x & 31) == 0 && c) atomicAdd(out, c);
-}
-int launch_dense_count(const FastSpec& fs, unsigned long long* d_out, cudaStream_t s) {
-  dense_count_kernel<<<fast_grid(((int64_t)fs.dense_cap + 255) / 256), 256, 0, s>>>(fs, d_out);
-  return 1;
-}
-
-}
+}
diff --git a/blaze_b200/csrc/kernels_fast.cuh b/blaze_b200/csrc/kernels_fast.cuh
--- a/blaze_b200/csrc/kernels_fast.cuh
+++ b/blaze_b200/csrc/kernels_fast.cuh
@@ -79,7 +79,6 @@
 
 int launch_agg_tile_wide(const ColTable& cols, const TileAggSpec& ts, const AggLayout& lay, const AggTable& tab, int64_t row_begin, int64_t n, cudaStream_t s);
 int launch_tile_wide_init(const TileAggSpec& ts, cudaStream_t s);
-int launch_tile_wide_count(const TileAggSpec& ts, unsigned long long* d_out, cudaStream_t s);
 int launch_tile_wide_normalise(const TileAggSpec& ts, cudaStream_t s);
 int launch_tile_wide_emit(const TileAggSpec& ts, const AggLayout& lay, const EmitTable& emit, unsigned long long* d_out_count, cudaStream_t s);
 
@@ -88,6 +87,5 @@
 int launch_key_skew_probe(const DevCol* key_cols, const uint8_t* phys, int nkeys, int64_t n, unsigned* d_hist , cudaStream_t s);
 int launch_key_range(const DevCol& col, int phys, int64_t n, long long* d_out, cudaStream_t s);
 int launch_agg_emit_dense(const FastSpec& fs, const EmitTable& emit, const DenseEmitMap& map, unsigned long long* d_out_count, cudaStream_t s);
-int launch_dense_count(const FastSpec& fs, unsigned long long* d_out, cudaStream_t s);
 
 }
diff --git a/blaze_b200/csrc/kernels_tile.cu b/blaze_b200/csrc/kernels_tile.cu
--- a/blaze_b200/csrc/kernels_tile.cu
+++ b/blaze_b200/csrc/kernels_tile.cu
@@ -403,17 +403,6 @@
   return ts.flavour == TF_MIN_S64 ? w == 0 : ts.flavour == TF_ADD_F64 ? as_f64(w) != 0.0 : w != 0;
 }
 __device__ __forceinline__ bool tw_present(const TileAggSpec& ts, const unsigned long long* e) { return tw_marked(ts, e[ts.presence_word]); }
-__global__ void __launch_bounds__(256) tile_wide_count_kernel(const TileAggSpec ts, unsigned long long* out) {
-  unsigned long long c = 0;
-  for (uint64_t i = blockIdx.x * (uint64_t)blockDim.x + threadIdx.x; i < ts.dense_cap; i += (uint64_t)gridDim.x * blockDim.x) c += tw_present(ts, ts.dense_tab + i * ts.G);
-#pragma unroll
-  for (int d = 16; d > 0; d >>= 1) c += __shfl_xor_sync(0xffffffffu, c, d);
-  if ((threadIdx.x & 31) == 0 && c) atomicAdd(out, c);
-}
-int launch_tile_wide_count(const TileAggSpec& ts, unsigned long long* d_out, cudaStream_t s) {
-  tile_wide_count_kernel<<<tile_grid(tile_wide_count_kernel, ((int64_t)ts.dense_cap + 16383) / 16384), 256, 0, s>>>(ts, d_out);
-  return 1;
-}
 __global__ void __launch_bounds__(256) tile_wide_normalise_kernel(const TileAggSpec ts) {
   for (uint64_t i = blockIdx.x * (uint64_t)blockDim.x + threadIdx.x; i < ts.dense_cap; i += (uint64_t)gridDim.x * blockDim.x) {
     unsigned long long* e = ts.dense_tab + i * ts.G + ts.dec_word;
diff --git a/blaze_b200/csrc/runtime.h b/blaze_b200/csrc/runtime.h
--- a/blaze_b200/csrc/runtime.h
+++ b/blaze_b200/csrc/runtime.h
@@ -77,6 +77,7 @@
   Metrics m;
   cudaEvent_t ev0 = nullptr, ev1 = nullptr;
   int cur_stage = 0;
+  std::vector<std::shared_ptr<void>> upload_sources;
 };
 
 class Stage {
diff --git a/blaze_b200/csrc/stages.cu b/blaze_b200/csrc/stages.cu
--- a/blaze_b200/csrc/stages.cu
+++ b/blaze_b200/csrc/stages.cu
@@ -14,14 +14,24 @@
 static std::mutex g_stream_mu;
 static std::unordered_map<cudaStream_t, std::weak_ptr<StreamRef>> g_streams;
 
+static std::unordered_map<int, std::vector<cudaStream_t>> g_idle_streams;
+static constexpr size_t IDLE_STREAMS_PER_DEVICE = 16;
 StreamRef::~StreamRef() {
-  { std::lock_guard<std::mutex> l(g_stream_mu); g_streams.erase(s); }
-  if (s) { cudaSetDevice(device); cudaStreamSynchronize(s); cudaStreamDestroy(s); }
+  if (!s) return;
+  cudaSetDevice(device); cudaStreamSynchronize(s);
+  std::lock_guard<std::mutex> l(g_stream_mu);
+  g_streams.erase(s);
+  auto& idle = g_idle_streams[device];
+  if (idle.size() < IDLE_STREAMS_PER_DEVICE) idle.push_back(s);
+  else cudaStreamDestroy(s);
 }
 std::shared_ptr<StreamRef> stream_ref_create(int device) {
   auto r = std::make_shared<StreamRef>(); r->device = device;
-  B200Q_CUDA(cudaStreamCreateWithFlags(&r->s, cudaStreamNonBlocking));
-  std::lock_guard<std::mutex> l(g_stream_mu); g_streams[r->s] = r;
+  std::lock_guard<std::mutex> l(g_stream_mu);
+  auto& idle = g_idle_streams[device];
+  if (!idle.empty()) { r->s = idle.back(); idle.pop_back(); }
+  else B200Q_CUDA(cudaStreamCreateWithFlags(&r->s, cudaStreamNonBlocking));
+  g_streams[r->s] = r;
   return r;
 }
 std::shared_ptr<StreamRef> stream_ref_lookup(cudaStream_t s) {
@@ -132,18 +142,18 @@
   if (hot) { cx.m.hot_ms += ms; cx.m.hot_rows += rows; cx.m.hot_launches++; }
 }
 
-static DevMemP upload_program(const CompiledProgram& cp, cudaStream_t s, std::vector<DevMemP>& blooms) {
-  DevMemP d = DevMem::alloc(sizeof(VmProgram), s);
-  VmProgram p = relocated_program(cp, d->ptr);
+static DevMemP upload_program(OpContext& cx, const CompiledProgram& cp, std::vector<DevMemP>& blooms) {
+  DevMemP d = DevMem::alloc(sizeof(VmProgram), cx.stream);
+  auto p = std::make_shared<VmProgram>(relocated_program(cp, d->ptr));
   for (const auto& b : cp.blooms) {
     const size_t bytes = b.filter->words.size() * 8;
-    DevMemP w = DevMem::alloc(bytes, s);
-    B200Q_CUDA(cudaMemcpyAsync(w->ptr, b.filter->words.data(), bytes, cudaMemcpyHostToDevice, s));
-    p.pool[b.pool_index] = (uint64_t)(uintptr_t)w->ptr;
+    DevMemP w = DevMem::alloc(bytes, cx.stream);
+    B200Q_CUDA(cudaMemcpyAsync(w->ptr, b.filter->words.data(), bytes, cudaMemcpyHostToDevice, cx.stream));
+    p->pool[b.pool_index] = (uint64_t)(uintptr_t)w->ptr;
     blooms.push_back(w);
   }
-  B200Q_CUDA(cudaMemcpyAsync(d->ptr, &p, sizeof(VmProgram), cudaMemcpyHostToDevice, s));
-  B200Q_CUDA(cudaStreamSynchronize(s));
+  B200Q_CUDA(cudaMemcpyAsync(d->ptr, p.get(), sizeof(VmProgram), cudaMemcpyHostToDevice, cx.stream));
+  cx.upload_sources.push_back(p);
   return d;
 }
 
@@ -218,7 +228,7 @@
     used_input_cols = cp_.used_cols;
     for (int c : out_src_) if (c >= 0 && std::find(used_input_cols.begin(), used_input_cols.end(), c) == used_input_cols.end()) used_input_cols.push_back(c);
     if (!cx.conf.force_generic_kernels && !varlen_ && !cp_.has_strings && !cp_.vm_only) detect_lean(filters, outs);
-    d_prog_ = upload_program(cp_, cx.stream, d_blooms_);
+    d_prog_ = upload_program(cx, cp_, d_blooms_);
   }
 
   void push(OpContext& cx, DevBatch& in, std::vector<DevBatch>& outs) override {
@@ -739,7 +749,7 @@
     if (merge_mode_ && !columnar_) used_input_cols.push_back(n_in_ - 1);
     std::sort(used_input_cols.begin(), used_input_cols.end());
     used_input_cols.erase(std::unique(used_input_cols.begin(), used_input_cols.end()), used_input_cols.end());
-    d_prog_ = upload_program(cp_, cx.stream, d_blooms_);
+    d_prog_ = upload_program(cx, cp_, d_blooms_);
     if (multi) {
       d_sets_ = DevMem::alloc(sizeof(AggSetDesc) * sets_.size(), cx.stream);
       B200Q_CUDA(cudaMemcpyAsync(d_sets_->ptr, sets_.data(), sizeof(AggSetDesc) * sets_.size(), cudaMemcpyHostToDevice, cx.stream));
@@ -758,12 +768,12 @@
       }
     }
 
-    capacity_ = std::max<uint64_t>(1ULL << 20, (uint64_t)((double)std::max<int64_t>(cx.conf.agg_initial_groups, 1) * AGG_SLOTS_PER_GROUP));
+    capacity_ = std::max<uint64_t>(AGG_MIN_SLOTS, (uint64_t)((double)std::max<int64_t>(cx.conf.agg_initial_groups, 1) * AGG_SLOTS_PER_GROUP));
     if (capacity_ >= (1ULL << 32)) throw PlanError(B200Q_ERR_UNSUPPORTED, "agg_initial_groups too large");
-    alloc_table(cx, capacity_, keys_, accs_, counters_);
+    check_table_budget(cx, (unsigned __int128)capacity_ * (lay_.kstride + lay_.astride) * 8, "hash table");
+    counters_ = DevMem::alloc(64, cx.stream, true);
+    if (!(fast_ok_ && dense_possible_) && !wide_possible_) alloc_table(cx, capacity_, keys_, accs_);
     if (lay_.nkeys == 0) seed_global_group(cx);
-    B200Q_CUDA(cudaStreamSynchronize(cx.stream));
-    cx.m.table_capacity = (int64_t)capacity_;
   }
 
 
@@ -969,7 +979,9 @@
     ts.G = w <= 2 ? 2 : w <= 4 ? 4 : 8;
     for (; w < ts.G; w++) ts.word[w] = constant_word(NOOP, 30);
     sink_ = DevMem::alloc((size_t)FAST_SINK_WARPS * 32, cx.stream);
-    { std::vector<unsigned long long> fill((size_t)FAST_SINK_WARPS * 4, NOOP); B200Q_CUDA(cudaMemcpyAsync(sink_->ptr, fill.data(), fill.size() * 8, cudaMemcpyHostToDevice, cx.stream)); B200Q_CUDA(cudaStreamSynchronize(cx.stream)); }
+    auto fill = std::make_shared<std::vector<unsigned long long>>((size_t)FAST_SINK_WARPS * 4, NOOP);
+    B200Q_CUDA(cudaMemcpyAsync(sink_->ptr, fill->data(), fill->size() * 8, cudaMemcpyHostToDevice, cx.stream));
+    cx.upload_sources.push_back(fill);
     ts.sink = (unsigned long long*)sink_->ptr;
     ws_ = ts; wide_possible_ = true;
   }
@@ -1056,7 +1068,8 @@
     dense_decided_ = true;
     if (!fast_ok_ || !dense_possible_ || n == 0) return;
     DenseRange dr;
-    if (!dense_range(cx, ct, n, fs_.nkeys, fs_.key_col, fs_.key_phys, fs_.dense_stride, cx.conf.agg_hot_key_cache != 0, dr)) return;
+    const bool probe_skew = cx.conf.agg_hot_key_cache != 0 && !(fs_.nfilt > 0 && fs_.nfcol >= 0);
+    if (!dense_range(cx, ct, n, fs_.nkeys, fs_.key_col, fs_.key_phys, fs_.dense_stride, probe_skew, dr)) return;
     fs_.dense_base = dr.base[0]; fs_.dense_cap0 = dr.span[0];
     fs_.dense_base1 = dr.base[1]; fs_.dense_r1 = dr.span[1];
     fs_.dense_cap = dr.entries;
@@ -1108,11 +1121,11 @@
       throw ExecError(B200Q_ERR_UNSUPPORTED, std::string("aggregate ") + what + " of " + std::to_string((unsigned long long)bytes) + " bytes exceeds the HBM budget (agg_max_table_bytes = " +
                                                  std::to_string(budget) + "): the table cannot spill on the GPU, fall back to the host path (agg_table.rs:540-588)");
   }
-  void alloc_table(OpContext& cx, uint64_t cap, DevMemP& keys, DevMemP& accs, DevMemP& counters) {
+  void alloc_table(OpContext& cx, uint64_t cap, DevMemP& keys, DevMemP& accs) {
     check_table_budget(cx, (unsigned __int128)cap * (lay_.kstride + lay_.astride) * 8, "hash table");
     keys = DevMem::alloc((size_t)cap * lay_.kstride * 8, cx.stream, true);
     accs = DevMem::alloc((size_t)cap * lay_.astride * 8, cx.stream);
-    counters = DevMem::alloc(64, cx.stream, true);
+    cx.m.table_capacity = (int64_t)cap;
   }
 
   void seed_global_group(OpContext& cx) {
@@ -1130,6 +1143,7 @@
   }
 
   static constexpr double AGG_SLOTS_PER_GROUP = 3.0, AGG_LOAD_LIMIT = 0.5;
+  static constexpr uint64_t AGG_MIN_SLOTS = 1ULL << 20;
   static uint64_t load_limit(uint64_t cap) {
     const uint64_t lim = (uint64_t)((double)cap * AGG_LOAD_LIMIT);
     return cap > (1ULL << 19) ? std::min<uint64_t>(lim, cap - (1ULL << 19)) : lim;
@@ -1147,14 +1161,15 @@
     uint64_t cap = capacity_;
     do cap <<= 1; while (load_limit(cap) < min_groups);
     if (cap >= (1ULL << 32)) throw ExecError(B200Q_ERR_UNSUPPORTED, "aggregate hash table beyond 2^32 slots");
-    DevMemP nkeys, naccs, ncounters;
-    alloc_table(cx, cap, nkeys, naccs, ncounters);
+    DevMemP nkeys, naccs;
+    alloc_table(cx, cap, nkeys, naccs);
+    DevMemP ncounters = DevMem::alloc(64, cx.stream, true);
     AggTable oldt = table_view(0);
     AggTable newt{}; newt.keys = (unsigned long long*)nkeys->ptr; newt.accs = (unsigned long long*)naccs->ptr; newt.capacity = cap; newt.max_groups = load_limit(cap); newt.counters = (unsigned long long*)ncounters->ptr;
     cx.m.launches += launch_agg_rehash(lay_, oldt, newt, cx.stream);
     B200Q_CUDA(cudaGetLastError());
     keys_ = nkeys; accs_ = naccs; counters_ = ncounters; capacity_ = cap;
-    cx.m.grow_count++; cx.m.table_capacity = (int64_t)cap;
+    cx.m.grow_count++;
   }
 
   void read_counters(OpContext& cx, unsigned long long (&h)[3]) {
@@ -1242,7 +1257,7 @@
       cx.m.launches += launch_update(cx, ct, table_view(0), begin, m, nullptr);
       B200Q_CUDA(cudaEventRecord(s.k1, cx.stream));
       B200Q_CUDA(cudaGetLastError());
-      B200Q_CUDA(cudaMemcpyAsync(s.h, counters_->ptr, 24, cudaMemcpyDeviceToHost, cx.stream));
+      cx.m.launches += launch_agg_counters_snapshot((const unsigned long long*)counters_->ptr, s.h, cx.stream);
       B200Q_CUDA(cudaEventRecord(s.ready, cx.stream));
       const double ts = hnow(); t_launch += ts - tl;
       const bool slow = have_prev && settle((idx & 1) ^ 1, prev_begin, prev_m, true, begin, m);
@@ -1266,6 +1281,10 @@
       ct.col[i] = dev_col_of(c < n_in_ ? in.cols[c] : state_cols[c - n_in_]);
     }
     if (!dense_decided_) { if (wide_possible_) decide_wide(cx, ct, n); else decide_dense(cx, ct, n); }
+    if (!keys_) {
+      if (fs_.dense || ws_.dense_tab) capacity_ = AGG_MIN_SLOTS;
+      alloc_table(cx, capacity_, keys_, accs_);
+    }
     update_rows(cx, ct, n);
     rows_pushed_ += (uint64_t)n;
   }
@@ -1298,23 +1317,22 @@
   }
 
   void finish(OpContext& cx, std::vector<DevBatch>& outs) override {
-    const bool wide = wide_possible_ && ws_.dense_tab;
+    const bool wide = wide_possible_ && ws_.dense_tab, dense = fs_.dense || wide;
     ensure_snaps();
     unsigned long long* hs = snap_[0].h;
-    DevMemP dc;
-    if (fs_.dense || wide) {
-      dc = DevMem::alloc(8, cx.stream, true);
+    int64_t g;
+    if (dense) {
+      g = ngroups_ + (int64_t)std::min<uint64_t>(fs_.dense ? fs_.dense_cap : ws_.dense_cap, rows_pushed_);
       if (wide) cx.m.launches += launch_tile_wide_normalise(ws_, cx.stream);
-      cx.m.launches += fs_.dense ? launch_dense_count(fs_, (unsigned long long*)dc->ptr, cx.stream) : launch_tile_wide_count(ws_, (unsigned long long*)dc->ptr, cx.stream);
-      B200Q_CUDA(cudaMemcpyAsync(hs + 3, dc->ptr, 8, cudaMemcpyDeviceToHost, cx.stream));
-    } else hs[3] = 0;
-    B200Q_CUDA(cudaMemcpyAsync(hs, counters_->ptr, 24, cudaMemcpyDeviceToHost, cx.stream));
-    B200Q_CUDA(cudaStreamSynchronize(cx.stream));
-    check_device_error_flags((int)hs[2]);
-    ngroups_ = (int64_t)hs[0];
-    const int64_t g = ngroups_ + (int64_t)hs[3];
-    cx.m.num_groups = g;
-    if (g == 0) return;
+    } else {
+      B200Q_CUDA(cudaMemcpyAsync(hs, counters_->ptr, 24, cudaMemcpyDeviceToHost, cx.stream));
+      B200Q_CUDA(cudaStreamSynchronize(cx.stream));
+      check_device_error_flags((int)hs[2]);
+      ngroups_ = (int64_t)hs[0];
+      g = ngroups_;
+      cx.m.num_groups = g;
+      if (g == 0) return;
+    }
     EmitTable et{}; et.ncols = (int)emit_.size();
     if (et.ncols > EMIT_MAX_COLS) throw ExecError(B200Q_ERR_UNSUPPORTED, "too many output columns");
     DevBatch ob; ob.num_rows = g;
@@ -1329,7 +1347,7 @@
       ob.cols.push_back(c);
     }
     DevMemP out_count = DevMem::alloc(8, cx.stream, true);
-    cx.m.launches += launch_agg_emit(lay_, table_view(0), et, (unsigned long long*)out_count->ptr, cx.stream);
+    if (ngroups_ > 0) cx.m.launches += launch_agg_emit(lay_, table_view(0), et, (unsigned long long*)out_count->ptr, cx.stream);
     if (fs_.dense) cx.m.launches += launch_agg_emit_dense(fs_, et, dmap_, (unsigned long long*)out_count->ptr, cx.stream);
     if (wide) cx.m.launches += launch_tile_wide_emit(ws_, lay_, et, (unsigned long long*)out_count->ptr, cx.stream);
     for (size_t i = 0; i < emit_.size(); i++) {
@@ -1337,6 +1355,15 @@
       if (bool_bytes[i]) ob.cols[i].values = pack_bits(cx, bool_bytes[i]->ptr, g);
     }
     B200Q_CUDA(cudaGetLastError());
+    auto read_count = [&] {
+      B200Q_CUDA(cudaMemcpyAsync(hs, counters_->ptr, 24, cudaMemcpyDeviceToHost, cx.stream));
+      B200Q_CUDA(cudaMemcpyAsync(hs + 3, out_count->ptr, 8, cudaMemcpyDeviceToHost, cx.stream));
+      B200Q_CUDA(cudaStreamSynchronize(cx.stream));
+      check_device_error_flags((int)hs[2]);
+      g = ob.num_rows = (int64_t)hs[3];
+      cx.m.num_groups = g;
+    };
+    if (dense && !final_ && !columnar_) { read_count(); if (g == 0) return; }
     if (!final_ && !columnar_) {
       FrozenTable ft{}; ft.nfields = (int)frozen_fields_.size();
       for (int k = 0; k < ft.nfields; k++) {
@@ -1360,7 +1387,8 @@
       ob.cols.resize(lay_.nkeys);
       ob.cols.push_back(bc);
     }
-    B200Q_CUDA(cudaStreamSynchronize(cx.stream));
+    if (dense && (final_ || columnar_)) { read_count(); if (g == 0) return; }
+    else B200Q_CUDA(cudaStreamSynchronize(cx.stream));
     outs.push_back(std::move(ob));
   }
 };
```

Result: faster. 87.36 billion, median of 6 (+3.3%).
